# BoloniniD/CSWin-UNet

Measured on AMD Instinct MI355X. Metric: training images/sec (224x224, cswin_tiny), higher is better.
Workload: dtype f32; 1 GPU; cswin_tiny_224_lite, synthetic 224x224 9-class, bs=24/GPU, fp32 matmul, fwd + 0.4CE+0.6Dice + bwd + SGD(momentum) step, drop_path 0.2; global_batch=24, img_size=224, parallelism=dp1, hip_graph=True

## Files before the change

cswin_unet_amd/_lib.py:

```python
import ctypes
import os
from ctypes import c_char_p, c_double, c_float, c_int, c_long, c_size_t, c_void_p

import torch

_HERE = os.path.dirname(os.path.abspath(__file__))
LIB_PATH = os.path.join(_HERE, "libcswin_hip.so")

P, I, F, SZ, L, D = c_void_p, c_int, c_float, c_size_t, c_long, c_double

ABI_VERSION = 4

SIGNATURES = {
    "cswin_last_error": (c_char_p, []),
    "cswin_abi_version": (I, []),
    "cswin_device_ok": (I, []),
    "cswin_attn_fwd": (I, [P, P, P, P, P, P, I, I, I, I, P, P, I, F, F, ctypes.c_ulonglong, P, I, P]),
    "cswin_attn_bwd_workspace": (SZ, [I, I, I, I, P, P, I]),
    "cswin_attn_bwd": (I, [P, P, P, P, P, P, P, P, P, P, SZ, I, I, I, I, P, P, I, F, P, F, ctypes.c_ulonglong, P, I, P]),
    "cswin_img2windows": (I, [P, P, I, I, I, I, I, I, P]),
    "cswin_windows2img": (I, [P, P, I, I, I, I, I, I, P]),
    "cswin_layernorm_fwd": (I, [P, P, P, P, P, P, I, I, F, I, P]),
    "cswin_layernorm_bwd_workspace": (SZ, [I, I]),
    "cswin_layernorm_bwd": (I, [P, P, P, P, P, P, P, P, P, P, SZ, I, I, P, P, P]),
    "cswin_linear_fwd": (I, [P, P, I, P, P, P, P, P, P, I, I, I, I, I, I, P]),
    "cswin_linear_bwd_data": (I, [P, P, P, P, I, P, P, I, P, I, I, I, I, I, P]),
    "cswin_linear_bwd_weight_workspace": (SZ, [I, I, I]),
    "cswin_linear_bwd_weight": (I, [P, P, P, I, P, I, P, P, P, SZ, I, I, I, P, I, P]),
    "cswin_linear_bwd_weight_batch": (I, [P, I, P, P, I, P]),
    "cswin_linear_bwd_tail": (I, [P, P, P, I, I, I, P, I, P, P, I, P]),
    "cswin_linear_bwd_weight_batch_masked": (I, [P, I, P, P, I, P, P, P]),
    "cswin_linear_bwd_tail_masked": (I, [P, P, P, I, I, I, P, I, P, P, I, P, P, P]),
    "cswin_rows_sum_multi": (I, [P, I, P]),
    "cswin_conv_tok_fwd": (I, [P, P, P, P, I, I, I, I, I, I, I, I, I, P]),
    "cswin_conv_tok_bwd_data": (I, [P, P, P, I, I, I, I, I, I, I, I, I, P]),
    "cswin_conv_tok_bwd_weight_workspace": (SZ, [I, I, I, I, I, I, I, I]),
    "cswin_conv_tok_bwd_weight": (I, [P, P, P, P, P, SZ, I, I, I, I, I, I, I, I, I, P, I, P]),
    "cswin_conv_weight_permute": (I, [P, P, P, I, I, I, I, P]),
    "cswin_conv_weight_unpermute": (I, [P, P, I, I, I, I, P]),
    "cswin_conv_weight_flipT": (I, [P, P, I, I, I, P]),
    "cswin_conv_weight_images": (I, [P, I, P]),
    "cswin_conv_tok_bwd_weight_cpad": (I, [P, P, P, P, P, SZ, I, I, I, I, I, I, I, I, I, P, I, P]),
    "cswin_nchw_to_tokens": (I, [P, P, I, I, I, I, I, P]),
    "cswin_tokens_to_nchw": (I, [P, P, I, I, I, I, I, P]),
    "cswin_carafe_fwd": (I, [P, P, P, P, P, I, I, I, I, I, P]),
    "cswin_carafe_bwd_workspace": (SZ, [I, I, I, I, I]),
    "cswin_carafe_bwd": (I, [P, P, P, P, P, P, P, SZ, I, I, I, I, I, P, P]),
    "cswin_carafe_fwd_nchw": (I, [P, P, P, P, P, I, I, I, I, I, I, P]),
    "cswin_carafe_bwd_nchw_ok": (I, [I, I, I, I]),
    "cswin_carafe_bwd_nchw": (I, [P, P, P, P, P, P, P, SZ, I, I, I, I, I, I, P, P]),
    "cswin_head_compose": (I, [P, P, P, P, P, I, I, I, I, P]),
    "cswin_head_compose_bwd": (I, [P, P, P, P, P, P, P, P, I, I, I, P]),
    "cswin_loss_workspace": (SZ, [I, I, L]),
    "cswin_loss_sums": (I, [P, P, P, P, SZ, I, I, L, I, P]),
    "cswin_loss_finalize": (I, [P, P, P, D, I, F, F, P, P]),
    "cswin_loss_bwd": (I, [P, P, P, P, P, F, F, I, I, L, I, P]),
    "cswin_cl_loss_workspace": (SZ, [I, I, L]),
    "cswin_cl_loss_sums": (I, [P, P, P, I, P, P, P, P, SZ, I, I, I, L, F, F, F, P]),
    "cswin_cl_loss_finalize": (I, [P, P, P, D, D, I, F, F, F, F, P]),
    "cswin_cl_loss_bwd": (I, [P, P, P, I, P, P, P, P, P, F, F, F, I, I, I, L, F, F, F, P]),
    "cswin_dropout": (I, [P, P, P, P, L, L, F, ctypes.c_ulonglong, P, P]),
    "cswin_sgd_flat": (I, [P, P, P, L, P, F, F, F, P, P]),
    "cswin_multi_copy": (I, [P, I, P]),
    "cswin_chunk_sumsq": (I, [P, P, P, I, P, P]),
    "cswin_norm_finalize": (I, [P, P, I, F, F, P, P, P]),
    "cswin_adamw_flat": (I, [P, P, P, P, P, I, P, P, P, D, D, D, F, F, D, D, P, P]),
    "cswin_tpgm_chunk_stats": (I, [P, P, P, P, I, I, P, P]),
    "cswin_tpgm_finalize": (I, [P, P, I, I, P, P, P, P, D, D, D, D, I, P, P, P, P]),
    "cswin_tpgm_project": (I, [P, P, P, P, P, I, P, P]),
    "cswin_pack_bf16": (I, [P, P, L, P]),
    "cswin_pack_bf16_scaled": (I, [P, P, L, F, P]),
    "cswin_unpack_bf16": (I, [P, P, L, P]),
    "cswin_seg_metrics_nbins": (I, [I, I, I]),
    "cswin_seg_metrics_workspace": (SZ, [I, I, I, I, I]),
    "cswin_seg_metrics": (I, [P, P, P, P, P, SZ, I, I, I, I, I, P]),
    "cswin_resize_banded": (I, [P, P, P, P, I, P, P, I, I, I, I, I, I, I, P]),
    "cswin_argmax_zoom_back": (I, [P, P, P, P, I, I, I, I, I, I, P]),
    "cswin_argmax_zoom_back_classes": (I, [P, P, P, P, P, I, I, I, I, I, I, I, P]),
    "cswin_class_counts": (I, [P, I, P, I, P, I, L, I, P]),
    "cswin_augment_gather": (I, [P, P, P, I, I, I, I, I, I, P]),
    "cswin_augment_labels": (I, [P, P, P, P, P, P, P, I, I, I, I, I, I, P]),
}



class WgradDesc(ctypes.Structure):
    _fields_ = [("dy", c_void_p), ("x", c_void_p), ("row_scale", c_void_p), ("dw", c_void_p), ("dbias", c_void_p),
                ("workspace", c_void_p), ("ws_bytes", c_size_t), ("rows_per_sample", c_int), ("M", c_int), ("N", c_int),
                ("K", c_int), ("precision", c_int), ("io_bf16", c_int)]


class ReduceJob(ctypes.Structure):
    _fields_ = [("part", c_void_p), ("out", c_void_p), ("out2", c_void_p), ("n_first", ctypes.c_longlong),
                ("n", ctypes.c_longlong), ("stride", ctypes.c_longlong), ("rows", c_int), ("reserved", c_int),
                ("conv_kk", c_int), ("conv_cin", c_int)]


class ConvImageJob(ctypes.Structure):
    _fields_ = [("w", c_void_p), ("w_perm", c_void_p), ("w_permT", c_void_p), ("w_flipT", c_void_p), ("Cout", c_int),
                ("Cin", c_int), ("ks", c_int), ("Cpad", c_int)]


class AugmentDesc(ctypes.Structure):
    _fields_ = [("kind", c_int), ("k", c_int), ("axis", c_int), ("src", c_int), ("map", c_void_p)]


_lib = None

PREC_FP32, PREC_BF16 = 0, 1
_state = {"precision": PREC_FP32, "act_bf16": True}


def precision():
    return _state["precision"]


def act_bf16():
    return _state["precision"] == PREC_BF16 and _state["act_bf16"]


def set_act_bf16(on):
    prev = _state["act_bf16"]
    _state["act_bf16"] = bool(on)
    return prev


_shadows = []


class _Shadow:

    def __init__(self, owner_obj, owner, seen):
        import weakref
        self.ref = weakref.ref(owner_obj)
        self.base, self.nbytes, self.seen = owner.data_ptr(), owner.numel() * 4, seen


def register_shadow(owner_obj, owner):
    _shadows[:] = [e for e in _shadows if e.ref() is not None and e.base != owner.data_ptr()]
    _shadows.append(_Shadow(owner_obj, owner, {p.data_ptr(): p._version for p in owner_obj.params}))


def shadow_ptr(w):
    if not _shadows or w is None:
        return None
    a = w.data_ptr()
    for e in _shadows:
        if e.base <= a < e.base + e.nbytes:
            opt = e.ref()
            if opt is None:
                return None
            if e.seen.get(a) != w._version:
                opt.refresh_shadow()
                e.seen.clear()
                e.seen.update({p.data_ptr(): p._version for p in opt.params})
                e.seen[a] = w._version
            return c_void_p(opt.flat_param16.data_ptr() + (a - e.base) // 2)
    return None


def shadows_current(opt):
    if _state["precision"] != PREC_BF16:
        return
    for e in _shadows:
        if e.ref() is opt:
            if any(e.seen.get(p.data_ptr()) != p._version for p in opt.params):
                opt.refresh_shadow()
                e.seen.clear()
                e.seen.update({p.data_ptr(): p._version for p in opt.params})
            return


def set_precision(mode):
    prev = _state["precision"]
    _state["precision"] = int(mode)
    if int(mode) == PREC_BF16 and prev != PREC_BF16:
        for e in _shadows:
            opt = e.ref()
            if opt is not None:
# ... 53 lines not shown
```

cswin_unet_amd/csrc/gemm.hip:

```cpp
#include <stdlib.h>

#include <type_traits>
#include "common.h"
#include "gemm_epilogue.h"

int cswin_gemm16(int mode, int epi_mode, const void* A, const void* B, const void* epilogue, int M, int NO, int R, void* stream);
int cswin_wgrad16_batch(const cswin_wgrad_desc* d, int n, const int* splits, const int* rows_per_split, const cswin_reduce_job* pending,
                        int npending, void* stream, long long* stamps);

namespace {

constexpr int BKMAX = 64;

typedef __bf16 bf16x8 __attribute__((ext_vector_type(8)));

#define CSWIN_CHECK_PRECISION(p, who) CSWIN_REQUIRE((p) == 0 || (p) == 1, CSWIN_ERR_UNSUPPORTED, who ": precision %d (0 = fp32, 1 = bf16 operands)", (p))

struct PlainSrc {
    const float* p; long ld; int rows, cols;
    const float* row_scale; int rows_per_sample;
    int bf16;
    static constexpr bool fast_div = false;
    struct Row { const float* base; float s; };
    typedef int Col;
    __device__ Col col(int j) const { return j; }
    __device__ Row row(int i) const {
        Row r;
        r.base = (i < rows) ? p + (long)i * ld : nullptr;
        r.s = (row_scale && i < rows) ? row_scale[i / rows_per_sample] : 1.0f;
        return r;
    }
    __device__ const float* ptr(const Row& r, int j) const { return (r.base && j < cols) ? r.base + j : nullptr; }
};

template <class S> __device__ __forceinline__ bool src_is_bf16(const S&) { return false; }
__device__ __forceinline__ bool src_is_bf16(const PlainSrc& s) { return s.bf16 != 0; }
template <class S> __device__ __forceinline__ u32x2 src_load4_bf16(const S&, const float*) { return u32x2{0u, 0u}; }
__device__ __forceinline__ u32x2 src_load4_bf16(const PlainSrc& s, const float* p) {
    return *reinterpret_cast<const u32x2*>(reinterpret_cast<const __bf16*>(s.p) + (p - s.p));
}
template <class S> __device__ __forceinline__ typename S::Row src_mapped_row(const S&, int, float) { return typename S::Row{}; }
__device__ __forceinline__ PlainSrc::Row src_mapped_row(const PlainSrc& s, int row, float f) {
    PlainSrc::Row r;
    r.base = row >= 0 ? s.p + (long)row * s.ld : nullptr;
    r.s = f;
    return r;
}
template <class S> __device__ __forceinline__ const float* src_row_scale(const S&) { return nullptr; }
__device__ __forceinline__ const float* src_row_scale(const PlainSrc& s) { return s.row_scale; }

struct ConcatSrc {
    const float* p0; const float* p1; long ld0, ld1; int rows, cols, c0;
    static constexpr bool fast_div = false;
    struct Row { const float* b0; const float* b1; float s; };
    typedef int Col;
    __device__ Col col(int j) const { return j; }
    __device__ Row row(int i) const {
        Row r;
        r.b0 = (i < rows) ? p0 + (long)i * ld0 : nullptr;
        r.b1 = (i < rows) ? p1 + (long)i * ld1 : nullptr;
        r.s = 1.0f;
        return r;
    }
    __device__ const float* ptr(const Row& r, int j) const {
        if (!r.b0 || j >= cols) return nullptr;
        return j < c0 ? r.b0 + j : r.b1 + (j - c0);
    }
};

template <bool FAST> __device__ __forceinline__ int qdiv(int n, int d, unsigned m) {
    if constexpr (FAST) return fdiv1(n, m);
    else return n / d;
}
struct ConvMagics { unsigned img, w, c, ks, stride; };

template <bool FAST>
struct ConvSrcT {
    const float* x; int B, H, W, C, OH, OW, ks, stride, pad; int rows, cols;
    static constexpr bool fast_div = FAST;
    ConvMagics m;
    struct Row { int b, iy0, ix0; float s; };
    struct Col { int ky, kx, ci; };
    __device__ Row row(int i) const {
        Row r;
        r.s = 1.0f;
        if (i >= rows) { r.b = -1; r.iy0 = r.ix0 = 0; return r; }
        int ohw = OH * OW;
        r.b = qdiv<FAST>(i, ohw, m.img);
        int rem = i - r.b * ohw;
        int oy = qdiv<FAST>(rem, OW, m.w);
        r.iy0 = oy * stride - pad;
        r.ix0 = (rem - oy * OW) * stride - pad;
        return r;
    }
    __device__ Col col(int j) const {
        Col c;
        if (j >= cols) { c.ky = c.kx = 0; c.ci = -1; return c; }
        int tap = qdiv<FAST>(j, C, m.c);
        c.ci = j - tap * C;
        c.ky = qdiv<FAST>(tap, ks, m.ks);
        c.kx = tap - c.ky * ks;
        return c;
    }
    __device__ const float* ptr(const Row& r, const Col& c) const {
        if (r.b < 0 || c.ci < 0) return nullptr;
        int iy = r.iy0 + c.ky, ix = r.ix0 + c.kx;
        if ((unsigned)iy >= (unsigned)H || (unsigned)ix >= (unsigned)W) return nullptr;
        return x + ((long)(r.b * H + iy) * W + ix) * C + c.ci;
    }
};

template <bool FAST>
struct ConvTSrcT {
    const float* dy; int B, H, W, C, OH, OW, ks, stride, pad; int rows, cols;
    static constexpr bool fast_div = FAST;
    ConvMagics m;
    struct Row { int b, iy, ix; float s; };
    struct Col { int ky, kx, co; };
    __device__ Row row(int i) const {
        Row r;
        r.s = 1.0f;
        if (i >= rows) { r.b = -1; r.iy = r.ix = 0; return r; }
        int hw = H * W;
        r.b = qdiv<FAST>(i, hw, m.img);
        int rem = i - r.b * hw;
        r.iy = qdiv<FAST>(rem, W, m.w);
        r.ix = rem - r.iy * W;
        return r;
    }
    __device__ Col col(int j) const {
        Col c;
        if (j >= cols) { c.ky = c.kx = 0; c.co = -1; return c; }
        int tap = qdiv<FAST>(j, C, m.c);
        c.co = j - tap * C;
        c.ky = qdiv<FAST>(tap, ks, m.ks);
        c.kx = tap - c.ky * ks;
        return c;
    }
    __device__ const float* ptr(const Row& r, const Col& c) const {
        if (r.b < 0 || c.co < 0) return nullptr;
        int ty = r.iy + pad - c.ky, tx = r.ix + pad - c.kx;
        if (ty < 0 || tx < 0) return nullptr;
        int oy = qdiv<FAST>(ty, stride, m.stride), ox = qdiv<FAST>(tx, stride, m.stride);
        if (oy * stride != ty || ox * stride != tx || oy >= OH || ox >= OW) return nullptr;
        return dy + ((long)(r.b * OH + oy) * OW + ox) * C + c.co;
    }
};

template <bool FAST>
struct ConvTS2SrcT {
    const float* dy; int B, H, W, C, OH, OW, py, px, H2, W2, kys, kxs; int rows, cols;
    static constexpr bool fast_div = FAST;
    ConvMagics m;
    struct Row { int b, iy, ix; float s; };
    struct Col { int ky, kx, co; };
    __device__ Row row(int i) const {
        Row r;
        r.s = 1.0f;
        if (i >= rows) { r.b = -1; r.iy = r.ix = 0; return r; }
        const int hw = H2 * W2;
        r.b = qdiv<FAST>(i, hw, m.img);
        const int rem = i - r.b * hw;
        const int jy = qdiv<FAST>(rem, W2, m.w);
        r.iy = 2 * jy + py;
        r.ix = 2 * (rem - jy * W2) + px;
        return r;
    }
    __device__ Col col(int j) const {
        Col c;
        if (j >= cols) { c.ky = c.kx = 0; c.co = -1; return c; }
        const int t = qdiv<FAST>(j, C, m.c);
        c.co = j - t * C;
        c.ky = (kys >> (2 * t)) & 3;
        c.kx = (kxs >> (2 * t)) & 3;
        return c;
    }
    __device__ const float* ptr(const Row& r, const Col& c) const {
        if (r.b < 0 || c.co < 0) return nullptr;
        const int oy = (r.iy + 1 - c.ky) >> 1, ox = (r.ix + 1 - c.kx) >> 1;
        if (oy >= OH || ox >= OW) return nullptr;
        return dy + ((long)(r.b * OH + oy) * OW + ox) * C + c.co;
    }
};

template <bool FAST>
struct TapRowsSrcT {
    const float* w; int Cout, Cin, taps; int rows, cols;
    unsigned m_cout;
    struct Row { const float* base; float s; };
    typedef int Col;
    __device__ Row row(int i) const {
        Row r;
        r.s = 1.0f;
        if (i >= rows) { r.base = nullptr; return r; }
        const int t = qdiv<FAST>(i, Cout, m_cout), co = i - t * Cout;
        r.base = w + ((long)((taps >> (4 * t)) & 15) * Cout + co) * Cin;
        return r;
    }
    __device__ Col col(int j) const { return j; }
    __device__ const float* ptr(const Row& r, int j) const { return (r.base && j < cols) ? r.base + j : nullptr; }
};

template <int BM, int BN, int BK, int KW, bool A_RC, bool B_RC>
constexpr int gemm_lds_floats() {
    constexpr int NW = (BM >= 64 ? 2 : 1) * (BN >= 64 ? 2 : 1);
    constexpr int LDR = BK + 4;
    constexpr int A_ELEMS = A_RC ? BM * LDR : BK * (BM + 4);
    constexpr int B_ELEMS = B_RC ? BN * LDR : BK * (BN + 4);
    return (A_ELEMS + B_ELEMS) > NW * EP_WAVE_FLOATS ? (A_ELEMS + B_ELEMS) : NW * EP_WAVE_FLOATS;
}

struct RowMask { const float* skip; int nsamples, rows_per_sample, splits; unsigned magic; };
constexpr int MASK_MAX_SAMPLES = 256;
struct KeptList { int n; int idx[MASK_MAX_SAMPLES]; float scale[MASK_MAX_SAMPLES]; };

template <int BM, int BN, int BK, int KW, bool A_RC, bool B_RC, int VEC, int EPI, bool SCALE_A, int PREC, class ASrc, class BSrc,
          bool MASKED = false>
__device__ __forceinline__ void gemm_body(float* lds, const ASrc& A, const BSrc& B, const Epilogue& epi, int M, int N, int R,
                                          int r_per_split, int tiles_m, int tiles_n, int bid, int nblk, int stamp_row,
                                          const RowMask* mk = nullptr, KeptList* kept = nullptr) {
    constexpr int WGM = BM >= 64 ? 2 : 1, WGN = BN >= 64 ? 2 : 1, NW = WGM * WGN;
    constexpr int WM = BM / WGM, WN = BN / WGN;
    constexpr int FM = WM / 32, FN = WN / 32;
    constexpr int LDR = BK + 4;
    constexpr int LDA = A_RC ? LDR : BM + 4;
    constexpr int LDB = B_RC ? LDR : BN + 4;
    constexpr int A_ELEMS = A_RC ? BM * LDR : BK * (BM + 4);
    constexpr int B_ELEMS = B_RC ? BN * LDR : BK * (BN + 4);
    constexpr int LDS_FLOATS = gemm_lds_floats<BM, BN, BK, KW, A_RC, B_RC>();
    static_assert(LDS_FLOATS >= A_ELEMS + B_ELEMS && LDS_FLOATS >= NW * EP_WAVE_FLOATS, "gemm_lds_floats out of step with the tile geometry");
    float* As = lds;
    float* Bs = lds + A_ELEMS;
    constexpr int LD16 = BK + 8;
    unsigned short* As16 = reinterpret_cast<unsigned short*>(lds);
    unsigned short* Bs16 = As16 + BM * LD16;
    static_assert(PREC == 0 || ((BM + BN) * LD16 * 2 <= LDS_FLOATS * 4 && (BK / KW) % 16 == 0), "bf16 tile does not fit");

    constexpr int NTH = 64 * NW * KW;
    const int tid = threadIdx.x, lane = tid & 63, wave = (tid >> 6) % NW, kg = tid / (64 * NW);
    const int li = lane & 31, lh = lane >> 5;
    const int xq = nblk >> 3, xr = nblk & 7, xcd = bid & 7;
    const int lb = (xcd < xr ? xcd * (xq + 1) : xr * (xq + 1) + (xcd - xr) * xq) + (bid >> 3);
    const int tiles = tiles_m * tiles_n;
    const int split = lb / tiles;
    const int tile = lb - split * tiles;
    const int m0 = (tile / tiles_n) * BM, n0 = (tile % tiles_n) * BN;
    if constexpr (MASKED) {
        static_assert(!A_RC && !B_RC && VEC == 4 && BM == BN && std::is_same<ASrc, PlainSrc>::value && std::is_same<BSrc, PlainSrc>::value,
                      "the sample mask serves weight gradients of plain matrices (one row mapping for both operands)");
        if (tid < 64) {
            int n = 0;
            for (int s0 = 0; s0 < mk->nsamples; s0 += 64) {
                const int s = s0 + lane;
                const bool keep = s < mk->nsamples && mk->skip[s] != 0.0f;
                const unsigned long long bal = __ballot(keep);
                if (keep) {
                    const int at = n + __popcll(bal & ((1ull << lane) - 1ull));
                    kept->idx[at] = s;
                    kept->scale[at] = src_row_scale(A) ? src_row_scale(A)[s] : 1.0f;
                }
                n += __popcll(bal);
            }
            if (tid == 0) kept->n = n;
        }
        __syncthreads();
        R = __builtin_amdgcn_readfirstlane(kept->n) * mk->rows_per_sample;
        r_per_split = ((R + mk->splits - 1) / mk->splits + 7) / 8 * 8;
    }
    const int r_begin = split * r_per_split;
    const int r_end = min(R, r_begin + r_per_split);
    const int wm0 = (wave / WGN) * WM, wn0 = (wave % WGN) * WN;

    constexpr int QA = BM * BK / (4 * NTH), QB = BN * BK / (4 * NTH);
    static_assert(QA >= 1 && QB >= 1 && (BK / KW) % 8 == 0, "tile too small for this many wave groups");
    constexpr int A_CPR = A_RC ? BK / 4 : BM / 4;
    constexpr int B_CPR = B_RC ? BK / 4 : BN / 4;
    constexpr int A_RPP = NTH / A_CPR, B_RPP = NTH / B_CPR;
    const int a_c = tid % A_CPR, a_r = tid / A_CPR;
    const int b_c = tid % B_CPR, b_r = tid / B_CPR;

    typename ASrc::Row arow[QA];
    typename BSrc::Row brow[QB];
    if (A_RC) {
#pragma unroll
        for (int q = 0; q < QA; ++q) arow[q] = A.row(m0 + a_r + q * A_RPP);
    }
    if (B_RC) {
#pragma unroll
        for (int q = 0; q < QB; ++q) brow[q] = B.row(n0 + b_r + q * B_RPP);
    }

    const typename ASrc::Col acol = A.col(m0 + 4 * a_c);
    const typename BSrc::Col bcol = B.col(n0 + 4 * b_c);

    f32x4 pa[QA], pb[QB];
    u32x2 pa16[QA], pb16[QB];
    float pas[QA];
    auto fetch = [&](int r0, auto a16, auto b16) {
        int mrow[QA];
        float msc[QA];
        if constexpr (MASKED) {
#pragma unroll
            for (int q = 0; q < QA; ++q) {
                const int c = r0 + a_r + q * A_RPP;
                mrow[q] = -1;
                msc[q] = 1.0f;
                if (c < r_end) {
                    const int j = fdiv1(c, mk->magic);
                    mrow[q] = kept->idx[j] * mk->rows_per_sample + (c - j * mk->rows_per_sample);
                    msc[q] = kept->scale[j];
                }
            }
        }
#pragma unroll
        for (int q = 0; q < QA; ++q) {
            typename ASrc::Row rr;
            int j;
            if (A_RC) {
                rr = arow[q];
                j = r0 + 4 * a_c;
            } else {
                const int r = r0 + a_r + q * A_RPP;
                if constexpr (MASKED) rr = src_mapped_row(A, mrow[q], msc[q]);
                else rr = A.row(r < r_end ? r : 0x7fffffff);
                j = m0 + 4 * a_c;
            }
            if (SCALE_A) pas[q] = rr.s;
            if (VEC == 4) {
                const float* p = A_RC ? (j < r_end ? A.ptr(rr, A.col(j)) : nullptr) : A.ptr(rr, acol);
                if constexpr (decltype(a16)::value) {
                    pa16[q] = u32x2{0u, 0u};
                    if (p) pa16[q] = src_load4_bf16(A, p);
                } else {
                    pa[q] = f32x4{0.f, 0.f, 0.f, 0.f};
                    if (p) pa[q] = *reinterpret_cast<const f32x4*>(p);
                }
            } else {
#pragma unroll
                for (int e = 0; e < 4; ++e) {
                    const float* p = (!A_RC || j + e < r_end) ? A.ptr(rr, A.col(j + e)) : nullptr;
                    pa[q][e] = p ? *p : 0.f;
                }
            }
        }
#pragma unroll
        for (int q = 0; q < QB; ++q) {
            typename BSrc::Row rr;
            int j;
            if (B_RC) {
                rr = brow[q];
                j = r0 + 4 * b_c;
            } else {
                const int r = r0 + b_r + q * B_RPP;
                if constexpr (MASKED) rr = src_mapped_row(B, mrow[q], 1.0f);
                else rr = B.row(r < r_end ? r : 0x7fffffff);
                j = n0 + 4 * b_c;
            }
            if (VEC == 4) {
                const float* p = B_RC ? (j < r_end ? B.ptr(rr, B.col(j)) : nullptr) : B.ptr(rr, bcol);
                if constexpr (decltype(b16)::value) {
                    pb16[q] = u32x2{0u, 0u};
                    if (p) pb16[q] = src_load4_bf16(B, p);
                } else {
                    pb[q] = f32x4{0.f, 0.f, 0.f, 0.f};
                    if (p) pb[q] = *reinterpret_cast<const f32x4*>(p);
                }
            } else {
#pragma unroll
                for (int e = 0; e < 4; ++e) {
                    const float* p = (!B_RC || j + e < r_end) ? B.ptr(rr, B.col(j + e)) : nullptr;
                    pb[q][e] = p ? *p : 0.f;
                }
            }
        }
    };
    auto stash = [&](auto a16, auto b16) {
#pragma unroll
        for (int q = 0; q < QA; ++q) {
            f32x4 v = f32x4{0.f, 0.f, 0.f, 0.f};
            if constexpr (!decltype(a16)::value) v = pa[q];
            if constexpr (PREC == 1) {
                unsigned h01, h23;
                if constexpr (decltype(a16)::value) {
                    h01 = pa16[q][0];
                    h23 = pa16[q][1];
                    if (SCALE_A) {
                        const u32x2 u = __builtin_bit_cast(u32x2, __builtin_convertvector(widen_bf16x4(pa16[q]) * pas[q], bf16x4));
                        h01 = u[0]; h23 = u[1];
                    }
                } else {
                    if (SCALE_A) v *= pas[q];
                    const u32x2 u = __builtin_bit_cast(u32x2, __builtin_convertvector(v, bf16x4));
                    h01 = u[0]; h23 = u[1];
                }
                if (A_RC) {
                    *reinterpret_cast<u32x2*>(&As16[(a_r + q * A_RPP) * LD16 + 4 * a_c]) = u32x2{h01, h23};
                } else {
                    unsigned short* col = &As16[4 * a_c * LD16 + a_r + q * A_RPP];
                    col[0] = (unsigned short)(h01 & 0xffffu);
                    col[LD16] = (unsigned short)(h01 >> 16);
                    col[2 * LD16] = (unsigned short)(h23 & 0xffffu);
                    col[3 * LD16] = (unsigned short)(h23 >> 16);
                }
            } else {
                if (SCALE_A) v *= pas[q];
                *reinterpret_cast<f32x4*>(&As[(a_r + q * A_RPP) * LDA + 4 * a_c]) = v;
            }
        }
#pragma unroll
        for (int q = 0; q < QB; ++q) {
            if constexpr (PREC == 1) {
                u32x2 hb;
                if constexpr (decltype(b16)::value) hb = pb16[q];
                else hb = __builtin_bit_cast(u32x2, __builtin_convertvector(pb[q], bf16x4));
                if (B_RC) {
                    *reinterpret_cast<u32x2*>(&Bs16[(b_r + q * B_RPP) * LD16 + 4 * b_c]) = hb;
                } else {
                    static_assert(B_RC || BN == 64, "transposed-read B image is laid out for 64-column tiles");
                    const int row = b_r + q * B_RPP;
                    *reinterpret_cast<u32x2*>(&Bs16[row * BN + 8 * ((b_c >> 1) ^ (((row >> 1) & 1) << 2)) + 4 * (b_c & 1)]) = hb;
                }
            } else {
                *reinterpret_cast<f32x4*>(&Bs[(b_r + q * B_RPP) * LDB + 4 * b_c]) = pb[q];
            }
        }
    };

    f32x16 acc[FM][FN];
#pragma unroll
    for (int i = 0; i < FM; ++i)
#pragma unroll
        for (int j = 0; j < FN; ++j)
#pragma unroll
            for (int e = 0; e < 16; ++e) acc[i][j][e] = 0.f;

    float csum = 0.f;
    const bool do_colsum = !A_RC && epi.colsum && n0 == 0 && tid < BM;

    if (epi.stamps && tid == 0) { epi.stamps[8L * stamp_row + 0] = __builtin_amdgcn_s_memtime(); epi.stamps[8L * stamp_row + 4] = __builtin_amdgcn_s_getreg(6164); epi.stamps[8L * stamp_row + 5] = __builtin_amdgcn_s_memrealtime(); }
    auto main_loop = [&](auto a16, auto b16) {
        fetch(r_begin, a16, b16);
        stash(a16, b16);
        __syncthreads();
        if (epi.stamps && tid == 0) epi.stamps[8L * stamp_row + 1] = __builtin_amdgcn_s_memtime();
        for (int r0 = r_begin; r0 < r_end; r0 += BK) {
            const bool more = r0 + BK < r_end;
            if (more) fetch(r0 + BK, a16, b16);
            if (do_colsum) {
                if constexpr (PREC == 1) {
#pragma unroll 8
                    for (int r = 0; r < BK; ++r)
                        csum += __builtin_bit_cast(float, (unsigned)As16[tid * LD16 + r] << 16);
                } else {
#pragma unroll 8
                    for (int r = 0; r < BK; ++r) csum += As[r * LDA + tid];
                }
            }
            if constexpr (PREC == 1) {
#pragma unroll
                for (int kk = kg * (BK / KW); kk < (kg + 1) * (BK / KW); kk += 16) {
                    bf16x8 af[FM], bf[FN];
#pragma unroll
                    for (int i = 0; i < FM; ++i)
                        af[i] = *reinterpret_cast<const bf16x8*>(&As16[(wm0 + i * 32 + li) * LD16 + kk + 8 * lh]);
#pragma unroll
                    for (int j = 0; j < FN; ++j) {
                        if constexpr (B_RC) {
                            bf[j] = *reinterpret_cast<const bf16x8*>(&Bs16[(wn0 + j * 32 + li) * LD16 + kk + 8 * lh]);
                        } else {
                            typedef short s16x4 __attribute__((ext_vector_type(4)));
                            typedef short s16x8 __attribute__((ext_vector_type(8)));
                            typedef __attribute__((address_space(3))) s16x4 lds_s16x4;
                            const int col = wn0 + j * 32 + 16 * ((lane >> 4) & 1) + 4 * (lane & 3);
                            const int row = kk + 8 * lh + ((lane & 15) >> 2);
                            const int sw = ((row >> 1) & 1) << 2;
                            const unsigned short* a0 = &Bs16[row * BN + 8 * ((col >> 3) ^ sw) + (col & 7)];
                            const s16x4 v0 = __builtin_amdgcn_ds_read_tr16_b64_v4i16((lds_s16x4*)a0);
                            const s16x4 v1 = __builtin_amdgcn_ds_read_tr16_b64_v4i16((lds_s16x4*)(a0 + 4 * BN));
                            const s16x8 f = {v0[0], v0[1], v0[2], v0[3], v1[0], v1[1], v1[2], v1[3]};
                            bf[j] = __builtin_bit_cast(bf16x8, f);
                        }
                    }
#pragma unroll
                    for (int i = 0; i < FM; ++i)
#pragma unroll
                        for (int j = 0; j < FN; ++j)
                            acc[i][j] = __builtin_amdgcn_mfma_f32_32x32x16_bf16(af[i], bf[j], acc[i][j], 0, 0, 0);
                }
            } else
#pragma unroll
            for (int kk = kg * (BK / KW); kk < (kg + 1) * (BK / KW); kk += 8) {
                f32x4 af[FM], bf[FN];
#pragma unroll
                for (int i = 0; i < FM; ++i) {
                    if (A_RC) {
                        af[i] = *reinterpret_cast<const f32x4*>(&As[(wm0 + i * 32 + li) * LDA + kk + 4 * lh]);
                    } else {
#pragma unroll
                        for (int s = 0; s < 4; ++s) af[i][s] = As[(kk + 4 * lh + s) * LDA + wm0 + i * 32 + li];
                    }
                }
#pragma unroll
                for (int j = 0; j < FN; ++j) {
                    if (B_RC) {
                        bf[j] = *reinterpret_cast<const f32x4*>(&Bs[(wn0 + j * 32 + li) * LDB + kk + 4 * lh]);
                    } else {
#pragma unroll
                        for (int s = 0; s < 4; ++s) bf[j][s] = Bs[(kk + 4 * lh + s) * LDB + wn0 + j * 32 + li];
                    }
                }
#pragma unroll
                for (int s = 0; s < 4; ++s)
#pragma unroll
                    for (int i = 0; i < FM; ++i)
#pragma unroll
                        for (int j = 0; j < FN; ++j)
                            acc[i][j] = __builtin_amdgcn_mfma_f32_32x32x2f32(af[i][s], bf[j][s], acc[i][j], 0, 0, 0);
            }
            __syncthreads();
            if (more) {
                stash(a16, b16);
                __syncthreads();
            }
        }
    };
    if (r_begin < r_end) {
        constexpr bool CAN_A16 = PREC == 1 && A_RC && VEC == 4 && std::is_same<ASrc, PlainSrc>::value;
        constexpr bool CAN_B16 = PREC == 1 && A_RC && VEC == 4 && std::is_same<BSrc, PlainSrc>::value;
        const bool a_is16 = CAN_A16 && src_is_bf16(A), b_is16 = CAN_B16 && src_is_bf16(B);
        if constexpr (CAN_A16 && CAN_B16) {
            if (a_is16 && b_is16) main_loop(std::true_type{}, std::true_type{});
            else if (a_is16) main_loop(std::true_type{}, std::false_type{});
            else if (b_is16) main_loop(std::false_type{}, std::true_type{});
            else main_loop(std::false_type{}, std::false_type{});
        } else if constexpr (CAN_B16) {
            if (b_is16) main_loop(std::false_type{}, std::true_type{});
            else main_loop(std::false_type{}, std::false_type{});
        } else {
            main_loop(std::false_type{}, std::false_type{});
        }
    }

    if (epi.stamps && tid == 0) epi.stamps[8L * stamp_row + 2] = __builtin_amdgcn_s_memtime();
    if (KW > 1) {
        static_assert(KW == 1 || (KW / 2) * NW * FM * FN * 16 * 64 <= LDS_FLOATS, "LDS too small for the k-group reduction");
        constexpr int PATCH = FM * FN * 16 * 64;
#pragma unroll
        for (int half = KW / 2; half >= 1; half >>= 1) {
            if (kg >= half && kg < 2 * half) {
                float* dst = lds + ((kg - half) * NW + wave) * PATCH + lane;
#pragma unroll
                for (int i = 0; i < FM; ++i)
#pragma unroll
                    for (int j = 0; j < FN; ++j)
#pragma unroll
                        for (int g = 0; g < 16; ++g) dst[((i * FN + j) * 16 + g) * 64] = acc[i][j][g];
            }
            __syncthreads();
            if (kg < half) {
                const float* src = lds + (kg * NW + wave) * PATCH + lane;
#pragma unroll
                for (int i = 0; i < FM; ++i)
#pragma unroll
                    for (int j = 0; j < FN; ++j)
#pragma unroll
                        for (int g = 0; g < 16; ++g) acc[i][j][g] += src[((i * FN + j) * 16 + g) * 64];
            }
            __syncthreads();
        }
        if (kg != 0) return;
    }
    Epilogue e = epi;
    e.C += (long)split * e.split_stride;
    if constexpr (EPI == EPI_GELUBWD) {
        if (e.pre_bf16) run_epilogue<EPI, FM, FN, true>(e, acc, M, N, m0 + wm0, n0 + wn0, lane, lds + wave * EP_WAVE_FLOATS, e.vec_store != 0);
        else run_epilogue<EPI, FM, FN, false>(e, acc, M, N, m0 + wm0, n0 + wn0, lane, lds + wave * EP_WAVE_FLOATS, e.vec_store != 0);
    } else {
        if constexpr (ASrc::fast_div)
            run_epilogue<EPI, FM, FN, false, true>(e, acc, M, N, m0 + wm0, n0 + wn0, lane, lds + wave * EP_WAVE_FLOATS, e.vec_store != 0, A.m.img, A.m.w);
        else
            run_epilogue<EPI, FM, FN>(e, acc, M, N, m0 + wm0, n0 + wn0, lane, lds + wave * EP_WAVE_FLOATS, e.vec_store != 0);
    }
    if (epi.stamps && tid == 0) { epi.stamps[8L * stamp_row + 3] = __builtin_amdgcn_s_memtime(); epi.stamps[8L * stamp_row + 6] = __builtin_amdgcn_s_memrealtime(); }
    if (do_colsum && m0 + tid < M) epi.colsum[(long)split * epi.colsum_stride + m0 + tid] = csum;
}

constexpr int gemm_threads(int BM, int BN, int KW) { return 64 * (BM >= 64 ? 2 : 1) * (BN >= 64 ? 2 : 1) * KW; }

template <int BM, int BN, int BK, int KW, bool A_RC, bool B_RC, int VEC, int EPI, bool SCALE_A, int PREC, class ASrc, class BSrc>
__global__ __launch_bounds__(gemm_threads(BM, BN, KW)) void gemm_kernel(ASrc A, BSrc B, Epilogue epi, int M, int N, int R,
                                                    int r_per_split, int tiles_m, int tiles_n) {
    __shared__ __attribute__((aligned(16))) float lds[gemm_lds_floats<BM, BN, BK, KW, A_RC, B_RC>()];
    gemm_body<BM, BN, BK, KW, A_RC, B_RC, VEC, EPI, SCALE_A, PREC, ASrc, BSrc>(lds, A, B, epi, M, N, R, r_per_split, tiles_m, tiles_n,
                                                                              (int)blockIdx.x, (int)gridDim.x, (int)blockIdx.x);
}

constexpr int WGRAD_BATCH = 4;
template <class ASrc, class BSrc>
struct GemmBatch {
    ASrc A[WGRAD_BATCH];
    BSrc B[WGRAD_BATCH];
    Epilogue e[WGRAD_BATCH];
    int M[WGRAD_BATCH], N[WGRAD_BATCH], R[WGRAD_BATCH], rps[WGRAD_BATCH], tm[WGRAD_BATCH], tn[WGRAD_BATCH];
    int first[WGRAD_BATCH + 1];
    int n;
    RowMask mask[WGRAD_BATCH];
};
typedef GemmBatch<PlainSrc, PlainSrc> WgradBatch;

__device__ __forceinline__ void wgrad_masked_batch_body(float* lds, KeptList* kept, const WgradBatch& b, int p, int bid) {
    if (b.mask[p].skip) {
        gemm_body<64, 64, 64, 2, false, false, 4, EPI_PLAIN, true, 0, PlainSrc, PlainSrc, true>(
            lds, b.A[p], b.B[p], b.e[p], b.M[p], b.N[p], b.R[p], b.rps[p], b.tm[p], b.tn[p], bid - b.first[p],
            b.first[p + 1] - b.first[p], bid, &b.mask[p], kept);
        return;
    }
    gemm_body<64, 64, 64, 2, false, false, 4, EPI_PLAIN, true, 0, PlainSrc, PlainSrc>(
        lds, b.A[p], b.B[p], b.e[p], b.M[p], b.N[p], b.R[p], b.rps[p], b.tm[p], b.tn[p], bid - b.first[p],
        b.first[p + 1] - b.first[p], bid);
}

template <int PREC>
__global__ __launch_bounds__(512) void gemm_wgrad_batch_kernel(WgradBatch b) {
    int p = 0;
    while (p + 1 < b.n && (int)blockIdx.x >= b.first[p + 1]) ++p;
    __shared__ __attribute__((aligned(16))) float lds[gemm_lds_floats<64, 64, 64, 2, false, false>()];
    gemm_body<64, 64, 64, 2, false, false, 4, EPI_PLAIN, true, PREC, PlainSrc, PlainSrc>(
        lds, b.A[p], b.B[p], b.e[p], b.M[p], b.N[p], b.R[p], b.rps[p], b.tm[p], b.tn[p], (int)blockIdx.x - b.first[p],
        b.first[p + 1] - b.first[p], (int)blockIdx.x);
}
__global__ __launch_bounds__(512) void gemm_wgrad_batch_masked_kernel(WgradBatch b) {
    int p = 0;
    while (p + 1 < b.n && (int)blockIdx.x >= b.first[p + 1]) ++p;
    __shared__ __attribute__((aligned(16))) float lds[gemm_lds_floats<64, 64, 64, 2, false, false>()];
    __shared__ KeptList kept;
    wgrad_masked_batch_body(lds, &kept, b, p, (int)blockIdx.x);
}

struct BlockTail {
    PlainSrc dA, dB;
    Epilogue de;
    int dM, dN, dR, drps, dtm, dtn, nd;
    WgradBatch w;
    ReduceRiders r;
};
constexpr int BLOCK_TAIL_LDS = gemm_lds_floats<64, 64, 64, 2, true, false>() > gemm_lds_floats<64, 64, 64, 2, false, false>()
                                   ? gemm_lds_floats<64, 64, 64, 2, true, false>() : gemm_lds_floats<64, 64, 64, 2, false, false>();
template <bool MASKED>
__device__ __forceinline__ void block_tail_body(float (&lds)[BLOCK_TAIL_LDS], KeptList* kept, const BlockTail& t) {
    const WgradBatch& b = t.w;
    const int nw = b.first[b.n];
    if ((int)blockIdx.x >= nw + t.nd) {
        if (threadIdx.x >= 256) return;
        static_assert(sizeof(lds) >= sizeof(float) * RS_G * (RS_COLS + 1), "reduction scratch");
        rows_sum_dispatch(t.r.j, t.r.first_block, t.r.njobs, (int)blockIdx.x - nw - t.nd, reinterpret_cast<float(*)[RS_COLS + 1]>(lds));
        return;
    }
    if ((int)blockIdx.x >= nw) {
        gemm_body<64, 64, 64, 2, true, false, 4, EPI_PLAIN, false, 0, PlainSrc, PlainSrc>(
            lds, t.dA, t.dB, t.de, t.dM, t.dN, t.dR, t.drps, t.dtm, t.dtn, (int)blockIdx.x - nw, t.nd, (int)blockIdx.x);
        return;
    }
    const int bid = (int)blockIdx.x;
    int p = 0;
    while (p + 1 < b.n && bid >= b.first[p + 1]) ++p;
    if constexpr (MASKED) {
        wgrad_masked_batch_body(lds, kept, b, p, bid);
    } else {
        gemm_body<64, 64, 64, 2, false, false, 4, EPI_PLAIN, true, 0, PlainSrc, PlainSrc>(
            lds, b.A[p], b.B[p], b.e[p], b.M[p], b.N[p], b.R[p], b.rps[p], b.tm[p], b.tn[p], bid - b.first[p],
            b.first[p + 1] - b.first[p], (int)blockIdx.x);
    }
}
__global__ __launch_bounds__(512) void gemm_block_tail_kernel(BlockTail t) {
    __shared__ __attribute__((aligned(16))) float lds[BLOCK_TAIL_LDS];
    block_tail_body<false>(lds, nullptr, t);
}
__global__ __launch_bounds__(512) void gemm_block_tail_masked_kernel(BlockTail t) {
    __shared__ __attribute__((aligned(16))) float lds[BLOCK_TAIL_LDS];
    __shared__ KeptList kept;
    block_tail_body<true>(lds, &kept, t);
}

template <int KW, int PREC, bool FAST>
__global__ __launch_bounds__(256 * KW) void gemm_conv_s2_dgrad_batch_kernel(GemmBatch<ConvTS2SrcT<FAST>, TapRowsSrcT<FAST>> b) {
    int p = 0;
    while (p + 1 < b.n && (int)blockIdx.x >= b.first[p + 1]) ++p;
    __shared__ __attribute__((aligned(16))) float lds[gemm_lds_floats<64, 64, (KW == 1 ? 32 : 64), KW, true, false>()];
    gemm_body<64, 64, (KW == 1 ? 32 : 64), KW, true, false, 4, EPI_PLAIN, false, PREC, ConvTS2SrcT<FAST>, TapRowsSrcT<FAST>>(
        lds, b.A[p], b.B[p], b.e[p], b.M[p], b.N[p], b.R[p], b.rps[p], b.tm[p], b.tn[p], (int)blockIdx.x - b.first[p],
        b.first[p + 1] - b.first[p], (int)blockIdx.x);
}

template <int BM, int BN, int BK, int KW, bool A_RC, bool B_RC, int VEC, int EPI, bool SCALE_A, int PREC, class ASrc, class BSrc>
void launch_cfg(const ASrc& A, const BSrc& B, const Epilogue& epi, int M, int N, int R, int splits, int r_per_split,
                hipStream_t st) {
    int tm = cdiv(M, BM), tn = cdiv(N, BN);
    dim3 grid(tm * tn * splits);
    const int pad_lds = cswin_tuning().gemm_pad_lds;
    hipLaunchKernelGGL((gemm_kernel<BM, BN, BK, KW, A_RC, B_RC, VEC, EPI, SCALE_A, PREC, ASrc, BSrc>), grid, dim3(gemm_threads(BM, BN, KW)), pad_lds, st, A, B, epi,
                       M, N, R, r_per_split, tm, tn);
}

int k_groups(long blocks, int r_len) {
    if (blocks < 320 && r_len >= 512) return 4;
    if (blocks < 640 && r_len >= 256) return 2;
    return 1;
}

int one_split(int R) { return cdiv(R, BKMAX) * BKMAX; }

template <bool A_RC, bool B_RC, int VEC, int EPI, bool SCALE_A, class ASrc, class BSrc>
void launch_gemm(const ASrc& A, const BSrc& B, const Epilogue& epi_in, int M, int N, int R, int splits, int r_per_split,
                 int precision, hipStream_t st) {
    Epilogue epi = epi_in;
    epi.vec_store = epilogue_vec_ok(epi, N);
    auto blocks = [&](int bm, int bn) { return (long)cdiv(M, bm) * cdiv(N, bn) * splits; };
    const int forced_kw = cswin_tuning().gemm_kw;
    const int forced_tile = cswin_tuning().gemm_tile;
    const double pen2 = cswin_tuning().gemm_pen2;
    auto cost = [&](int bm, int bn, double pen) { return (double)((blocks(bm, bn) + 255) / 256) * bm * bn * pen; };
    int tile = 1;
    if (splits == 1 && cost(64, 32, pen2) < cost(64, 64, 1.0)) tile = 2;
    if (forced_tile) tile = forced_tile;
    const int r_len = r_per_split < R ? r_per_split : R;
    const bool wgrad = !A_RC && !B_RC;
    if (precision == 1) {
        if (k_groups(blocks(64, 64), r_len) >= 2 || (wgrad && r_len >= 256))
            launch_cfg<64, 64, 64, 2, A_RC, B_RC, VEC, EPI, SCALE_A, 1>(A, B, epi, M, N, R, splits, r_per_split, st);
        else launch_cfg<64, 64, 64, 1, A_RC, B_RC, VEC, EPI, SCALE_A, 1>(A, B, epi, M, N, R, splits, r_per_split, st);
        return;
    }
    if (tile == 2) {
        if (k_groups(blocks(64, 32), r_len) >= 2)
            return launch_cfg<64, 32, 64, 2, A_RC, B_RC, VEC, EPI, SCALE_A, 0>(A, B, epi, M, N, R, splits, r_per_split, st);
        return launch_cfg<64, 32, 32, 1, A_RC, B_RC, VEC, EPI, SCALE_A, 0>(A, B, epi, M, N, R, splits, r_per_split, st);
    }
    int kw = k_groups(blocks(64, 64), r_len);
    if (wgrad && r_len >= 256 && kw < 2) kw = 2;
    if (forced_kw) kw = forced_kw;
    if (kw == 4) launch_cfg<64, 64, 64, 4, A_RC, B_RC, VEC, EPI, SCALE_A, 0>(A, B, epi, M, N, R, splits, r_per_split, st);
    else if (kw == 2) launch_cfg<64, 64, 64, 2, A_RC, B_RC, VEC, EPI, SCALE_A, 0>(A, B, epi, M, N, R, splits, r_per_split, st);
    else launch_cfg<64, 64, 32, 1, A_RC, B_RC, VEC, EPI, SCALE_A, 0>(A, B, epi, M, N, R, splits, r_per_split, st);
}

template <bool A_RC, bool B_RC, int EPI, bool SCALE_A, class ASrc, class BSrc>
void launch_gemm_vec(bool vec, const ASrc& A, const BSrc& B, const Epilogue& epi, int M, int N, int R, int splits, int r_per_split,
// ... 222 lines not shown
        if (x.njobs > 0) {
            rblocks = fill_reduce_table(x.jobs, x.njobs, t.r.j, t.r.first_block);
            CSWIN_REQUIRE(rblocks >= 0, CSWIN_ERR_SHAPE, "linear_bwd_tail: bad pending reduction");
            t.r.njobs = x.njobs;
        }
        static_assert(sizeof(BlockTail) <= 4096, "kernel argument block");
        if (any_mask) hipLaunchKernelGGL(gemm_block_tail_masked_kernel, dim3(blocks + t.nd + rblocks), dim3(512), 0, (hipStream_t)stream, t);
        else hipLaunchKernelGGL(gemm_block_tail_kernel, dim3(blocks + t.nd + rblocks), dim3(512), 0, (hipStream_t)stream, t);
    } else if (any_mask) {
        hipLaunchKernelGGL(gemm_wgrad_batch_masked_kernel, dim3(blocks), dim3(512), 0, (hipStream_t)stream, b);
    } else if (precision == 1) {
        hipLaunchKernelGGL(gemm_wgrad_batch_kernel<1>, dim3(blocks), dim3(512), 0, (hipStream_t)stream, b);
    } else {
        hipLaunchKernelGGL(gemm_wgrad_batch_kernel<0>, dim3(blocks), dim3(512), 0, (hipStream_t)stream, b);
    }
    CSWIN_LAUNCH_CHECK();
    return CSWIN_OK;
}

bool conv_magics(ConvMagics* m, long nrows, int img, int w, long ncols, int c, int ks, int cmax, int stride) {
    *m = ConvMagics{fdiv_magic(img), fdiv_magic(w), fdiv_magic(c), fdiv_magic(ks), fdiv_magic(stride)};
    return fdiv_exact(nrows + 63, img) && fdiv_exact(img - 1, w) && fdiv_exact(ncols - 1, c) && fdiv_exact((long)ks * ks - 1, ks) &&
           (stride == 0 || fdiv_exact(cmax, stride));
}
template <class F> void with_fast_div(bool fast, F f) {
    if (fast) f(std::true_type{});
    else f(std::false_type{});
}

int conv_wgrad_impl(const float* dy, const float* x, float* dw_perm, float* dbias, void* workspace, size_t ws_bytes, int B, int H,
                    int W, int Cin, int Cout, int ks, int stride, int pad, int torch_layout, int Cin_param,
                    cswin_reduce_job* deferred, int precision, void* stream) {
    CSWIN_CHECK_PRECISION(precision, "conv_tok_bwd_weight");
    CSWIN_REQUIRE(dy && x && dw_perm, CSWIN_ERR_SHAPE, "conv_tok_bwd_weight: null pointer");
    CSWIN_REQUIRE(Cin % 4 == 0 && Cout % 4 == 0 && aligned16(dy) && aligned16(x), CSWIN_ERR_ALIGN, "conv_tok_bwd_weight: channels %% 4 and 16-B alignment required");
    CSWIN_REQUIRE(!torch_layout || Cin < 65536, CSWIN_ERR_UNSUPPORTED, "conv_tok_bwd_weight: torch_layout needs Cin < 65536");
    int OH = (H + 2 * pad - ks) / stride + 1, OW = (W + 2 * pad - ks) / stride + 1;
    int M = B * OH * OW, K = ks * ks * Cin;
    size_t need = WgradSlabs::bytes(M, Cout, K);
    CSWIN_REQUIRE(workspace && ws_bytes >= need, CSWIN_ERR_WORKSPACE, "conv_tok_bwd_weight: workspace %zu < %zu", ws_bytes, need);
    hipStream_t st = (hipStream_t)stream;
    int splits, rps;
    choose_split(M, Cout, K, &splits, &rps);
    const WgradSlabs slabs(workspace, Cout, K);
    PlainSrc A = {dy, Cout, M, Cout, nullptr, 1};
    ConvMagics mg;
    with_fast_div(conv_magics(&mg, M, OH * OW, OW, K, Cin, ks, 0, 0), [&](auto fast) {
        ConvSrcT<decltype(fast)::value> Bm = {x, B, H, W, Cin, OH, OW, ks, stride, pad, M, K, mg};
        launch_gemm<false, false, 4, EPI_PLAIN, false>(A, Bm, slabs.epilogue(dbias != nullptr), Cout, K, M, splits, rps, precision, st);
    });
    CSWIN_LAUNCH_CHECK();
    reduce_now_or_defer(slabs.job(dw_perm, dbias, splits, torch_layout ? ks * ks : 0,
                                  torch_layout ? (Cin | (Cin_param != Cin ? Cin_param << 16 : 0)) : 0), deferred, st);
    CSWIN_LAUNCH_CHECK();
    return CSWIN_OK;
}

}

extern "C" {

void cswin_debug_set_stamps(void* p) { g_stamps = (long long*)p; }

int cswin_linear_bwd_weight_batch_masked(const cswin_wgrad_desc* d, int n, cswin_reduce_job* deferred, const cswin_reduce_job* pending,
                                         int npending, const float* const* skip, const int* nsamples, void* stream);
int cswin_linear_bwd_tail_masked(const float* dy, const float* w, float* dx, int M, int N, int K, const cswin_wgrad_desc* d, int n,
                                 cswin_reduce_job* deferred, const cswin_reduce_job* pending, int npending, const float* const* skip,
                                 const int* nsamples, void* stream);

int cswin_linear_fwd(const float* x, const float* x2, int k_split, const float* w, const float* bias, float* y,
                     float* y_act, const float* residual, const float* row_scale, int rows_per_sample, int M, int N,
                     int K, int precision, int io_bf16, void* stream) {
    CSWIN_CHECK_PRECISION(precision, "linear_fwd");
    CSWIN_REQUIRE(io_bf16 == 0 || (precision == 1 && (!x2 || !(io_bf16 & 1)) && (io_bf16 & ~7) == 0 && K % 4 == 0 && N % 4 == 0 && !((io_bf16 & 2) && residual)), CSWIN_ERR_UNSUPPORTED,
                  "linear_fwd: bf16 storage (io_bf16 = %d: 1 = x, 2 = y / y_act, 4 = w) needs precision 1, a plain input for bit 1, K and N multiples of 4; a residual output stays fp32", io_bf16);
    CSWIN_REQUIRE(x && w && y && M > 0 && N > 0 && K > 0, CSWIN_ERR_SHAPE, "linear_fwd: bad arguments M=%d N=%d K=%d", M, N, K);
    CSWIN_REQUIRE(!x2 || (k_split > 0 && k_split < K), CSWIN_ERR_SHAPE, "linear_fwd: bad concat split %d of K=%d", k_split, K);
    CSWIN_REQUIRE(!row_scale || rows_per_sample > 0, CSWIN_ERR_SHAPE, "linear_fwd: rows_per_sample must be > 0");
    hipStream_t st = (hipStream_t)stream;
    Epilogue e = plain_epilogue(y, N);
    e.bias = bias;
    e.Cact = y_act; e.ldact = N;
    e.residual = residual; e.ldres = N;
    e.row_scale = row_scale; e.rows_per_sample = rows_per_sample;
    e.c_bf16 = (io_bf16 & 2) != 0;
    PlainSrc B = {w, K, N, K, nullptr, 1, (io_bf16 >> 2) & 1};
    CSWIN_REQUIRE(!(y_act && residual), CSWIN_ERR_UNSUPPORTED, "linear_fwd: activation and residual epilogues are exclusive");
    const int rk = one_split(K);
    if (x2) {
        CSWIN_REQUIRE(!y_act, CSWIN_ERR_UNSUPPORTED, "linear_fwd: concat input does not support the activation epilogue");
        ConcatSrc A = {x, x2, k_split, K - k_split, M, K, k_split};
        bool vec = (k_split % 4 == 0) && (K % 4 == 0) && aligned16(x) && aligned16(x2) && aligned16(w);
        CSWIN_REQUIRE(io_bf16 == 0 || (io_bf16 == 4 && vec), CSWIN_ERR_UNSUPPORTED, "linear_fwd: a concat input takes only the bf16 weight flag (4), with 16-B aligned operands");
        if (residual) launch_gemm_vec<true, true, EPI_RES, false>(vec, A, B, e, M, N, K, 1, rk, precision, st);
        else launch_gemm_vec<true, true, EPI_PLAIN, false>(vec, A, B, e, M, N, K, 1, rk, precision, st);
    } else {
        if (precision == 1 && (io_bf16 & 5) == 5) {
            if (cswin_gemm16(0, y_act ? EPI_ACT : (residual ? EPI_RES : EPI_PLAIN), x, w, &e, M, N, K, stream) == 0) {
                CSWIN_LAUNCH_CHECK();
                return CSWIN_OK;
            }
        }
        PlainSrc A = {x, K, M, K, nullptr, 1, io_bf16 & 1};
        bool vec = (K % 4 == 0) && aligned16(x) && aligned16(w);
        CSWIN_REQUIRE(io_bf16 == 0 || (vec && aligned16(y) && (!y_act || aligned16(y_act)) && (!bias || aligned16(bias))), CSWIN_ERR_ALIGN,
                      "linear_fwd: bf16 storage needs 16-B aligned operands");
        if (y_act) launch_gemm_vec<true, true, EPI_ACT, false>(vec, A, B, e, M, N, K, 1, rk, precision, st);
        else if (residual) launch_gemm_vec<true, true, EPI_RES, false>(vec, A, B, e, M, N, K, 1, rk, precision, st);
        else launch_gemm_vec<true, true, EPI_PLAIN, false>(vec, A, B, e, M, N, K, 1, rk, precision, st);
    }
    CSWIN_LAUNCH_CHECK();
    return CSWIN_OK;
}

int cswin_linear_bwd_data(const float* dy, const float* w, float* dx, float* dx2, int k_split, const float* gelu_pre,
                          const float* row_scale, int rows_per_sample, const float* add, int M, int N, int K,
                          int precision, int io_bf16, void* stream) {
    CSWIN_CHECK_PRECISION(precision, "linear_bwd_data");
    CSWIN_REQUIRE(io_bf16 == 0 || (precision == 1 && ((!dx2 && !add) || (io_bf16 & ~4) == 0) && (io_bf16 & ~15) == 0 && K % 4 == 0 && N % 4 == 0), CSWIN_ERR_UNSUPPORTED,
                  "linear_bwd_data: bf16 storage (io_bf16 = %d: 1 = dy, 2 = dx, 4 = w, 8 = gelu_pre) needs precision 1, K and N multiples of 4; split / add outputs take only the weight flag", io_bf16);
    CSWIN_REQUIRE(dy && w && dx && M > 0 && N > 0 && K > 0, CSWIN_ERR_SHAPE, "linear_bwd_data: bad arguments");
    CSWIN_REQUIRE(!dx2 || (k_split > 0 && k_split < K), CSWIN_ERR_SHAPE, "linear_bwd_data: bad concat split");
    CSWIN_REQUIRE(!row_scale || rows_per_sample > 0, CSWIN_ERR_SHAPE, "linear_bwd_data: rows_per_sample must be > 0");
    hipStream_t st = (hipStream_t)stream;
    Epilogue e = plain_epilogue(dx, dx2 ? k_split : K);
    e.C2 = dx2; e.ldc2 = K - k_split; e.col_split = dx2 ? k_split : 0;
    e.gelu_pre = gelu_pre; e.ldpre = K;
    e.row_scale = row_scale; e.rows_per_sample = rows_per_sample;
    e.residual = add; e.ldres = K;
    e.c_bf16 = (io_bf16 & 2) != 0;
    e.pre_bf16 = (io_bf16 & 8) != 0;
    CSWIN_REQUIRE(io_bf16 == 0 || (aligned16(dy) && aligned16(w) && aligned16(dx) && (!gelu_pre || aligned16(gelu_pre))), CSWIN_ERR_ALIGN,
                  "linear_bwd_data: bf16 storage needs 16-B aligned operands");
    PlainSrc A = {dy, N, M, N, nullptr, 1, io_bf16 & 1};
    PlainSrc B = {w, K, N, K, nullptr, 1, (io_bf16 >> 2) & 1};
    bool vec = (N % 4 == 0) && (K % 4 == 0) && aligned16(dy) && aligned16(w);
    const int rn = one_split(N);
    const int modes = (dx2 != nullptr) + (gelu_pre != nullptr) + (add != nullptr);
    CSWIN_REQUIRE(modes <= 1, CSWIN_ERR_UNSUPPORTED, "linear_bwd_data: dx2 / gelu_pre / add are mutually exclusive");
    if (precision == 1 && !dx2 && !add && (io_bf16 & 5) == 5) {
        if (cswin_gemm16(1, gelu_pre ? EPI_GELUBWD : EPI_PLAIN, dy, w, &e, M, K, N, stream) == 0) {
            CSWIN_LAUNCH_CHECK();
            return CSWIN_OK;
        }
    }
    if (dx2) launch_gemm_vec<true, false, EPI_SPLIT2, false>(vec, A, B, e, M, K, N, 1, rn, precision, st);
    else if (gelu_pre) launch_gemm_vec<true, false, EPI_GELUBWD, false>(vec, A, B, e, M, K, N, 1, rn, precision, st);
    else if (add) launch_gemm_vec<true, false, EPI_RES, false>(vec, A, B, e, M, K, N, 1, rn, precision, st);
    else launch_gemm_vec<true, false, EPI_PLAIN, false>(vec, A, B, e, M, K, N, 1, rn, precision, st);
    CSWIN_LAUNCH_CHECK();
    return CSWIN_OK;
}

size_t cswin_linear_bwd_weight_workspace(int M, int N, int K) { return WgradSlabs::bytes(M, N, K); }

int cswin_linear_bwd_weight(const float* dy, const float* x, const float* x2, int k_split, const float* row_scale,
                            int rows_per_sample, float* dw, float* dbias, void* workspace, size_t ws_bytes, int M,
                            int N, int K, cswin_reduce_job* deferred, int precision, void* stream) {
    CSWIN_CHECK_PRECISION(precision, "linear_bwd_weight");
    CSWIN_REQUIRE(dy && x && dw && M > 0 && N > 0 && K > 0, CSWIN_ERR_SHAPE, "linear_bwd_weight: bad arguments");
    CSWIN_REQUIRE(!x2 || (k_split > 0 && k_split < K), CSWIN_ERR_SHAPE, "linear_bwd_weight: bad concat split");
    CSWIN_REQUIRE(!row_scale || rows_per_sample > 0, CSWIN_ERR_SHAPE, "linear_bwd_weight: rows_per_sample must be > 0");
    size_t need = WgradSlabs::bytes(M, N, K);
    CSWIN_REQUIRE(workspace && ws_bytes >= need, CSWIN_ERR_WORKSPACE, "linear_bwd_weight: workspace %zu < %zu", ws_bytes, need);
    hipStream_t st = (hipStream_t)stream;
    const cswin_wgrad_desc d1 = {dy, x, row_scale, dw, dbias, workspace, ws_bytes, rows_per_sample, M, N, K, precision, 0};
    if (precision == 1 && !x2 && wgrad_aligned(d1)) {
        cswin_reduce_job job;
        int rc = wgrad_batch_impl(&d1, 1, &job, TailExtras{"linear_bwd_weight_batch"}, stream);
        if (rc) return rc;
        reduce_now_or_defer(job, deferred, st);
        CSWIN_LAUNCH_CHECK();
        return CSWIN_OK;
    }
    return wgrad_tiled(dy, x, x2, k_split, row_scale, rows_per_sample, dw, dbias, workspace, M, N, K, deferred, precision, st);
}

int cswin_linear_bwd_weight_batch(const cswin_wgrad_desc* d, int n, cswin_reduce_job* deferred, const cswin_reduce_job* pending, int npending,
                                  void* stream) {
    return cswin_linear_bwd_weight_batch_masked(d, n, deferred, pending, npending, nullptr, nullptr, stream);
}

int cswin_linear_bwd_weight_batch_masked(const cswin_wgrad_desc* d, int n, cswin_reduce_job* deferred, const cswin_reduce_job* pending,
                                         int npending, const float* const* skip, const int* nsamples, void* stream) {
    return wgrad_batch_impl(d, n, deferred,
                            TailExtras{"linear_bwd_weight_batch", nullptr, nullptr, nullptr, 0, 0, 0, pending, npending, skip, nsamples}, stream);
}

int cswin_linear_bwd_tail(const float* dy, const float* w, float* dx, int M, int N, int K, const cswin_wgrad_desc* d, int n,
                          cswin_reduce_job* deferred, const cswin_reduce_job* pending, int npending, void* stream) {
    return cswin_linear_bwd_tail_masked(dy, w, dx, M, N, K, d, n, deferred, pending, npending, nullptr, nullptr, stream);
}

int cswin_linear_bwd_tail_masked(const float* dy, const float* w, float* dx, int M, int N, int K, const cswin_wgrad_desc* d, int n,
                                 cswin_reduce_job* deferred, const cswin_reduce_job* pending, int npending, const float* const* skip,
                                 const int* nsamples, void* stream) {
    CSWIN_REQUIRE(dy && w && dx && M > 0 && N > 0 && K > 0, CSWIN_ERR_SHAPE, "linear_bwd_tail: bad data-gradient arguments");
    return wgrad_batch_impl(d, n, deferred, TailExtras{"linear_bwd_tail", dy, w, dx, M, N, K, pending, npending, skip, nsamples}, stream);
}

int cswin_conv_tok_fwd(const float* x, const float* w_perm, const float* bias, float* y, int B, int H, int W, int Cin,
                       int Cout, int ks, int stride, int pad, int precision, void* stream) {
    CSWIN_CHECK_PRECISION(precision, "conv_tok_fwd");
    CSWIN_REQUIRE(x && w_perm && y && B > 0 && H > 0 && W > 0 && Cin > 0 && Cout > 0, CSWIN_ERR_SHAPE, "conv_tok_fwd: bad arguments");
    CSWIN_REQUIRE(Cin % 4 == 0 && aligned16(x) && aligned16(w_perm), CSWIN_ERR_ALIGN, "conv_tok_fwd: Cin %% 4 and 16-B alignment required");
    int OH = (H + 2 * pad - ks) / stride + 1, OW = (W + 2 * pad - ks) / stride + 1;
    int M = B * OH * OW, R = ks * ks * Cin;
    PlainSrc Bm = {w_perm, R, Cout, R, nullptr, 1};
    Epilogue e = plain_epilogue(y, Cout);
    e.bias = bias;
    ConvMagics mg;
    with_fast_div(conv_magics(&mg, M, OH * OW, OW, R, Cin, ks, 0, 0), [&](auto fast) {
        ConvSrcT<decltype(fast)::value> A = {x, B, H, W, Cin, OH, OW, ks, stride, pad, M, R, mg};
        launch_gemm<true, true, 4, EPI_PLAIN, false>(A, Bm, e, M, Cout, R, 1, one_split(R), precision, (hipStream_t)stream);
    });
    CSWIN_LAUNCH_CHECK();
    return CSWIN_OK;
}

int cswin_conv_tok_bwd_data(const float* dy, const float* w_permT, float* dx, int B, int H, int W, int Cin, int Cout,
                            int ks, int stride, int pad, int precision, void* stream) {
    CSWIN_CHECK_PRECISION(precision, "conv_tok_bwd_data");
    CSWIN_REQUIRE(dy && w_permT && dx, CSWIN_ERR_SHAPE, "conv_tok_bwd_data: null pointer");
    CSWIN_REQUIRE(Cin % 4 == 0 && Cout % 4 == 0 && aligned16(dy) && aligned16(w_permT), CSWIN_ERR_ALIGN, "conv_tok_bwd_data: channels %% 4 and 16-B alignment required");
    int OH = (H + 2 * pad - ks) / stride + 1, OW = (W + 2 * pad - ks) / stride + 1;
    if (ks == 3 && stride == 2 && pad == 1) {
        bool fast_ok = true;
        for (int py = 0; py < 2; ++py)
            for (int px = 0; px < 2; ++px) {
                const int H2 = (H - py + 1) / 2, W2 = (W - px + 1) / 2;
                ConvMagics mg;
                if (H2 > 0 && W2 > 0) fast_ok = fast_ok && conv_magics(&mg, (long)B * H2 * W2, H2 * W2, W2, 4L * Cout, Cout, 1, 0, 0);
            }
        with_fast_div(fast_ok, [&](auto fast) {
            constexpr bool FAST = decltype(fast)::value;
            GemmBatch<ConvTS2SrcT<FAST>, TapRowsSrcT<FAST>> b = {};
            int rmax = 0;
            for (int py = 0; py < 2; ++py)
                for (int px = 0; px < 2; ++px) {
                    const int H2 = (H - py + 1) / 2, W2 = (W - px + 1) / 2;
                    if (H2 <= 0 || W2 <= 0) continue;
                    int kys = 0, kxs = 0, taps = 0, nt = 0;
                    for (int ky = (py ? 0 : 1); ky < 3; ky += 2)
                        for (int kx = (px ? 0 : 1); kx < 3; kx += 2) {
                            kys |= ky << (2 * nt);
                            kxs |= kx << (2 * nt);
                            taps |= (ky * 3 + kx) << (4 * nt);
                            ++nt;
                        }
                    const int Mc = B * H2 * W2, Rc = nt * Cout;
                    Epilogue e = plain_epilogue(dx, Cin);
                    e.rm_on = 1; e.rm_H = H; e.rm_W = W; e.rm_H2 = H2; e.rm_W2 = W2; e.rm_py = py; e.rm_px = px;
                    ConvMagics mg;
                    conv_magics(&mg, Mc, H2 * W2, W2, Rc, Cout, 1, 0, 0);
                    push(b, ConvTS2SrcT<FAST>{dy, B, H, W, Cout, OH, OW, py, px, H2, W2, kys, kxs, Mc, Rc, mg},
                         TapRowsSrcT<FAST>{w_permT, Cout, Cin, taps, Rc, Cin, mg.c}, e, Mc, Cin, Rc, one_split(Rc), 1);
                    rmax = Rc > rmax ? Rc : rmax;
                }
            if (b.n > 0) {
                const int blocks = b.first[b.n];
                hipStream_t st = (hipStream_t)stream;
                const int kw = k_groups(blocks, rmax);
                if (precision == 1) hipLaunchKernelGGL((gemm_conv_s2_dgrad_batch_kernel<2, 1, FAST>), dim3(blocks), dim3(512), 0, st, b);
                else if (kw == 4) hipLaunchKernelGGL((gemm_conv_s2_dgrad_batch_kernel<4, 0, FAST>), dim3(blocks), dim3(1024), 0, st, b);
                else if (kw == 2) hipLaunchKernelGGL((gemm_conv_s2_dgrad_batch_kernel<2, 0, FAST>), dim3(blocks), dim3(512), 0, st, b);
                else hipLaunchKernelGGL((gemm_conv_s2_dgrad_batch_kernel<1, 0, FAST>), dim3(blocks), dim3(256), 0, st, b);
            }
        });
        CSWIN_LAUNCH_CHECK();
        return CSWIN_OK;
    }
    int M = B * H * W, R = ks * ks * Cout;
    PlainSrc Bm = {w_permT, Cin, R, Cin, nullptr, 1};
    Epilogue e = plain_epilogue(dx, Cin);
    ConvMagics mg;
    with_fast_div(conv_magics(&mg, M, H * W, W, R, Cout, ks, (H > W ? H : W) + pad, stride), [&](auto fast) {
        ConvTSrcT<decltype(fast)::value> A = {dy, B, H, W, Cout, OH, OW, ks, stride, pad, M, R, mg};
        launch_gemm<true, false, 4, EPI_PLAIN, false>(A, Bm, e, M, Cin, R, 1, one_split(R), precision, (hipStream_t)stream);
    });
    CSWIN_LAUNCH_CHECK();
    return CSWIN_OK;
}

size_t cswin_conv_tok_bwd_weight_workspace(int B, int H, int W, int Cin, int Cout, int ks, int stride, int pad) {
    int OH = (H + 2 * pad - ks) / stride + 1, OW = (W + 2 * pad - ks) / stride + 1;
    return WgradSlabs::bytes(B * OH * OW, Cout, ks * ks * Cin);
}

int cswin_conv_tok_bwd_weight(const float* dy, const float* x, float* dw_perm, float* dbias, void* workspace,
                              size_t ws_bytes, int B, int H, int W, int Cin, int Cout, int ks, int stride, int pad,
                              int torch_layout, cswin_reduce_job* deferred, int precision, void* stream) {
    return conv_wgrad_impl(dy, x, dw_perm, dbias, workspace, ws_bytes, B, H, W, Cin, Cout, ks, stride, pad, torch_layout, Cin, deferred,
                           precision, stream);
}

int cswin_conv_tok_bwd_weight_cpad(const float* dy, const float* x, float* dw, float* dbias, void* workspace, size_t ws_bytes,
                                   int B, int H, int W, int Cin, int Cin_param, int Cout, int ks, int stride, int pad,
                                   cswin_reduce_job* deferred, int precision, void* stream) {
    CSWIN_REQUIRE(Cin_param > 0 && Cin_param <= Cin && Cin < 65536, CSWIN_ERR_SHAPE, "conv_tok_bwd_weight_cpad: 0 < Cin_param <= Cin < 65536");
    return conv_wgrad_impl(dy, x, dw, dbias, workspace, ws_bytes, B, H, W, Cin, Cout, ks, stride, pad, 1, Cin_param, deferred, precision,
                           stream);
}

int cswin_rows_sum_multi(const cswin_reduce_job* jobs, int njobs, void* stream) { return rows_sum_multi(jobs, njobs, stream); }

}
// ... 1 lines not shown
```

cswin_unet_amd/csrc/gemm_epilogue.h:

```cpp
#pragma once
#include "common.h"

namespace {

__device__ __forceinline__ f32x4 widen_bf16x4(u32x2 raw) {
    return f32x4{__builtin_bit_cast(float, raw[0] << 16), __builtin_bit_cast(float, raw[0] & 0xffff0000u),
                 __builtin_bit_cast(float, raw[1] << 16), __builtin_bit_cast(float, raw[1] & 0xffff0000u)};
}
__device__ __forceinline__ void epi_store4(float* base, long idx, f32x4 v, int bf16) {
    if (bf16) *reinterpret_cast<bf16x4*>(reinterpret_cast<__bf16*>(base) + idx) = __builtin_convertvector(v, bf16x4);
    else *reinterpret_cast<f32x4*>(base + idx) = v;
}

enum { EPI_PLAIN = 0, EPI_ACT = 1, EPI_RES = 2, EPI_GELUBWD = 3, EPI_SPLIT2 = 4 };

struct Epilogue {
    float* C; long ldc;
    float* C2; long ldc2; int col_split;
    const float* bias;
    float* Cact; long ldact;
    const float* residual; long ldres;
    const float* row_scale; int rows_per_sample;
    const float* gelu_pre; long ldpre;
    long split_stride;
    float* colsum; int colsum_stride;
    int rm_on, rm_H, rm_W, rm_H2, rm_W2, rm_py, rm_px;
    int vec_store;
    int c_bf16;
    int pre_bf16;
    long long* stamps;
};

constexpr int EP_LD = 36;
constexpr int EP_WAVE_FLOATS = 32 * EP_LD;

template <int EPI, int FM, int FN, bool PRE16 = false, bool FDIV = false>
__device__ __forceinline__ void run_epilogue(const Epilogue& e, f32x16 (&acc)[FM][FN], int M, int N, int mb, int nb,
                                             int lane, float* wbuf, bool vec, unsigned m_hw = 0, unsigned m_w2 = 0) {
    const int li = lane & 31, lh = lane >> 5;
    const int rrow = lane >> 3, rcol = (lane & 7) * 4;
    const bool has_rs = e.row_scale != nullptr;
    auto out_row = [&](int m) -> long {
        if (!e.rm_on) return m;
        const int hw = e.rm_H2 * e.rm_W2;
        int b, jy;
        if constexpr (FDIV) { b = fdiv1(m, m_hw); jy = fdiv1(m - b * hw, m_w2); }
        else { b = m / hw; jy = (m - b * hw) / e.rm_W2; }
        const int rem = m - b * hw;
        return ((long)b * e.rm_H + 2 * jy + e.rm_py) * e.rm_W + 2 * (rem - jy * e.rm_W2) + e.rm_px;
    };
#pragma unroll
    for (int i = 0; i < FM; ++i) {
#pragma unroll
        for (int j = 0; j < FN; ++j) {
#pragma unroll
            for (int g = 0; g < 16; ++g) wbuf[((g & 3) + 8 * (g >> 2) + 4 * lh) * EP_LD + li] = acc[i][j][g];
            __builtin_amdgcn_fence(__ATOMIC_RELEASE, "wavefront");
            __builtin_amdgcn_wave_barrier();
            __builtin_amdgcn_fence(__ATOMIC_ACQUIRE, "wavefront");
            const int n = nb + j * 32 + rcol;
            if (vec) {
                f32x4 bias_v = {0.f, 0.f, 0.f, 0.f};
                if (e.bias && n < N) bias_v = *reinterpret_cast<const f32x4*>(e.bias + n);
                f32x4 v[4], aux[4];
                u32x2 aux16[4];
                float rs[4];
#pragma unroll
                for (int p = 0; p < 4; ++p) {
                    const int m = mb + i * 32 + rrow + 8 * p;
                    const bool ok = m < M && n < N;
                    v[p] = *reinterpret_cast<const f32x4*>(&wbuf[(rrow + 8 * p) * EP_LD + rcol]);
                    rs[p] = (has_rs && ok) ? e.row_scale[m / e.rows_per_sample] : 1.0f;
                    if (EPI == EPI_RES || EPI == EPI_GELUBWD) {
                        const float* ap = EPI == EPI_RES ? e.residual : e.gelu_pre;
                        const long ld = EPI == EPI_RES ? e.ldres : e.ldpre;
                        aux[p] = f32x4{0.f, 0.f, 0.f, 0.f};
                        aux16[p] = u32x2{0u, 0u};
                        if (ok) {
                            if constexpr (PRE16) aux16[p] = *reinterpret_cast<const u32x2*>(reinterpret_cast<const __bf16*>(ap) + (long)m * ld + n);
                            else aux[p] = *reinterpret_cast<const f32x4*>(ap + (long)m * ld + n);
                        }
                    }
                }
#pragma unroll
                for (int p = 0; p < 4; ++p) {
                    const int m = mb + i * 32 + rrow + 8 * p;
                    if (m >= M || n >= N) continue;
                    f32x4 o = v[p] + bias_v;
                    if (EPI == EPI_GELUBWD) {
                        const f32x4 pre = PRE16 ? widen_bf16x4(aux16[p]) : aux[p];
#pragma unroll
                        for (int c = 0; c < 4; ++c) o[c] *= gelu_grad_f(pre[c]);
                    }
                    if (has_rs) o *= rs[p];
                    if (EPI == EPI_RES) o += aux[p];
                    if (EPI == EPI_SPLIT2 && n >= e.col_split)
                        *reinterpret_cast<f32x4*>(e.C2 + (long)m * e.ldc2 + (n - e.col_split)) = o;
                    else
                        epi_store4(e.C, out_row(m) * e.ldc + n, o, e.c_bf16);
                    if (EPI == EPI_ACT) {
                        f32x4 a;
#pragma unroll
                        for (int c = 0; c < 4; ++c) a[c] = gelu_f(o[c]);
                        epi_store4(e.Cact, (long)m * e.ldact + n, a, e.c_bf16);
                    }
                }
            } else {
#pragma unroll
                for (int p = 0; p < 4; ++p) {
                    const int m = mb + i * 32 + rrow + 8 * p;
                    if (m >= M) continue;
                    const float rsv = has_rs ? e.row_scale[m / e.rows_per_sample] : 1.0f;
#pragma unroll
                    for (int c = 0; c < 4; ++c) {
                        const int nn = n + c;
                        if (nn >= N) continue;
                        float o = wbuf[(rrow + 8 * p) * EP_LD + rcol + c] + (e.bias ? e.bias[nn] : 0.f);
                        if (EPI == EPI_GELUBWD) o *= gelu_grad_f(e.gelu_pre[(long)m * e.ldpre + nn]);
                        o *= rsv;
                        if (EPI == EPI_RES) o += e.residual[(long)m * e.ldres + nn];
                        if (EPI == EPI_SPLIT2 && nn >= e.col_split) e.C2[(long)m * e.ldc2 + (nn - e.col_split)] = o;
                        else e.C[out_row(m) * e.ldc + nn] = o;
                        if (EPI == EPI_ACT) e.Cact[(long)m * e.ldact + nn] = gelu_f(o);
                    }
                }
            }
            __builtin_amdgcn_fence(__ATOMIC_RELEASE, "wavefront");
            __builtin_amdgcn_wave_barrier();
        }
    }
}


inline bool aligned16(const void* p) { return (reinterpret_cast<uintptr_t>(p) & 15) == 0; }

inline int epilogue_vec_ok(const Epilogue& e, int n_out) {
    auto ok = [](const void* p, long ld) { return !p || (aligned16(p) && ld % 4 == 0); };
    return n_out % 4 == 0 && aligned16(e.C) && e.ldc % 4 == 0 && ok(e.C2, e.ldc2) && (!e.C2 || e.col_split % 4 == 0) &&
           ok(e.bias, 4) && ok(e.Cact, e.ldact) && ok(e.residual, e.ldres) && ok(e.gelu_pre, e.ldpre) &&
           e.split_stride % 4 == 0;
}

}
```

cswin_unet_amd/csrc/ln.hip:

```cpp
#include "common.h"

namespace {

__device__ __forceinline__ void ln_store4(float* y, long idx, f32x4 v, int y_bf16) {
    if (y_bf16) *reinterpret_cast<bf16x4*>(reinterpret_cast<__bf16*>(y) + idx) = __builtin_convertvector(v, bf16x4);
    else *reinterpret_cast<f32x4*>(y + idx) = v;
}

template <int LPR, int VPL>
__global__ __launch_bounds__(256) void ln_fwd_kernel(const float* __restrict__ x, const float* __restrict__ gamma,
                                                      const float* __restrict__ beta, float* __restrict__ y,
                                                      float* __restrict__ mean, float* __restrict__ rstd, int M,
                                                      float eps, int y_bf16) {
    constexpr int C = 4 * LPR * VPL;
    constexpr int RPB = 256 / LPR;
    const int sub = threadIdx.x % LPR, rib = threadIdx.x / LPR;
    f32x4 g[VPL], b[VPL];
#pragma unroll
    for (int v = 0; v < VPL; ++v) {
        g[v] = *reinterpret_cast<const f32x4*>(gamma + 4 * (sub + v * LPR));
        b[v] = *reinterpret_cast<const f32x4*>(beta + 4 * (sub + v * LPR));
    }
    for (long row = (long)blockIdx.x * RPB + rib; row < M; row += (long)gridDim.x * RPB) {
        f32x4 xv[VPL];
        float s = 0.f;
#pragma unroll
        for (int v = 0; v < VPL; ++v) {
            xv[v] = *reinterpret_cast<const f32x4*>(x + row * C + 4 * (sub + v * LPR));
            s += xv[v][0] + xv[v][1] + xv[v][2] + xv[v][3];
        }
#pragma unroll
        for (int o = LPR / 2; o > 0; o >>= 1) s += __shfl_xor(s, o, 64);
        const float mu = s * (1.0f / C);
        float q = 0.f;
#pragma unroll
        for (int v = 0; v < VPL; ++v)
#pragma unroll
            for (int e = 0; e < 4; ++e) {
                float d = xv[v][e] - mu;
                q += d * d;
            }
#pragma unroll
        for (int o = LPR / 2; o > 0; o >>= 1) q += __shfl_xor(q, o, 64);
        const float rs = rsqrtf(q * (1.0f / C) + eps);
#pragma unroll
        for (int v = 0; v < VPL; ++v) {
            f32x4 o4;
#pragma unroll
            for (int e = 0; e < 4; ++e) o4[e] = (xv[v][e] - mu) * rs * g[v][e] + b[v][e];
            ln_store4(y, row * C + 4 * (sub + v * LPR), o4, y_bf16);
        }
        if (sub == 0) {
            mean[row] = mu;
            rstd[row] = rs;
        }
    }
}

template <int LPR, int VPL>
__global__ __launch_bounds__(256) void ln_bwd_kernel(const float* __restrict__ dy, const float* __restrict__ x,
                                                      const float* __restrict__ mean, const float* __restrict__ rstd,
                                                      const float* __restrict__ gamma, const float* __restrict__ dres,
                                                      float* __restrict__ dx, float* __restrict__ partial, int M,
                                                      __bf16* __restrict__ dx16) {
    constexpr int C = 4 * LPR * VPL;
    constexpr int RPB = 256 / LPR;
    __shared__ float red[2 * RPB * C];
    const int sub = threadIdx.x % LPR, rib = threadIdx.x / LPR;
    f32x4 g[VPL], dg[VPL], db[VPL];
#pragma unroll
    for (int v = 0; v < VPL; ++v) {
        g[v] = *reinterpret_cast<const f32x4*>(gamma + 4 * (sub + v * LPR));
        dg[v] = f32x4{0.f, 0.f, 0.f, 0.f};
        db[v] = f32x4{0.f, 0.f, 0.f, 0.f};
    }
    for (long row = (long)blockIdx.x * RPB + rib; row < M; row += (long)gridDim.x * RPB) {
        const float mu = mean[row], rs = rstd[row];
        f32x4 xh[VPL], gy[VPL];
        float s1 = 0.f, s2 = 0.f;
#pragma unroll
        for (int v = 0; v < VPL; ++v) {
            const long off = row * C + 4 * (sub + v * LPR);
            f32x4 xv = *reinterpret_cast<const f32x4*>(x + off);
            f32x4 dv = *reinterpret_cast<const f32x4*>(dy + off);
#pragma unroll
            for (int e = 0; e < 4; ++e) {
                xh[v][e] = (xv[e] - mu) * rs;
                gy[v][e] = dv[e] * g[v][e];
                s1 += gy[v][e];
                s2 += gy[v][e] * xh[v][e];
                dg[v][e] += dv[e] * xh[v][e];
                db[v][e] += dv[e];
            }
        }
#pragma unroll
        for (int o = LPR / 2; o > 0; o >>= 1) {
            s1 += __shfl_xor(s1, o, 64);
            s2 += __shfl_xor(s2, o, 64);
        }
        s1 *= (1.0f / C);
        s2 *= (1.0f / C);
#pragma unroll
        for (int v = 0; v < VPL; ++v) {
            const long off = row * C + 4 * (sub + v * LPR);
            f32x4 o4;
#pragma unroll
            for (int e = 0; e < 4; ++e) o4[e] = rs * (gy[v][e] - s1 - xh[v][e] * s2);
            if (dres) o4 += *reinterpret_cast<const f32x4*>(dres + off);
            *reinterpret_cast<f32x4*>(dx + off) = o4;
            if (dx16) *reinterpret_cast<bf16x4*>(dx16 + off) = __builtin_convertvector(o4, bf16x4);
        }
    }
#pragma unroll
    for (int v = 0; v < VPL; ++v)
#pragma unroll
        for (int e = 0; e < 4; ++e) {
            const int c = 4 * (sub + v * LPR) + e;
            red[rib * C + c] = dg[v][e];
            red[RPB * C + rib * C + c] = db[v][e];
        }
    __syncthreads();
    for (int c = threadIdx.x; c < 2 * C; c += 256) {
        const int which = c / C, cc = c - which * C;
        float s = 0.f;
        for (int r = 0; r < RPB; ++r) s += red[which * RPB * C + r * C + cc];
        partial[(long)blockIdx.x * 2 * C + c] = s;
    }
}

constexpr int GEN_MAXV = 4;

__global__ __launch_bounds__(256) void ln_fwd_generic_kernel(const float* __restrict__ x, const float* __restrict__ gamma,
                                                              const float* __restrict__ beta, float* __restrict__ y,
                                                              float* __restrict__ mean, float* __restrict__ rstd, int M, int C,
                                                              float eps, int y_bf16) {
    const int lane = threadIdx.x & 63, wib = threadIdx.x >> 6, nchunk = C >> 2;
    for (long row = (long)blockIdx.x * 4 + wib; row < M; row += (long)gridDim.x * 4) {
        f32x4 xv[GEN_MAXV];
        float s = 0.f;
#pragma unroll
        for (int v = 0; v < GEN_MAXV; ++v) {
            const int ch = lane + 64 * v;
            xv[v] = ch < nchunk ? *reinterpret_cast<const f32x4*>(x + row * C + 4 * ch) : f32x4{0.f, 0.f, 0.f, 0.f};
            s += xv[v][0] + xv[v][1] + xv[v][2] + xv[v][3];
        }
        const float mu = wave_sum(s) / C;
        float q = 0.f;
#pragma unroll
        for (int v = 0; v < GEN_MAXV; ++v)
            if (lane + 64 * v < nchunk) {
#pragma unroll
                for (int e = 0; e < 4; ++e) q += (xv[v][e] - mu) * (xv[v][e] - mu);
            }
        const float rs = rsqrtf(wave_sum(q) / C + eps);
#pragma unroll
        for (int v = 0; v < GEN_MAXV; ++v) {
            const int ch = lane + 64 * v;
            if (ch < nchunk) {
                const f32x4 g = *reinterpret_cast<const f32x4*>(gamma + 4 * ch), b = *reinterpret_cast<const f32x4*>(beta + 4 * ch);
                f32x4 o4;
#pragma unroll
                for (int e = 0; e < 4; ++e) o4[e] = (xv[v][e] - mu) * rs * g[e] + b[e];
                ln_store4(y, row * C + 4 * ch, o4, y_bf16);
            }
        }
        if (lane == 0) {
            mean[row] = mu;
            rstd[row] = rs;
        }
    }
}

__global__ __launch_bounds__(256) void ln_bwd_generic_kernel(const float* __restrict__ dy, const float* __restrict__ x,
                                                              const float* __restrict__ mean, const float* __restrict__ rstd,
                                                              const float* __restrict__ gamma, const float* __restrict__ dres,
                                                              float* __restrict__ dx, float* __restrict__ partial, int M, int C,
                                                              __bf16* __restrict__ dx16) {
    extern __shared__ float red[];
    const int lane = threadIdx.x & 63, wib = threadIdx.x >> 6, nchunk = C >> 2;
    f32x4 dg[GEN_MAXV], db[GEN_MAXV];
#pragma unroll
    for (int v = 0; v < GEN_MAXV; ++v) dg[v] = db[v] = f32x4{0.f, 0.f, 0.f, 0.f};
    for (long row = (long)blockIdx.x * 4 + wib; row < M; row += (long)gridDim.x * 4) {
        const float mu = mean[row], rs = rstd[row];
        f32x4 xh[GEN_MAXV], gy[GEN_MAXV];
        float s1 = 0.f, s2 = 0.f;
#pragma unroll
        for (int v = 0; v < GEN_MAXV; ++v) {
            const int ch = lane + 64 * v;
            xh[v] = gy[v] = f32x4{0.f, 0.f, 0.f, 0.f};
            if (ch < nchunk) {
                const f32x4 xv = *reinterpret_cast<const f32x4*>(x + row * C + 4 * ch);
                const f32x4 dv = *reinterpret_cast<const f32x4*>(dy + row * C + 4 * ch);
                const f32x4 g = *reinterpret_cast<const f32x4*>(gamma + 4 * ch);
#pragma unroll
                for (int e = 0; e < 4; ++e) {
                    xh[v][e] = (xv[e] - mu) * rs;
                    gy[v][e] = dv[e] * g[e];
                    s1 += gy[v][e];
                    s2 += gy[v][e] * xh[v][e];
                    dg[v][e] += dv[e] * xh[v][e];
                    db[v][e] += dv[e];
                }
            }
        }
        s1 = wave_sum(s1) / C;
        s2 = wave_sum(s2) / C;
#pragma unroll
        for (int v = 0; v < GEN_MAXV; ++v) {
            const int ch = lane + 64 * v;
            if (ch < nchunk) {
                f32x4 o4;
#pragma unroll
                for (int e = 0; e < 4; ++e) o4[e] = rs * (gy[v][e] - s1 - xh[v][e] * s2);
                if (dres) o4 += *reinterpret_cast<const f32x4*>(dres + row * C + 4 * ch);
                *reinterpret_cast<f32x4*>(dx + row * C + 4 * ch) = o4;
                if (dx16) *reinterpret_cast<bf16x4*>(dx16 + row * C + 4 * ch) = __builtin_convertvector(o4, bf16x4);
            }
        }
    }
#pragma unroll
    for (int v = 0; v < GEN_MAXV; ++v) {
        const int ch = lane + 64 * v;
        if (ch < nchunk) {
#pragma unroll
            for (int e = 0; e < 4; ++e) {
                red[wib * 2 * C + 4 * ch + e] = dg[v][e];
                red[wib * 2 * C + C + 4 * ch + e] = db[v][e];
            }
        }
    }
    __syncthreads();
    for (int c = threadIdx.x; c < 2 * C; c += 256)
        partial[(long)blockIdx.x * 2 * C + c] = red[c] + red[2 * C + c] + red[4 * C + c] + red[6 * C + c];
}

int ln_grid(int M, int rpb) { return min(cdiv(M, rpb), 512); }

template <int LPR, int VPL>
void launch_fwd(const float* x, const float* g, const float* b, float* y, float* mean, float* rstd, int M, float eps,
                int y_bf16, hipStream_t st) {
    hipLaunchKernelGGL((ln_fwd_kernel<LPR, VPL>), dim3(ln_grid(M, 256 / LPR)), dim3(256), 0, st, x, g, b, y, mean, rstd, M, eps, y_bf16);
}
template <int LPR, int VPL>
void launch_bwd(const float* dy, const float* x, const float* mean, const float* rstd, const float* g,
                const float* dres, float* dx, float* partial, int M, __bf16* dx16, hipStream_t st) {
    hipLaunchKernelGGL((ln_bwd_kernel<LPR, VPL>), dim3(ln_grid(M, 256 / LPR)), dim3(256), 0, st, dy, x, mean, rstd, g, dres, dx, partial, M, dx16);
}

bool ln_fast(int C) { return C == 64 || C == 128 || C == 256 || C == 512 || C == 32 || C == 1024; }
bool ln_supported(int C) { return C > 0 && C % 4 == 0 && C <= 256 * GEN_MAXV; }

}

extern "C" {

int cswin_layernorm_fwd(const float* x, const float* gamma, const float* beta, float* y, float* mean, float* rstd,
                        int M, int C, float eps, int y_bf16, void* stream) {
    CSWIN_REQUIRE(x && gamma && beta && y && mean && rstd && M > 0, CSWIN_ERR_SHAPE, "layernorm_fwd: bad arguments");
    y_bf16 = y_bf16 != 0;
    CSWIN_REQUIRE(ln_supported(C), CSWIN_ERR_UNSUPPORTED, "layernorm: C=%d must be a multiple of 4, at most 1024", C);
    hipStream_t st = (hipStream_t)stream;
    if (!ln_fast(C)) {
        hipLaunchKernelGGL(ln_fwd_generic_kernel, dim3(ln_grid(M, 4)), dim3(256), 0, st, x, gamma, beta, y, mean, rstd, M, C, eps, y_bf16);
        CSWIN_LAUNCH_CHECK();
        return CSWIN_OK;
    }
    switch (C) {
        case 32: launch_fwd<8, 1>(x, gamma, beta, y, mean, rstd, M, eps, y_bf16, st); break;
        case 64: launch_fwd<16, 1>(x, gamma, beta, y, mean, rstd, M, eps, y_bf16, st); break;
        case 128: launch_fwd<32, 1>(x, gamma, beta, y, mean, rstd, M, eps, y_bf16, st); break;
        case 256: launch_fwd<64, 1>(x, gamma, beta, y, mean, rstd, M, eps, y_bf16, st); break;
        case 512: launch_fwd<64, 2>(x, gamma, beta, y, mean, rstd, M, eps, y_bf16, st); break;
        case 1024: launch_fwd<64, 4>(x, gamma, beta, y, mean, rstd, M, eps, y_bf16, st); break;
    }
    CSWIN_LAUNCH_CHECK();
    return CSWIN_OK;
}

size_t cswin_layernorm_bwd_workspace(int M, int C) {
    if (!ln_fast(C)) return (size_t)ln_grid(M, 4) * 2 * C * sizeof(float);
    int lpr = C / 4 > 64 ? 64 : C / 4;
    return (size_t)ln_grid(M, 256 / lpr) * 2 * C * sizeof(float);
}

int cswin_layernorm_bwd(const float* dy, const float* x, const float* mean, const float* rstd, const float* gamma,
                        const float* dres, float* dx, float* dgamma, float* dbeta, void* workspace, size_t ws_bytes,
                        int M, int C, cswin_reduce_job* deferred, void* dx_bf16, void* stream) {
    __bf16* dx16 = (__bf16*)dx_bf16;
    CSWIN_REQUIRE(dy && x && mean && rstd && gamma && dx && dgamma && dbeta && M > 0, CSWIN_ERR_SHAPE, "layernorm_bwd: bad arguments");
    CSWIN_REQUIRE(ln_supported(C), CSWIN_ERR_UNSUPPORTED, "layernorm: C=%d must be a multiple of 4, at most 1024", C);
    CSWIN_REQUIRE(workspace && ws_bytes >= cswin_layernorm_bwd_workspace(M, C), CSWIN_ERR_WORKSPACE, "layernorm_bwd: workspace too small");
    hipStream_t st = (hipStream_t)stream;
    float* partial = (float*)workspace;
    int lpr = C / 4 > 64 ? 64 : C / 4;
    int nblk = ln_fast(C) ? ln_grid(M, 256 / lpr) : ln_grid(M, 4);
    if (!ln_fast(C))
        hipLaunchKernelGGL(ln_bwd_generic_kernel, dim3(nblk), dim3(256), (size_t)8 * C * sizeof(float), st, dy, x, mean, rstd, gamma, dres, dx, partial, M, C, dx16);
    else switch (C) {
        case 32: launch_bwd<8, 1>(dy, x, mean, rstd, gamma, dres, dx, partial, M, dx16, st); break;
        case 64: launch_bwd<16, 1>(dy, x, mean, rstd, gamma, dres, dx, partial, M, dx16, st); break;
        case 128: launch_bwd<32, 1>(dy, x, mean, rstd, gamma, dres, dx, partial, M, dx16, st); break;
        case 256: launch_bwd<64, 1>(dy, x, mean, rstd, gamma, dres, dx, partial, M, dx16, st); break;
        case 512: launch_bwd<64, 2>(dy, x, mean, rstd, gamma, dres, dx, partial, M, dx16, st); break;
        case 1024: launch_bwd<64, 4>(dy, x, mean, rstd, gamma, dres, dx, partial, M, dx16, st); break;
    }
    CSWIN_LAUNCH_CHECK();
    cswin_reduce_job job = {partial, dgamma, dbeta, C, 2LL * C, 2LL * C, nblk, 0};
    reduce_now_or_defer(job, deferred, st);
    CSWIN_LAUNCH_CHECK();
    return CSWIN_OK;
}

}
```

cswin_unet_amd/networks/cswin_unet.py:

```python
import math

import numpy as np
import torch
import torch.nn as nn
import torch.utils.checkpoint as checkpoint

from .. import ops
from ..layers import DropPath, TokenRearrange, trunc_normal_


def _square_side(n_tokens):
    side = int(math.isqrt(n_tokens))
    if side * side != n_tokens:
        raise ValueError(f"token count {n_tokens} is not a square map")
    return side


class Mlp(nn.Module):
    def __init__(self, in_features, hidden_features=None, out_features=None, act_layer=nn.GELU, drop=0.):
        super().__init__()
        out_features = out_features or in_features
        hidden_features = hidden_features or in_features
        self.fc1 = nn.Linear(in_features, hidden_features)
        self.act = act_layer()
        self.fc2 = nn.Linear(hidden_features, out_features)
        self.drop = nn.Dropout(drop)
        if not isinstance(self.act, nn.GELU) or getattr(self.act, "approximate", "none") != "none":
            raise NotImplementedError("the HIP Mlp kernel fuses the exact (erf) GELU only")

    def forward(self, x, residual=None, row_scale=None):
        p = self.drop.p if self.training else 0.0
        return ops.mlp(x, self.fc1.weight, self.fc1.bias, self.fc2.weight, self.fc2.bias, residual, row_scale, drop_p=p)


class LePEAttention(nn.Module):

    def __init__(self, dim, resolution, idx, split_size, dim_out=None, num_heads=9, attn_drop=0., proj_drop=0.,
                 qk_scale=None):
        super().__init__()
        if idx not in (-1, 0, 1):
            raise ValueError(f"ERROR MODE {idx}")
        self.dim, self.dim_out = dim, dim_out or dim
        self.resolution, self.split_size, self.num_heads, self.idx = resolution, split_size, num_heads, idx
        self.scale = qk_scale or (dim // num_heads) ** -0.5
        self.H_sp = resolution if idx in (-1, 0) else split_size
        self.W_sp = resolution if idx in (-1, 1) else split_size
        self.get_v = nn.Conv2d(dim, dim, kernel_size=3, stride=1, padding=1, groups=dim)
        self.attn_drop = nn.Dropout(attn_drop)

    def forward(self, qkv):
        q, k, v = qkv[0], qkv[1], qkv[2]
        if q.shape[1] != self.resolution * self.resolution:
            raise AssertionError("flatten img_tokens has wrong size")
        packed = torch.cat([q, k, v], dim=-1)
        return ops.stripe_attention(packed, self.resolution, self.split_size, [self.idx], [self.num_heads],
                                    [self.get_v.weight], [self.get_v.bias], self.scale,
                                    attn_drop=self.attn_drop.p if self.training else 0.0)


class CSWinBlock(nn.Module):
    def __init__(self, dim, reso, num_heads, split_size, mlp_ratio=4., qkv_bias=False, qk_scale=None, drop=0.,
                 attn_drop=0., drop_path=0., act_layer=nn.GELU, norm_layer=nn.LayerNorm, last_stage=False):
        super().__init__()
        self.dim, self.num_heads, self.patches_resolution = dim, num_heads, reso
        self.split_size, self.mlp_ratio = split_size, mlp_ratio
        self.qkv = nn.Linear(dim, dim * 3, bias=qkv_bias)
        self.norm1 = norm_layer(dim)
        single = last_stage or reso == split_size
        self.branch_num = 1 if single else 2
        self.proj = nn.Linear(dim, dim)
        self.proj_drop = nn.Dropout(drop)
        bdim, bheads = (dim, num_heads) if single else (dim // 2, num_heads // 2)
        self.attns = nn.ModuleList(
            LePEAttention(bdim, resolution=reso, idx=(-1 if single else i), split_size=split_size, num_heads=bheads,
                          dim_out=bdim, qk_scale=qk_scale, attn_drop=attn_drop, proj_drop=drop)
            for i in range(self.branch_num))
        self.drop_path = DropPath(drop_path) if drop_path > 0. else nn.Identity()
        self.mlp = Mlp(in_features=dim, hidden_features=int(dim * mlp_ratio), out_features=dim, act_layer=act_layer,
                       drop=drop)
        self.norm2 = norm_layer(dim)

    def _keep_scales(self, x):
        dp = self.drop_path
        if isinstance(dp, DropPath) and self.training and dp.drop_prob > 0.:
            preset = getattr(self, "_dp_preset", None)
            if preset:
                return preset[0], preset[1]
            return dp.sample_scale(x.shape[0], x.device), dp.sample_scale(x.shape[0], x.device)
        return None, None

    def forward(self, x):
        B, L, C = x.shape
        if L != self.patches_resolution ** 2:
            raise AssertionError("flatten img_tokens has wrong size")
        a = self.attns
        ad = a[0].attn_drop.p if self.training else 0.0
        if type(self.norm1) is not nn.LayerNorm or type(self.norm2) is not nn.LayerNorm:
            raise NotImplementedError("the HIP block fuses nn.LayerNorm only")
        rs1, rs2 = self._keep_scales(x)
        if self.training and (self.proj_drop.p > 0 or self.mlp.drop.p > 0):
            n1, n2 = self.norm1, self.norm2
            qkv = ops.linear(ops.layer_norm(x, n1.weight, n1.bias, n1.eps), self.qkv.weight, self.qkv.bias)
            att = ops.stripe_attention(qkv, self.patches_resolution, self.split_size, [m.idx for m in a], [m.num_heads for m in a],
                                       [m.get_v.weight for m in a], [m.get_v.bias for m in a], a[0].scale, attn_drop=ad)
            x = ops.dropout(ops.linear(att, self.proj.weight, self.proj.bias), self.proj_drop.p, residual=x, row_scale=rs1)
            return self.mlp(ops.layer_norm(x, n2.weight, n2.bias, n2.eps), residual=x, row_scale=rs2)
        return ops.cswin_block(x, self.patches_resolution, self.split_size, [m.idx for m in a], [m.num_heads for m in a],
                               a[0].scale, self.norm1, self.qkv, self.proj, self.norm2, self.mlp.fc1, self.mlp.fc2,
                               [m.get_v.weight for m in a], [m.get_v.bias for m in a], rs1, rs2, attn_drop=ad)


def img2windows(img, H_sp, W_sp):
    return ops.img2windows(img, H_sp, W_sp)


def windows2img(img_splits_hw, H_sp, W_sp, H, W):
    return ops.windows2img(img_splits_hw, H_sp, W_sp, H, W)


class Merge_Block(nn.Module):
    def __init__(self, dim, dim_out, norm_layer=nn.LayerNorm):
        super().__init__()
        self.conv = nn.Conv2d(dim, dim_out, 3, 2, 1)
        self.norm = norm_layer(dim_out)

    def forward(self, x):
        side = _square_side(x.shape[1])
        y = ops.conv_tokens(x, self.conv.weight, self.conv.bias, side, side, 2, 1)
        return ops.layer_norm(y, self.norm.weight, self.norm.bias, self.norm.eps)


class _CarafeBase(nn.Module):
    def __init__(self, dim, dim_out, kernel_size, up_factor):
        super().__init__()
        if kernel_size != 3:
            raise NotImplementedError("the HIP reassembly kernel is written for the 3x3 neighbourhood the reference uses")
        self.kernel_size, self.up_factor = kernel_size, up_factor
        self.down = nn.Conv2d(dim, dim // 4, 1)
        self.encoder = nn.Conv2d(dim // 4, up_factor ** 2 * kernel_size ** 2, kernel_size, 1, kernel_size // 2)
        self.out = nn.Conv2d(dim, dim_out, 1)

    def kernel_logits(self, x, side):
        mid = ops.linear(x, self.down.weight.flatten(1), self.down.bias)
        return ops.conv_tokens(mid, self.encoder.weight, self.encoder.bias, side, side, 1, 1)

    def forward(self, x):
        side = _square_side(x.shape[1])
        mid, z = ops.linear_pair(x, self.down.weight.flatten(1), self.down.bias, self.out.weight.flatten(1), None)
        e = ops.conv_tokens(mid, self.encoder.weight, self.encoder.bias, side, side, 1, 1)
        return ops.carafe_reassemble(e, z, self.out.bias, side, side, self.up_factor)


class CARAFE(_CarafeBase):
    def __init__(self, dim, dim_out, kernel_size=3, up_factor=2):
        super().__init__(dim, dim_out, kernel_size, up_factor)


class CARAFE4(_CarafeBase):
    def __init__(self, dim, dim_out, kernel_size=3, up_factor=4):
        super().__init__(dim, dim_out, kernel_size, up_factor)


class _SumInputChannels(torch.autograd.Function):

    @staticmethod
    def forward(ctx, w):
        ctx.cin = w.shape[1]
        return w.sum(1, keepdim=True)

    @staticmethod
    def backward(ctx, g):
        return g.repeat(1, ctx.cin, 1, 1)


class _PatchEmbed(nn.Sequential):

    def conv_weight(self, img):
        w = self[0].weight
        if img.shape[1] == 1 and w.shape[1] > 1:
            w = _SumInputChannels.apply(w)
        return w

    def forward(self, img, w=None):
        conv, norm = self[0], self[2]
        if w is None:
            w = self.conv_weight(img)
        tok = ops.patch_embed_conv(img, w, conv.bias, conv.stride[0], conv.padding[0])
        return ops.layer_norm(tok, norm.weight, norm.bias, norm.eps)


class CSWinTransformer(nn.Module):

    def __init__(self, img_size=224, patch_size=16, in_chans=3, num_classes=8, embed_dim=64, depth=[1, 2, 9, 1],
                 split_size=[1, 2, 7, 7], num_heads=12, mlp_ratio=4., qkv_bias=True, qk_scale=None, drop_rate=0.,
                 attn_drop_rate=0., drop_path_rate=0, hybrid_backbone=None, norm_layer=nn.LayerNorm, use_chk=False):
        super().__init__()
        self.use_chk, self.num_classes = use_chk, num_classes
        self.num_features = self.embed_dim = embed_dim
        heads = num_heads
        E = embed_dim
        self.img_size = img_size

        self.stage1_conv_embed = _PatchEmbed(nn.Conv2d(in_chans, E, 7, 4, 2), TokenRearrange(), nn.LayerNorm(E))
        self.pos_drop = nn.Dropout(p=drop_rate)

        rates = torch.linspace(0, drop_path_rate, int(np.sum(depth))).tolist()
        first = np.concatenate([[0], np.cumsum(depth)]).astype(int)

        def make_stage(si, last=False):
            return nn.ModuleList(
                CSWinBlock(dim=E << si, num_heads=heads[si], reso=img_size // (4 << si), mlp_ratio=mlp_ratio,
                           qkv_bias=qkv_bias, qk_scale=qk_scale, split_size=split_size[si], drop=drop_rate,
                           attn_drop=attn_drop_rate, drop_path=rates[first[si] + i], norm_layer=norm_layer,
                           last_stage=last)
                for i in range(depth[si]))

        self.stage1 = make_stage(0)
        self.merge1 = Merge_Block(E, 2 * E)
        self.stage2 = make_stage(1)
        self.merge2 = Merge_Block(2 * E, 4 * E)
        self.stage3 = make_stage(2)
        self.merge3 = Merge_Block(4 * E, 8 * E)
        self.stage4 = make_stage(3, last=True)
        self.norm = norm_layer(8 * E)
        self.stage_up4 = make_stage(3, last=True)
        self.upsample4 = CARAFE(8 * E, 4 * E)
        self.concat_linear4 = nn.Linear(8 * E, 4 * E)
        self.stage_up3 = make_stage(2)
        self.upsample3 = CARAFE(4 * E, 2 * E)
        self.concat_linear3 = nn.Linear(4 * E, 2 * E)
        self.stage_up2 = make_stage(1)
        self.upsample2 = CARAFE(2 * E, E)
        self.concat_linear2 = nn.Linear(2 * E, E)
        self.stage_up1 = make_stage(0)
        self.upsample1 = CARAFE4(E, E)
        self.norm_up = norm_layer(E)
        self.output = nn.Conv2d(in_channels=E, out_channels=self.num_classes, kernel_size=1, bias=False)

        self.apply(self._init_weights)

    def _init_weights(self, m):
        if isinstance(m, nn.Linear):
            trunc_normal_(m.weight, std=.02)
            if m.bias is not None:
                nn.init.constant_(m.bias, 0)
        elif isinstance(m, (nn.LayerNorm, nn.BatchNorm2d)):
            nn.init.constant_(m.bias, 0)
            nn.init.constant_(m.weight, 1.0)

    @torch.jit.ignore
    def no_weight_decay(self):
        return {'pos_embed', 'cls_token'}

    @torch.jit.ignore
    def no_weight_decay_keywords(self):
        return {'relative_position_bias_table'}

    def _run(self, blocks, x):
        for blk in blocks:
            x = checkpoint.checkpoint(blk, x, use_reentrant=False) if self.use_chk else blk(x)
        return x

    def _predraw_drop_path(self, batch, device):
        blocks = [b for st in (self.stage1, self.stage2, self.stage3, self.stage4, self.stage_up4, self.stage_up3,
                               self.stage_up2, self.stage_up1) for b in st]
        live = [b for b in blocks if isinstance(b.drop_path, DropPath) and b.drop_path.drop_prob > 0.]
        for b in blocks:
            b._dp_preset = None
        if not (self.training and live):
            return
        cache = getattr(self, "_dp_keep", None)
        if cache is None or cache.device != device or cache.shape[0] != 2 * len(live):
            cache = torch.tensor([1.0 - b.drop_path.drop_prob for b in live for _ in (0, 1)], dtype=torch.float32,
                                 device=device)[:, None]
            self._dp_keep = cache
        keep = cache
        scales = (torch.rand(keep.shape[0], batch, device=device) < keep).to(torch.float32) / keep
        for i, b in enumerate(live):
            b._dp_preset = [scales[2 * i], scales[2 * i + 1]]

    def forward_features(self, x, pe_weight=None):
        self._predraw_drop_path(x.shape[0], x.device)
        ops.clear_twins()
        x = self.stage1_conv_embed(x, pe_weight)
        if self.pos_drop.p > 0 and self.training:
            x = ops.dropout(x, self.pos_drop.p)
        x = self._run(self.stage1, x)
        self.x1 = x
        x = self._run(self.stage2, self.merge1(x))
        self.x2 = x
        self.enc_mid_in = None
        if getattr(self, "detach_decoder_inputs", False) and torch.is_grad_enabled():
            x = x.detach().requires_grad_()
            self.enc_mid_in = x
        x = self._run(self.stage3, self.merge2(x))
        self.x3 = x
        x = self._run(self.stage4, self.merge3(x))
        return ops.layer_norm(x, self.norm.weight, self.norm.bias, self.norm.eps)

    def forward_up_features(self, x):
        _, s1, s2, s3 = getattr(self, "dec_in", None) or (None, self.x1, self.x2, self.x3)
        for blocks, up, cl, skip in ((self.stage_up4, self.upsample4, self.concat_linear4, s3),
                                    (self.stage_up3, self.upsample3, self.concat_linear3, s2),
                                    (self.stage_up2, self.upsample2, self.concat_linear2, s1)):
            x = up(self._run(blocks, x))
            x = ops.linear(skip, cl.weight, cl.bias, x2=x)
        x = self._run(self.stage_up1, x)
        return ops.layer_norm(x, self.norm_up.weight, self.norm_up.bias, self.norm_up.eps)

    def up_x4(self, x):
        up, head = self.upsample1, self.output
        side = _square_side(x.shape[1])
        ncls = head.out_channels
        cpad = max(16, 1 << (ncls - 1).bit_length())
        w_fused, b_fused = ops.head_compose(head.weight, up.out.weight, up.out.bias, cpad)
        mid, z = ops.linear_pair(x, up.down.weight.flatten(1), up.down.bias, w_fused, None)
        e = ops.conv_tokens(mid, up.encoder.weight, up.encoder.bias, side, side, 1, 1)
        return ops.carafe_reassemble_nchw(e, z, b_fused, side, side, up.up_factor, ncls)

    def _conv_specs(self, pe_weight):
        pe = self.stage1_conv_embed[0]
        specs = [(pe_weight, (pe_weight.shape[1] + 3) // 4 * 4, pe.stride[0], pe.padding[0])]
        specs += [(m.conv.weight, m.conv.weight.shape[1], 2, 1) for m in (self.merge1, self.merge2, self.merge3)]
        specs += [(u.encoder.weight, u.encoder.weight.shape[1], 1, 1)
                  for u in (self.upsample4, self.upsample3, self.upsample2, self.upsample1)]
        return specs

    def forward(self, x):
        pe_weight = self.stage1_conv_embed.conv_weight(x)
        with ops.conv_weight_images(self._conv_specs(pe_weight)):
            return self._forward(x, pe_weight)

    def _forward(self, x, pe_weight):
        x = self.forward_features(x, pe_weight)
        self.xb = x
        bound = [x, self.x1, self.x2, self.x3]
        if getattr(self, "detach_decoder_inputs", False) and torch.is_grad_enabled():
            bound = [t.detach().requires_grad_() for t in bound]
        self.dec_in = bound
        x = self.forward_up_features(bound[0])
        return self.up_x4(x)
```

cswin_unet_amd/ops.py:

```python
import ctypes
import math

import numpy as np
import torch
from torch.autograd import Function
from torch.autograd.function import once_differentiable

from ._lib import AugmentDesc, ConvImageJob, CswinHipError, ReduceJob, WgradDesc, act_bf16, call, dev_f32, lib, precision, ptr, shadow_ptr, stream

__all__ = ["layer_norm", "linear", "linear_pair", "mlp", "stripe_attention", "cswin_block", "conv_tokens", "patch_embed_conv", "carafe_reassemble",
           "carafe_reassemble_nchw", "conv_weight_images", "head_compose", "tokens_to_nchw", "matmul_nn", "ce_dice_loss", "continual_loss", "dropout", "img2windows", "windows2img",
           "seg_metrics", "resize_slices", "argmax_zoom_back", "augment_batch", "class_counts"]


MAX_REDUCE_JOBS = 48
TAIL_RIDER_JOBS = 16


class engine_backward:

    def __init__(self, opt=None):
        self._flat = opt.flat_grad if opt is not None else None
        self._slots = {p.data_ptr(): (o, p.numel()) for p, o in zip(opt.params, opt.offsets)} if opt is not None else {}
        self._queue = []
        self._given = set()

    def __enter__(self):
        global _pass
        self._outer, _pass = _pass, self
        return self

    def __exit__(self, *exc):
        global _pass
        _pass = self._outer
        if exc[0] is None:
            self.flush()
        return False

    def grad(self, param_key, shape, device):
        if param_key is None:
            return None
        n = math.prod(shape)
        o, numel = self._slots.get(param_key, (0, -1)) if param_key else (0, -1)
        if numel != n:
            return torch.empty(tuple(shape), dtype=torch.float32, device=device)
        if o in self._given:
            raise CswinHipError(f"engine_backward: two ops of one backward pass use the leaf parameter at offset {o} of flat_grad; "
                                f"the first gradient is already placed there and its reduction may still be waiting")
        self._given.add(o)
        return self._flat[o:o + n].view(shape)

    def _in_flat(self, address):
        return self._flat is not None and 0 <= address - self._flat.data_ptr() < 4 * self._flat.numel()

    def reduce(self, jobs, reads):
        now = []
        for j in jobs:
            if j.part and all(self._in_flat(a) for a in (j.out, j.out2) if a):
                self._queue.append((ReduceJob.from_buffer_copy(j), reads))
            elif j.part:
                now.append(j)
        if now:
            _rows_sum((ReduceJob * len(now))(*now))

    def queued_outputs(self):
        return [a for j, _ in self._queue for a in (j.out, j.out2) if a]

    def take_pending(self, maxn=TAIL_RIDER_JOBS):
        taken, self._queue = self._queue[:maxn], self._queue[maxn:]
        arr = (ReduceJob * len(taken))(*[j for j, _ in taken])
        return (_job_ptr(arr) if taken else None), len(taken), (arr, taken)

    def flush(self):
        while self._queue:
            _rows_sum(self.take_pending(MAX_REDUCE_JOBS)[2][0])


_pass = engine_backward()


def _param_keys(*ts):
    return tuple(None if t is None else t.data_ptr() if t.is_leaf else 0 for t in ts)


def _job_ptr(jobs, i=0):
    return ctypes.c_void_p(ctypes.addressof(jobs) + i * ctypes.sizeof(ReduceJob))


def _rows_sum(jobs):
    call("cswin_rows_sum_multi", _job_ptr(jobs), len(jobs), stream())


def _ws(nbytes, device):
    return torch.empty(max(int(nbytes), 16) // 4 + 4, dtype=torch.float32, device=device)


def _reduced(nbytes, device, launch, njobs=1):
    ws, jobs = _ws(nbytes, device), (ReduceJob * njobs)()
    launch(ptr(ws), nbytes, _job_ptr(jobs))
    _pass.reduce(jobs, (ws,))


def _int_array(vals):
    return (ctypes.c_int * len(vals))(*vals)


def _ptr_array(tensors):
    return (ctypes.c_void_p * len(tensors))(*[t.data_ptr() for t in tensors])


def _stored16(*ts):
    return sum(1 << i for i, t in enumerate(ts) if t is not None and t.dtype == torch.bfloat16)


def _rows_per_sample(t):
    return t.numel() // (t.shape[0] * t.shape[-1])


def _layernorm_fwd(x, gamma, beta, eps, dtype=torch.float32):
    C = x.shape[-1]
    M = x.numel() // C
    y = torch.empty_like(x, dtype=dtype)
    mean = torch.empty(M, dtype=torch.float32, device=x.device)
    rstd = torch.empty_like(mean)
    call("cswin_layernorm_fwd", ptr(x), ptr(gamma), ptr(beta), ptr(y), ptr(mean), ptr(rstd), M, C, eps, _stored16(y), stream())
    return y, mean, rstd


def _layernorm_bwd(dy, x, mean, rstd, gamma, dx, dg, db, slab=None, *, dres=None, dx16=None):
    C = x.shape[-1]
    M = x.numel() // C
    if slab is None:
        return _reduced(lib().cswin_layernorm_bwd_workspace(M, C), x.device,
                        lambda *s: _layernorm_bwd(dy, x, mean, rstd, gamma, dx, dg, db, s, dres=dres, dx16=dx16))
    ws, nbytes, job = slab
    call("cswin_layernorm_bwd", ptr(dy), ptr(x), ptr(mean), ptr(rstd), ptr(gamma), ptr(dres), ptr(dx), ptr(dg), ptr(db), ws, nbytes,
         M, C, job, ptr(dx16), stream())


class _LayerNorm(Function):
    @staticmethod
    def forward(ctx, x, gamma, beta, eps):
        x, gamma, beta = dev_f32(x, "layer_norm input"), dev_f32(gamma), dev_f32(beta)
        y, mean, rstd = _layernorm_fwd(x, gamma, beta, eps)
        ctx.save_for_backward(x, gamma, mean, rstd)
        ctx.keys = _param_keys(gamma, beta)
        return y

    @staticmethod
    @once_differentiable
    def backward(ctx, dy):
        x, gamma, mean, rstd = ctx.saved_tensors
        dx = torch.empty_like(x)
        dg, db = (_pass.grad(k, gamma.shape, gamma.device) for k in ctx.keys)
        _layernorm_bwd(dev_f32(dy), x, mean, rstd, gamma, dx, dg, db)
        return dx, dg, db, None


def layer_norm(x, gamma, beta, eps=1e-5):
    return _LayerNorm.apply(x, gamma, beta, eps)


_twins = {}


def _twin_put(t, t16):
    _twins[t.data_ptr()] = (t, t16)


def _twin_take(t):
    e = _twins.pop(t.data_ptr(), None)
    return e[1] if e is not None and e[0]._cdata == t._cdata else None


def clear_twins():
    _twins.clear()


def _wsrc(w):
    if act_bf16() and w.shape[0] % 4 == 0 and w.shape[1] % 4 == 0:
        sp = shadow_ptr(w)
        if sp is not None:
            return sp, 4
    return ptr(w), 0


def _linear_fwd(x, w, b, N, *, dtype=torch.float32, gelu=False, x2=None, residual=None, row_scale=None):
    pw, w16 = w if isinstance(w, tuple) else (ptr(w), 0)
    K1 = x.shape[-1]
    K = K1 + (x2.shape[-1] if x2 is not None else 0)
    y = torch.empty(x.shape[:-1] + (N,), dtype=dtype, device=x.device)
    y_act = torch.empty_like(y) if gelu else None
    call("cswin_linear_fwd", ptr(x), ptr(x2), K1 if x2 is not None else 0, pw, ptr(b), ptr(y), ptr(y_act), ptr(residual), ptr(row_scale),
         _rows_per_sample(x), x.numel() // K1, N, K, precision(), _stored16(x, y) | w16, stream())
    return (y, y_act) if gelu else y


def _linear_bwd_data(dy, w, dx, *, dx2=None, gelu_pre=None, row_scale=None, add=None):
    pw, w16 = w if isinstance(w, tuple) else (ptr(w), 0)
    N, K1 = dy.shape[-1], dx.shape[-1]
    K = K1 + (dx2.shape[-1] if dx2 is not None else 0)
    call("cswin_linear_bwd_data", ptr(dy), pw, ptr(dx), ptr(dx2), K1 if dx2 is not None else 0, ptr(gelu_pre), ptr(row_scale),
         _rows_per_sample(dy), ptr(add), dy.numel() // N, N, K, precision(), _stored16(dy, dx, None, gelu_pre) | w16, stream())


def _linear_bwd_weight(dy, x, dw, db, slab=None, *, x2=None, row_scale=None):
    N, K1 = dy.shape[-1], x.shape[-1]
    K = K1 + (x2.shape[-1] if x2 is not None else 0)
    M = dy.numel() // N
    if slab is None:
        return _reduced(lib().cswin_linear_bwd_weight_workspace(M, N, K), dy.device,
                        lambda *s: _linear_bwd_weight(dy, x, dw, db, s, x2=x2, row_scale=row_scale))
    ws, nbytes, job = slab
    call("cswin_linear_bwd_weight", ptr(dy), ptr(x), ptr(x2), K1 if x2 is not None else 0, ptr(row_scale), _rows_per_sample(dy),
         ptr(dw), ptr(db), ws, nbytes, M, N, K, job, precision(), stream())


MAX_MASK_SAMPLES = 256


def _fill_wgrad(d, dy, x, row_scale, dw, dbias, workspace, ws_bytes):
    d.dy, d.x, d.row_scale, d.dw, d.dbias = (t.data_ptr() if t is not None else None for t in (dy, x, row_scale, dw, dbias))
    d.workspace, d.ws_bytes, d.rows_per_sample = workspace, ws_bytes, _rows_per_sample(dy)
    d.N, d.K = dy.shape[-1], x.shape[-1]
    d.M, d.precision, d.io_bf16 = dy.numel() // d.N, precision(), _stored16(dy, x)


def _linear_bwd_weight_batch(wg, jobs, pending=(None, 0)):
    call("cswin_linear_bwd_weight_batch", ctypes.cast(wg, ctypes.c_void_p), len(wg), _job_ptr(jobs), *pending, stream())


class _Linear(Function):
    @staticmethod
    def forward(ctx, x, w, b, x2, residual, row_scale):
        x, w = dev_f32(x, "linear input"), dev_f32(w, "linear weight")
        b, x2, residual, row_scale = dev_f32(b), dev_f32(x2), dev_f32(residual), dev_f32(row_scale)
        K = x.shape[-1] + (x2.shape[-1] if x2 is not None else 0)
        assert w.shape[1] == K, f"linear: weight {tuple(w.shape)} vs input features {K}"
        y = _linear_fwd(x, _wsrc(w), b, w.shape[0], x2=x2, residual=residual, row_scale=row_scale)
        ctx.save_for_backward(x, w, x2, row_scale)
        ctx.has_res, ctx.keys = residual is not None, _param_keys(w, b)
        return y

    @staticmethod
    @once_differentiable
    def backward(ctx, dy):
        x, w, x2, row_scale = ctx.saved_tensors
        dy = dev_f32(dy)
        need = ctx.needs_input_grad
        dx = dx2 = dw = db = None
        if need[0] or (x2 is not None and need[3]):
            dx = torch.empty_like(x)
            dx2 = torch.empty_like(x2) if x2 is not None else None
            _linear_bwd_data(dy, _wsrc(w), dx, dx2=dx2, row_scale=row_scale)
        if need[1]:
            dw = _pass.grad(ctx.keys[0], w.shape, w.device)
            db = _pass.grad(ctx.keys[1], w.shape[:1], w.device)
            _linear_bwd_weight(dy, x, dw, db, x2=x2, row_scale=row_scale)
        return dx, dw, db, dx2, (dy if ctx.has_res else None), None


def linear(x, w, b=None, x2=None, residual=None, row_scale=None):
    return _Linear.apply(x, w, b, x2, residual, row_scale)


class _LinearPair(Function):

    @staticmethod
    def forward(ctx, x, w1, b1, w2, b2):
        x, w1, b1, w2, b2 = (dev_f32(t) for t in (x, w1, b1, w2, b2))
        assert w1.shape[1] == w2.shape[1] == x.shape[-1]
        ctx.save_for_backward(x, w1, w2)
        ctx.keys = _param_keys(w1, b1, w2, b2)
        return tuple(_linear_fwd(x, w, b, w.shape[0]) for w, b in ((w1, b1), (w2, b2)))

    @staticmethod
    @once_differentiable
    def backward(ctx, dy1, dy2):
        x, w1, w2 = ctx.saved_tensors
        dy1, dy2 = dev_f32(dy1), dev_f32(dy2)
        K = x.shape[-1]
        M = x.numel() // K
        dx = None
        if ctx.needs_input_grad[0]:
            dx = torch.empty_like(x)
            _linear_bwd_data(dy1, w1, dx)
            _linear_bwd_data(dy2, w2, dx, add=dx)
        grads, keep = [], []
        wg, jobs = (WgradDesc * 2)(), (ReduceJob * 2)()
        for i, (dy, w) in enumerate(((dy1, w1), (dy2, w2))):
            dw = _pass.grad(ctx.keys[2 * i], w.shape, w.device)
            db = _pass.grad(ctx.keys[2 * i + 1], w.shape[:1], w.device)
            nbytes = lib().cswin_linear_bwd_weight_workspace(M, w.shape[0], K)
            keep.append(_ws(nbytes, w.device))
            _fill_wgrad(wg[i], dy, x, None, dw, db, ptr(keep[-1]), nbytes)
            grads += [dw, db]
        _linear_bwd_weight_batch(wg, jobs)
        _pass.reduce(jobs, keep)
        return (dx,) + tuple(grads)


def linear_pair(x, w1, b1, w2, b2):
    return _LinearPair.apply(x, w1, b1, w2, b2)


_epoch = {}


def dropout_epoch(device):
    t = _epoch.get(device)
    if t is None:
        t = _epoch[device] = torch.zeros(1, dtype=torch.int64, device=device)
    return t


def advance_dropout_epoch(device):
    dropout_epoch(device).add_(1)


def _draw_seeds(n):
    return tuple(int(v) for v in torch.randint(0, 2 ** 62, (n,)).tolist())


def _dropout(x, y, p, seed, *, residual=None, row_scale=None):
    call("cswin_dropout", ptr(x), ptr(residual), ptr(row_scale), ptr(y), x.numel(), x.numel() // x.shape[0], float(p), int(seed),
         ptr(dropout_epoch(x.device)), stream())


class _Mlp(Function):

    @staticmethod
    def forward(ctx, x, w1, b1, w2, b2, residual, row_scale, drop_p, seeds):
        x, w1, b1, w2, b2 = (dev_f32(t) for t in (x, w1, b1, w2, b2))
        residual, row_scale = dev_f32(residual), dev_f32(row_scale)
        s1, s2 = _wsrc(w1), _wsrc(w2)
        pre, act = _linear_fwd(x, s1, b1, w1.shape[0], gelu=True)
        if drop_p > 0:
            _dropout(act, act, drop_p, seeds[0])
            y = _linear_fwd(act, s2, b2, w2.shape[0])
            _dropout(y, y, drop_p, seeds[1], residual=residual, row_scale=row_scale)
        else:
            y = _linear_fwd(act, s2, b2, w2.shape[0], residual=residual, row_scale=row_scale)
        ctx.save_for_backward(x, w1, w2, pre, act, row_scale)
        ctx.has_res, ctx.keys = residual is not None, _param_keys(w1, b1, w2, b2)
        ctx.drop = (float(drop_p), seeds)
        return y

    @staticmethod
    @once_differentiable
    def backward(ctx, dy):
        x, w1, w2, pre, act, row_scale = ctx.saved_tensors
        dy = dev_f32(dy)
        K = x.shape[-1]
        Hd, N = w1.shape[0], w2.shape[0]
        M = x.numel() // K
        dev = x.device
        drop_p, seeds = ctx.drop
        dyl, rs_gemm = dy, row_scale
        if drop_p > 0:
            dyl = torch.empty_like(dy)
            _dropout(dy, dyl, drop_p, seeds[1], row_scale=row_scale)
            rs_gemm = None
        dpre = torch.empty_like(pre)
        _linear_bwd_data(dyl, w2, dpre, gelu_pre=pre, row_scale=rs_gemm)
        if drop_p > 0:
            _dropout(dpre, dpre, drop_p, seeds[0])
        dx = None
        if ctx.needs_input_grad[0]:
            dx = torch.empty_like(x)
            _linear_bwd_data(dpre, w1, dx)
        k1, kb1, k2, kb2 = ctx.keys
        dw2, db2 = _pass.grad(k2, w2.shape, dev), _pass.grad(kb2, (N,), dev)
        nbytes = max(lib().cswin_linear_bwd_weight_workspace(M, N, Hd), lib().cswin_linear_bwd_weight_workspace(M, Hd, K))
        ws, ws1 = _ws(nbytes, dev), _ws(nbytes, dev)
        jobs = (ReduceJob * 2)()
        _linear_bwd_weight(dyl, act, dw2, db2, (ptr(ws), nbytes, _job_ptr(jobs, 0)), row_scale=rs_gemm)
        dw1, db1 = _pass.grad(k1, w1.shape, dev), _pass.grad(kb1, (Hd,), dev)
        _linear_bwd_weight(dpre, x, dw1, db1, (ptr(ws1), nbytes, _job_ptr(jobs, 1)))
        _pass.reduce(jobs, (ws, ws1))
        return dx, dw1, db1, dw2, db2, (dy if ctx.has_res else None), None, None, None


def mlp(x, w1, b1, w2, b2, residual=None, row_scale=None, drop_p=0.0):
    return _Mlp.apply(x, w1, b1, w2, b2, residual, row_scale, float(drop_p), _draw_seeds(2) if drop_p > 0 else (0, 0))


class _MatmulNN(Function):

    @staticmethod
    def forward(ctx, a, b):
        a, b = dev_f32(a), dev_f32(b)
        c = torch.empty(a.shape[0], b.shape[1], dtype=torch.float32, device=a.device)
        _linear_bwd_data(a, b, c)
        ctx.save_for_backward(a, b)
        return c

    @staticmethod
    @once_differentiable
    def backward(ctx, dc):
        a, b = ctx.saved_tensors
        dc = dev_f32(dc)
        da = _linear_fwd(dc, b, None, a.shape[1])
        db = torch.empty_like(b)
        _linear_bwd_weight(a, dc, db, None)
        return da, db


def matmul_nn(a, b):
    return _MatmulNN.apply(a, b)


ATTN_FP32, ATTN_QKV16, ATTN_IO16, ATTN_MFMA16 = 0, 1, 3, 7


def _attn_drop_args(drop, device):
    return drop[0], drop[1], ptr(dropout_epoch(device)) if drop[0] > 0 else None


def _attn_fwd(qkv, lw, lb, y, y0, lse, reso, split, idx, heads, scale, drop, mode):
    B, _, C3 = qkv.shape
    call("cswin_attn_fwd", ptr(qkv), _ptr_array(lw), _ptr_array(lb), ptr(y), ptr(y0), ptr(lse), B, reso, C3 // 3, len(idx),
         _int_array(heads), _int_array(idx), split, float(scale or 0.0), *_attn_drop_args(drop, qkv.device), mode, stream())


def _attn_bwd(qkv, lw, lb, lse, y0, dy, dqkv, dlw, dlb, reso, split, idx, heads, scale, drop, mode, slab=None):
    B, _, C3 = qkv.shape
    ha, ia = _int_array(heads), _int_array(idx)
    if slab is None:
        nbytes = lib().cswin_attn_bwd_workspace(B, reso, C3 // 3, len(idx), ha, ia, split)
        again = lambda *s: _attn_bwd(qkv, lw, lb, lse, y0, dy, dqkv, dlw, dlb, reso, split, idx, heads, scale, drop, mode, s)
        return _reduced(nbytes, qkv.device, again, njobs=2)
    ws, nbytes, jobs = slab
    call("cswin_attn_bwd", ptr(qkv), _ptr_array(lw), _ptr_array(lb), ptr(lse), ptr(y0), ptr(dy), ptr(dqkv), _ptr_array(dlw),
         _ptr_array(dlb), ws, nbytes, B, reso, C3 // 3, len(idx), ha, ia, split, float(scale or 0.0), jobs,
         *_attn_drop_args(drop, qkv.device), mode, stream())


class _StripeAttention(Function):
    @staticmethod
    def forward(ctx, qkv, reso, split, idx, heads, scale, drop, *wb):
        q16 = qkv.dtype == torch.bfloat16 and qkv.is_cuda
        qkv = qkv.contiguous() if q16 else dev_f32(qkv, "attention qkv")
        nb = len(idx)
        ws_ = [dev_f32(t).view(t.shape[0], 9) for t in wb[:nb]]
        bs_ = [dev_f32(t) for t in wb[nb:]]
        B, L, C3 = qkv.shape
        if L != reso * reso:
            raise ValueError("flatten img_tokens has wrong size")
        y = torch.empty(B, L, C3 // 3, dtype=torch.float32, device=qkv.device)
        y0 = torch.empty_like(y) if any(ctx.needs_input_grad) else None
        lse = torch.empty(B, sum(heads), L, dtype=torch.float32, device=qkv.device)
        ctx.meta = (reso, split, tuple(idx), tuple(heads), scale, drop, ATTN_QKV16 if q16 else ATTN_FP32)
        _attn_fwd(qkv, ws_, bs_, y, y0, lse, *ctx.meta)
        ctx.save_for_backward(qkv, lse, y0, *ws_, *bs_)
        ctx.keys = _param_keys(*wb)
        return y

    @staticmethod
    @once_differentiable
    def backward(ctx, dy):
        qkv, lse, y0, *wb_ = ctx.saved_tensors
        nb = len(wb_) // 2
        ws_, bs_ = wb_[:nb], wb_[nb:]
        dqkv = torch.empty_like(qkv)
        dws = [_pass.grad(k, t.shape, t.device) for k, t in zip(ctx.keys[:nb], ws_)]
        dbs = [_pass.grad(k, t.shape, t.device) for k, t in zip(ctx.keys[nb:], bs_)]
        _attn_bwd(qkv, ws_, bs_, lse, y0, dev_f32(dy), dqkv, dws, dbs, *ctx.meta)
        return (dqkv, None, None, None, None, None, None) + tuple(d.view(d.shape[0], 1, 3, 3) for d in dws) + tuple(dbs)


def _attn_drop(p):
    p = float(p)
    return (p, _draw_seeds(1)[0]) if p > 0 else (0.0, 0)


def stripe_attention(qkv, reso, split, idx, heads, lepe_w, lepe_b, scale=None, attn_drop=0.0):
    return _StripeAttention.apply(qkv, reso, split, tuple(idx), tuple(heads), scale, _attn_drop(attn_drop), *lepe_w, *lepe_b)


class _CSWinBlock(Function):

    @staticmethod
    def forward(ctx, x, reso, split, idx, heads, scale, eps1, eps2, rs1, rs2, drop, g1, b1, wqkv, bqkv, wp, bp, g2, b2, w1, bb1,
                w2, bb2, *lepe):
        x = dev_f32(x, "block input")
        B, L, C = x.shape
        if L != reso * reso:
            raise ValueError("flatten img_tokens has wrong size")
        dev = x.device
        nb = len(idx)
        lw = [dev_f32(t).view(t.shape[0], 9) for t in lepe[:nb]]
        lb = [dev_f32(t) for t in lepe[nb:]]
        rs1, rs2 = dev_f32(rs1), dev_f32(rs2)
        s16 = act_bf16() and C % 4 == 0
        t16 = torch.bfloat16 if s16 else torch.float32
        E16 = lambda *shape: torch.empty(*shape, dtype=t16, device=dev)
        sq, sp, s1, s2 = (_wsrc(w) if s16 else w for w in (wqkv, wp, w1, w2))
        attn = (reso, split, tuple(idx), tuple(heads), scale, drop, ATTN_MFMA16 if s16 else ATTN_FP32)
        h1, m1, r1 = _layernorm_fwd(x, g1, b1, eps1, t16)
        qkv = _linear_fwd(h1, sq, bqkv, 3 * C, dtype=t16)
        att, lse = E16(B, L, C), torch.empty(B, sum(heads), L, dtype=torch.float32, device=dev)
        att0 = E16(B, L, C) if any(ctx.needs_input_grad) else None
        _attn_fwd(qkv, lw, lb, att, att0, lse, *attn)
        x1 = _linear_fwd(att, sp, bp, C, residual=x, row_scale=rs1)
        h2, m2, r2 = _layernorm_fwd(x1, g2, b2, eps2, t16)
        pre, act = _linear_fwd(h2, s1, bb1, w1.shape[0], dtype=t16, gelu=True)
        y = _linear_fwd(act, s2, bb2, C, residual=x1, row_scale=rs2)
        ctx.save_for_backward(x, m1, r1, h1, qkv, lse, att, att0, x1, m2, r2, h2, pre, act, rs1, rs2, g1, wqkv, wp, g2, w1, w2, *lw, *lb)
        ctx.attn = attn
        ctx.keys = _param_keys(g1, b1, wqkv, bqkv, wp, bp, g2, b2, w1, bb1, w2, bb2, *lepe)
        return y

    @staticmethod
    @once_differentiable
    def backward(ctx, dy):
        (x, m1, r1, h1, qkv, lse, att, att0, x1, m2, r2, h2, pre, act, rs1, rs2, g1, wqkv, wp, g2, w1, w2, *lwb) = ctx.saved_tensors
        nb = len(lwb) // 2
        lw, lb = lwb[:nb], lwb[nb:]
        dy = dev_f32(dy)
        B, L, C = x.shape
        M, Hd = B * L, w1.shape[0]
        dev, h = x.device, lib()
        s16 = h1.dtype == torch.bfloat16
        wq, lq = h.cswin_linear_bwd_weight_workspace, h.cswin_layernorm_bwd_workspace
        sizes = [wq(M, C, Hd), wq(M, Hd, C), lq(M, C), wq(M, C, C), wq(M, 3 * C, C), lq(M, C)]
        sizes = [(n + 255) // 256 * 256 for n in sizes]
        ws = _ws(sum(sizes), dev)
        wsp = [ctypes.c_void_p(ws.data_ptr() + sum(sizes[:i])) for i in range(6)]
        jobs = (ReduceJob * 8)()
        sq, sp, s1, s2 = (_wsrc(w) if s16 else w for w in (wqkv, wp, w1, w2))
        dy16 = _twin_take(dy) if s16 else None
        dyg = dy16 if dy16 is not None else dy
        dpre = torch.empty_like(pre)
        _linear_bwd_data(dyg, s2, dpre, gelu_pre=pre, row_scale=rs2)
        wg = (WgradDesc * 4)()
        kg1, kb1, kwqkv, kbqkv, kwp, kbp, kg2, kb2, kw1, kbb1, kw2, kbb2, *klepe = ctx.keys
        G = lambda key, *shape: _pass.grad(key, shape, dev)
        dw2, db2 = G(kw2, *w2.shape), G(kbb2, C)
        _fill_wgrad(wg[0], dyg, act, rs2, dw2, db2, wsp[0], sizes[0])
        dw1, db1 = G(kw1, *w1.shape), G(kbb1, Hd)
        _fill_wgrad(wg[1], dpre, h2, None, dw1, db1, wsp[1], sizes[1])
        dh2 = torch.empty_like(x)
        _linear_bwd_data(dpre, s1, dh2)
        dx1, dg2, dbt2 = torch.empty_like(x), G(kg2, C), G(kb2, C)
        dx1_16 = torch.empty_like(x, dtype=torch.bfloat16) if s16 else None
        _layernorm_bwd(dh2, x1, m2, r2, g2, dx1, dg2, dbt2, (wsp[2], sizes[2], _job_ptr(jobs, 2)), dres=dy, dx16=dx1_16)
        dx1g = dx1_16 if s16 else dx1
        datt = dh2
        _linear_bwd_data(dx1g, sp, datt, row_scale=rs1)
        dwp, dbp = G(kwp, *wp.shape), G(kbp, C)
        _fill_wgrad(wg[2], dx1g, att, rs1, dwp, dbp, wsp[3], sizes[3])
        dqkv = torch.empty_like(qkv)
        dlw = [G(k, *t.shape) for k, t in zip(klepe[:nb], lw)]
        dlb = [G(k, *t.shape) for k, t in zip(klepe[nb:], lb)]
        reso, split, idx, heads = ctx.attn[:4]
        naw = h.cswin_attn_bwd_workspace(B, reso, C, nb, _int_array(heads), _int_array(idx), split)
        aws = _ws(naw, dev)
        _attn_bwd(qkv, lw, lb, lse, att0, datt, dqkv, dlw, dlb, *ctx.attn, (ptr(aws), naw, _job_ptr(jobs, 6)))
        dwqkv, dbqkv = G(kwqkv, *wqkv.shape), G(kbqkv, 3 * C)
        _fill_wgrad(wg[3], dqkv, h1, None, dwqkv, dbqkv, wsp[4], sizes[4])
        wjobs = (ReduceJob * 4)()
        dh1 = datt
        pend, npend, riders = _pass.take_pending()
        if precision() == 0:
            tail = (ptr(dqkv), ptr(wqkv), ptr(dh1), M, 3 * C, C, ctypes.cast(wg, ctypes.c_void_p), 4, _job_ptr(wjobs), pend, npend)
            masks = (rs2, rs2, rs1, rs1) if B <= MAX_MASK_SAMPLES else (None,) * 4
            if any(m is not None for m in masks):
                skip = (ctypes.c_void_p * 4)(*[m.data_ptr() if m is not None else None for m in masks])
                call("cswin_linear_bwd_tail_masked", *tail, skip, _int_array([B] * 4), stream())
            else:
                call("cswin_linear_bwd_tail", *tail, stream())
        else:
            _linear_bwd_weight_batch(wg, wjobs, (pend, npend))
            _linear_bwd_data(dqkv, sq, dh1)
        for slot, ji in enumerate((0, 1, 3, 4)):
            jobs[ji] = wjobs[slot]
        dx, dg1, dbt1 = torch.empty_like(x), G(kg1, C), G(kb1, C)
        dx16 = torch.empty_like(x, dtype=torch.bfloat16) if s16 else None
        _layernorm_bwd(dh1, x, m1, r1, g1, dx, dg1, dbt1, (wsp[5], sizes[5], _job_ptr(jobs, 5)), dres=dx1, dx16=dx16)
        if s16:
            _twin_put(dx, dx16)
        _pass.reduce(jobs, (ws, aws))
        grads = (dx, None, None, None, None, None, None, None, None, None, None, dg1, dbt1, dwqkv, dbqkv, dwp, dbp, dg2, dbt2, dw1, db1,
                 dw2, db2)
        return grads + tuple(d.view(d.shape[0], 1, 3, 3) for d in dlw) + tuple(dlb)


def cswin_block(x, reso, split, idx, heads, scale, norm1, qkv, proj, norm2, fc1, fc2, lepe_w, lepe_b, rs1=None, rs2=None, attn_drop=0.0):
    return _CSWinBlock.apply(x, reso, split, tuple(idx), tuple(heads), scale, norm1.eps, norm2.eps, rs1, rs2, _attn_drop(attn_drop),
                             norm1.weight, norm1.bias, qkv.weight, qkv.bias, proj.weight, proj.bias, norm2.weight,
                             norm2.bias, fc1.weight, fc1.bias, fc2.weight, fc2.bias, *lepe_w, *lepe_b)


MAX_CONV_IMAGE_JOBS = 16
_conv_images = {}


def _same_conv(w, stride, pad):
    return stride == 1 and 2 * pad == w.shape[2] - 1 and w.shape[0] % 4 == 0


class conv_weight_images:

    def __init__(self, specs):
        self._specs = [sp for sp in specs if sp[0] is not None and sp[0].is_cuda and sp[0].dtype == torch.float32 and sp[0].is_contiguous()]

    def __enter__(self):
        global _conv_images
        self._outer = _conv_images
        images, jobs = {}, []
        grad = torch.is_grad_enabled()
        for w, cpad, stride, pad in self._specs[:MAX_CONV_IMAGE_JOBS]:
            Cout, Cin, ks, _ = w.shape
            E = lambda *shape: torch.empty(*shape, dtype=torch.float32, device=w.device)
            same = _same_conv(w, stride, pad)
            need_dx = grad and cpad == Cin
            wp = E(Cout, ks * ks, cpad)
            wpt = E(ks * ks, Cout, cpad) if need_dx and not same else None
            wf = E(Cin, ks * ks, Cout) if need_dx and same else None
            images[w.data_ptr()] = (w, cpad, wp, wpt, wf)
            jobs.append(ConvImageJob(w.data_ptr(), wp.data_ptr(), wpt.data_ptr() if wpt is not None else None,
                                     wf.data_ptr() if wf is not None else None, Cout, Cin, ks, cpad))
        if jobs:
            arr = (ConvImageJob * len(jobs))(*jobs)
            call("cswin_conv_weight_images", ctypes.cast(arr, ctypes.c_void_p), len(jobs), stream())
        _conv_images = images
        return self

    def __exit__(self, *exc):
        global _conv_images
        _conv_images = self._outer
        return False


def _images_of(w, cpad):
    e = _conv_images.get(w.data_ptr())
    if e is not None and e[0].shape == w.shape and e[1] == cpad:
        return e[2:]
    return None


def _permute_w(w, cpad, want_t):
    Cout, Cin, ks, _ = w.shape
    wp = torch.empty(Cout, ks * ks, cpad, dtype=torch.float32, device=w.device)
    wpt = torch.empty(ks * ks, Cout, cpad, dtype=torch.float32, device=w.device) if want_t else None
    call("cswin_conv_weight_permute", ptr(w), ptr(wp), ptr(wpt), Cout, Cin, ks, cpad, stream())
    return wp, wpt


def _conv_tok_fwd(x, w_img, b, y, H, W, ks, stride, pad):
    call("cswin_conv_tok_fwd", ptr(x), ptr(w_img), ptr(b), ptr(y), x.shape[0], H, W, x.shape[-1], y.shape[-1], ks, stride, pad,
         precision(), stream())


class _ConvTokens(Function):
    @staticmethod
    def forward(ctx, x, w, b, H, W, stride, pad):
        x, w, b = dev_f32(x, "conv input"), dev_f32(w), dev_f32(b)
        B, L, Cin = x.shape
        assert L == H * W and w.shape[1] == Cin
        Cout, ks = w.shape[0], w.shape[2]
        OH, OW = (H + 2 * pad - ks) // stride + 1, (W + 2 * pad - ks) // stride + 1
        need_dx = ctx.needs_input_grad[0]
        same = _same_conv(w, stride, pad)
        img = _images_of(w, Cin)
        wf = None
        if img is not None and (img[1] is not None or same or not need_dx):
            wp, wpt, wf = img
        else:
            wp, wpt = _permute_w(w, Cin, need_dx and not same)
        y = torch.empty(B, OH * OW, Cout, dtype=torch.float32, device=x.device)
        _conv_tok_fwd(x, wp, b, y, H, W, ks, stride, pad)
        ctx.save_for_backward(x, w, wpt, wf if need_dx else None)
        ctx.meta = (H, W, stride, pad)
        ctx.keys = _param_keys(w, b)
        return y

    @staticmethod
    @once_differentiable
    def backward(ctx, dy):
        x, w, wpt, wf = ctx.saved_tensors
        H, W, stride, pad = ctx.meta
        dy = dev_f32(dy)
        B, L, Cin = x.shape
        Cout, ks = w.shape[0], w.shape[2]
        dx = None
        if ctx.needs_input_grad[0]:
            dx = torch.empty_like(x)
            if _same_conv(w, stride, pad):
                if wf is None:
                    wf = torch.empty(Cin, ks * ks, Cout, dtype=torch.float32, device=x.device)
                    call("cswin_conv_weight_flipT", ptr(w), ptr(wf), Cout, Cin, ks, stream())
                _conv_tok_fwd(dy, wf, None, dx, H, W, ks, 1, pad)
            else:
                if wpt is None:
                    _, wpt = _permute_w(w, Cin, True)
                call("cswin_conv_tok_bwd_data", ptr(dy), ptr(wpt), ptr(dx), B, H, W, Cin, Cout, ks, stride, pad, precision(), stream())
        dw = _pass.grad(ctx.keys[0], w.shape, x.device)
        db = _pass.grad(ctx.keys[1], (Cout,), x.device)
        _reduced(lib().cswin_conv_tok_bwd_weight_workspace(B, H, W, Cin, Cout, ks, stride, pad), x.device,
                 lambda ws, nbytes, job: call("cswin_conv_tok_bwd_weight", ptr(dy), ptr(x), ptr(dw), ptr(db), ws, nbytes, B, H, W, Cin,
                                              Cout, ks, stride, pad, 1, job, precision(), stream()))
        return dx, dw, db, None, None, None, None


def conv_tokens(x, w, b, H, W, stride, pad):
    return _ConvTokens.apply(x, w, b, H, W, stride, pad)


class _PatchEmbedConv(Function):

    @staticmethod
    def forward(ctx, img, w, b, stride, pad):
        img, w, b = dev_f32(img, "image"), dev_f32(w), dev_f32(b)
        B, Cin, H, W = img.shape
        Cout, ks = w.shape[0], w.shape[2]
        cpad = (Cin + 3) // 4 * 4
        st = stream()
        x = torch.empty(B, H * W, cpad, dtype=torch.float32, device=img.device)
        call("cswin_nchw_to_tokens", ptr(img), ptr(x), B, Cin, H, W, cpad, st)
        images = _images_of(w, cpad)
        wp = images[0] if images is not None else _permute_w(w, cpad, False)[0]
        OH, OW = (H + 2 * pad - ks) // stride + 1, (W + 2 * pad - ks) // stride + 1
        y = torch.empty(B, OH * OW, Cout, dtype=torch.float32, device=img.device)
        _conv_tok_fwd(x, wp, b, y, H, W, ks, stride, pad)
        ctx.save_for_backward(x, w)
        ctx.meta = (H, W, stride, pad)
        ctx.keys = _param_keys(w, b)
        return y

    @staticmethod
    @once_differentiable
    def backward(ctx, dy):
        x, w = ctx.saved_tensors
        H, W, stride, pad = ctx.meta
        dy = dev_f32(dy)
        B, cpad = x.shape[0], x.shape[-1]
        Cout, Cin, ks, _ = w.shape
        dw = _pass.grad(ctx.keys[0], w.shape, x.device)
        db = _pass.grad(ctx.keys[1], (Cout,), x.device)
        _reduced(lib().cswin_conv_tok_bwd_weight_workspace(B, H, W, cpad, Cout, ks, stride, pad), x.device,
                 lambda ws, nbytes, job: call("cswin_conv_tok_bwd_weight_cpad", ptr(dy), ptr(x), ptr(dw), ptr(db), ws, nbytes, B, H, W,
                                              cpad, Cin, Cout, ks, stride, pad, job, precision(), stream()))
# ... 459 lines not shown
```

include/cswin_hip.h:

```cpp
#ifndef CSWIN_HIP_H
#define CSWIN_HIP_H

#include <stddef.h>

#ifdef __cplusplus
extern "C" {
#endif

#define CSWIN_ABI_VERSION 4

#define CSWIN_OK 0
#define CSWIN_ERR_SHAPE (-1)
#define CSWIN_ERR_ALIGN (-2)
#define CSWIN_ERR_WORKSPACE (-3)
#define CSWIN_ERR_HIP (-4)
#define CSWIN_ERR_UNSUPPORTED (-5)

typedef struct cswin_reduce_job {
    const float* part;
    float* out;
    float* out2;
    long long n_first, n, stride;
    int rows, reserved;
    int conv_kk, conv_cin;
} cswin_reduce_job;

const char* cswin_last_error(void);
int cswin_abi_version(void);
int cswin_device_ok(void);

int cswin_attn_fwd(const float* qkv, const float* const* lepe_w, const float* const* lepe_b, float* y, float* y0, float* lse,
                   int B, int reso, int C, int nbranch, const int* heads, const int* idx, int split, float scale,
                   float drop_p, unsigned long long drop_seed, const unsigned long long* drop_epoch, int qkv_bf16, void* stream);
size_t cswin_attn_bwd_workspace(int B, int reso, int C, int nbranch, const int* heads, const int* idx, int split);
int cswin_attn_bwd(const float* qkv, const float* const* lepe_w, const float* const* lepe_b, const float* lse,
                   const float* y0, const float* dy, float* dqkv, float* const* dlepe_w, float* const* dlepe_b,
                   void* workspace, size_t ws_bytes, int B, int reso, int C, int nbranch, const int* heads, const int* idx,
                   int split, float scale, cswin_reduce_job* deferred, float drop_p, unsigned long long drop_seed,
                   const unsigned long long* drop_epoch, int qkv_bf16, void* stream);

int cswin_img2windows(const float* img, float* out, int B, int C, int H, int W, int H_sp, int W_sp, void* stream);
int cswin_windows2img(const float* win, float* out, int B, int C, int H, int W, int H_sp, int W_sp, void* stream);

int cswin_layernorm_fwd(const float* x, const float* gamma, const float* beta, float* y, float* mean, float* rstd,
                        int M, int C, float eps, int y_bf16, void* stream);
size_t cswin_layernorm_bwd_workspace(int M, int C);
int cswin_layernorm_bwd(const float* dy, const float* x, const float* mean, const float* rstd, const float* gamma,
                        const float* dres, float* dx, float* dgamma, float* dbeta, void* workspace, size_t ws_bytes,
                        int M, int C, cswin_reduce_job* deferred, void* dx_bf16, void* stream);

int cswin_linear_fwd(const float* x, const float* x2, int k_split, const float* w, const float* bias, float* y,
                     float* y_act, const float* residual, const float* row_scale, int rows_per_sample, int M, int N,
                     int K, int precision, int io_bf16, void* stream);
int cswin_linear_bwd_data(const float* dy, const float* w, float* dx, float* dx2, int k_split, const float* gelu_pre,
                          const float* row_scale, int rows_per_sample, const float* add, int M, int N, int K,
                          int precision, int io_bf16, void* stream);
size_t cswin_linear_bwd_weight_workspace(int M, int N, int K);
int cswin_linear_bwd_weight(const float* dy, const float* x, const float* x2, int k_split, const float* row_scale,
                            int rows_per_sample, float* dw, float* dbias, void* workspace, size_t ws_bytes, int M,
                            int N, int K, cswin_reduce_job* deferred, int precision, void* stream);
typedef struct cswin_wgrad_desc {
    const float* dy;
    const float* x;
    const float* row_scale;
    float* dw;
    float* dbias;
    void* workspace;
    size_t ws_bytes;
    int rows_per_sample, M, N, K;
    int precision;
    int io_bf16;
} cswin_wgrad_desc;
int cswin_linear_bwd_weight_batch(const cswin_wgrad_desc* problems, int n, cswin_reduce_job* deferred, const cswin_reduce_job* pending,
                                  int npending, void* stream);
int cswin_linear_bwd_tail(const float* dy, const float* w, float* dx, int M, int N, int K, const cswin_wgrad_desc* problems, int n,
                          cswin_reduce_job* deferred, const cswin_reduce_job* pending, int npending, void* stream);
int cswin_linear_bwd_weight_batch_masked(const cswin_wgrad_desc* problems, int n, cswin_reduce_job* deferred,
                                         const cswin_reduce_job* pending, int npending, const float* const* skip, const int* nsamples,
                                         void* stream);
int cswin_linear_bwd_tail_masked(const float* dy, const float* w, float* dx, int M, int N, int K, const cswin_wgrad_desc* problems, int n,
                                 cswin_reduce_job* deferred, const cswin_reduce_job* pending, int npending, const float* const* skip,
                                 const int* nsamples, void* stream);
int cswin_rows_sum_multi(const cswin_reduce_job* jobs, int njobs, void* stream);

int cswin_conv_tok_fwd(const float* x, const float* w_perm, const float* bias, float* y, int B, int H, int W, int Cin,
                       int Cout, int ks, int stride, int pad, int precision, void* stream);
int cswin_conv_tok_bwd_data(const float* dy, const float* w_permT, float* dx, int B, int H, int W, int Cin, int Cout,
                            int ks, int stride, int pad, int precision, void* stream);
size_t cswin_conv_tok_bwd_weight_workspace(int B, int H, int W, int Cin, int Cout, int ks, int stride, int pad);
int cswin_conv_tok_bwd_weight(const float* dy, const float* x, float* dw, float* dbias, void* workspace,
                              size_t ws_bytes, int B, int H, int W, int Cin, int Cout, int ks, int stride, int pad,
                              int torch_layout, cswin_reduce_job* deferred, int precision, void* stream);
int cswin_conv_weight_permute(const float* w, float* w_perm, float* w_permT, int Cout, int Cin, int ks, int Cpad,
                              void* stream);
int cswin_conv_weight_unpermute(const float* dw_perm, float* dw, int Cout, int Cin, int ks, int Cpad, void* stream);
int cswin_conv_weight_flipT(const float* w, float* wf, int Cout, int Cin, int ks, void* stream);
typedef struct cswin_conv_image_job {
    const float* w;
    float* w_perm;
    float* w_permT;
    float* w_flipT;
    int Cout, Cin, ks, Cpad;
} cswin_conv_image_job;
int cswin_conv_weight_images(const cswin_conv_image_job* jobs, int njobs, void* stream);
int cswin_conv_tok_bwd_weight_cpad(const float* dy, const float* x, float* dw, float* dbias, void* workspace, size_t ws_bytes,
                                   int B, int H, int W, int Cin, int Cin_param, int Cout, int ks, int stride, int pad,
                                   cswin_reduce_job* deferred, int precision, void* stream);

int cswin_nchw_to_tokens(const float* x, float* y, int B, int C, int H, int W, int Cpad, void* stream);
int cswin_tokens_to_nchw(const float* x, float* y, int B, int C, int H, int W, int Cpad, void* stream);

int cswin_carafe_fwd(const float* e, const float* z, const float* bias, float* out, float* wt_save, int B, int H,
                     int W, int Cz, int S, void* stream);
size_t cswin_carafe_bwd_workspace(int B, int H, int W, int Cz, int S);
int cswin_carafe_bwd(const float* dout, const float* z, const float* wt_save, float* de, float* dz, float* dbias,
                     void* workspace, size_t ws_bytes, int B, int H, int W, int Cz, int S, cswin_reduce_job* deferred, void* stream);
int cswin_carafe_fwd_nchw(const float* e, const float* z, const float* bias, float* out, float* wt_save, int B, int H, int W,
                          int Cz, int C, int S, void* stream);
int cswin_carafe_bwd_nchw_ok(int H, int W, int Cz, int S);
int cswin_carafe_bwd_nchw(const float* dout, const float* z, const float* wt_save, float* de, float* dz, float* dbias,
                          void* workspace, size_t ws_bytes, int B, int H, int W, int Cz, int C, int S, cswin_reduce_job* deferred,
                          void* stream);

int cswin_head_compose(const float* w_head, const float* w_out, const float* b_out, float* w_fused, float* b_fused, int ncls,
                       int E, int C, int Cpad, void* stream);
int cswin_head_compose_bwd(const float* w_head, const float* w_out, const float* b_out, const float* dw_fused,
                           const float* db_fused, float* dw_head, float* dw_out, float* db_out, int ncls, int E, int C,
                           void* stream);

size_t cswin_loss_workspace(int B, int ncls, long HW);
int cswin_loss_sums(const float* logits, const long long* labels, float* sums, void* workspace, size_t ws_bytes, int B,
                    int ncls, long HW, int inputs_are_probs, void* stream);
int cswin_loss_finalize(const float* sums, float* out3, float* coef, double n_pixels, int ncls, float w_ce,
                        float w_dice, const float* class_weight, void* stream);
int cswin_loss_bwd(const float* logits, const long long* labels, const float* coef, const float* grad_out,
                   float* dlogits, float ce_scale, float dice_scale, int B, int ncls, long HW, int inputs_are_probs,
                   void* stream);

size_t cswin_cl_loss_workspace(int B, int ncls, long HW);
int cswin_cl_loss_sums(const float* logits, const long long* labels, const int* label_map, int n_map, const float* teacher,
                       const float* class_weight, float* sums, void* workspace, size_t ws_bytes, int B, int ncls, int nold,
                       long HW, float temperature, float focal_alpha, float focal_gamma, void* stream);
int cswin_cl_loss_finalize(const float* sums, float* out5, float* coef, double n_pixels, double batch, int ncls, float w_focal,
                           float w_dice, float kd_weight, float temperature, void* stream);
int cswin_cl_loss_bwd(const float* logits, const long long* labels, const int* label_map, int n_map, const float* teacher,
                      const float* class_weight, const float* coef, const float* grad_out, float* dlogits, float focal_scale,
                      float dice_scale, float kd_scale, int B, int ncls, int nold, long HW, float temperature, float focal_alpha,
                      float focal_gamma, void* stream);

int cswin_sgd_flat(float* p, const float* g, float* m, long n, const float* lr_dev, float momentum,
                   float weight_decay, float grad_scale, void* shadow_bf16, void* stream);
int cswin_multi_copy(const void* table, int nchunks, void* stream);


int cswin_chunk_sumsq(const float* g, const float* p, const void* chunks, int nchunks, float* partial, void* stream);
int cswin_norm_finalize(const float* partial, const int* first_chunk, int ntensors, float grad_scale, float max_norm,
                        float* tensor_sumsq, float* scalars, void* stream);
int cswin_adamw_flat(float* p, const float* g, float* m, float* v, const void* chunks, int nchunks, const float* lr_dev,
                     const float* lr_mult, const float* scalars, double beta1, double beta2, double eps, float weight_decay,
                     float grad_scale, double bc1, double bc2, void* shadow_bf16, void* stream);

int cswin_tpgm_chunk_stats(const float* p, const float* anchor, const float* g, const void* chunks, int nchunks, int l1,
                           float* partial, void* stream);
int cswin_tpgm_finalize(const float* partial, const int* first_chunk, int ntensors, int l1, const int* flags, float* gamma,
                        float* gm, float* gv, double grad_scale, double proj_lr, double bc1, double bc2, int mode, float* ratio,
                        float* norm, float* scalars, void* stream);
int cswin_tpgm_project(const float* src, const float* anchor, float* dst, const float* ratio, const void* chunks, int nchunks,
                       void* shadow_bf16, void* stream);

int cswin_dropout(const float* x, const float* residual, const float* row_scale, float* y, long n, long elems_per_sample,
                  float p, unsigned long long seed, const unsigned long long* seed_epoch, void* stream);
int cswin_pack_bf16(const float* src, void* dst_bf16, long n, void* stream);
int cswin_pack_bf16_scaled(const float* src, void* dst_bf16, long n, float scale, void* stream);
int cswin_unpack_bf16(const void* src_bf16, float* dst, long n, void* stream);

int    cswin_seg_metrics_nbins(int D, int H, int W);
size_t cswin_seg_metrics_workspace(int D, int H, int W, int ndim, int ncls);
int    cswin_seg_metrics(const unsigned char* pred, const unsigned char* label, long long* counts, unsigned int* hist,
                         void* workspace, size_t ws_bytes, int D, int H, int W, int ndim, int ncls, void* stream);

int cswin_resize_banded(const void* x, float* y, const double* wh, const int* sh, int Th, const double* ww, const int* sw, int Tw,
                        int D, int H, int W, int h, int w, int x_f64, void* stream);
int cswin_argmax_zoom_back(const float* logits, unsigned char* out, const int* src_row, const int* src_col, int B, int ncls, int h,
                           int w, int H, int W, void* stream);
int cswin_argmax_zoom_back_classes(const float* logits, unsigned char* out, const int* src_row, const int* src_col,
                                   const int* classes, int nsel, int B, int ncls, int h, int w, int H, int W, void* stream);

int cswin_class_counts(const void* labels, int label_bytes, const int* label_map, int nmap, long long* counts, int N,
                       long long slice_elems, int ncls, void* stream);

typedef struct cswin_augment_desc {
    int kind, k, axis;
    int src;
    const int* map;
} cswin_augment_desc;
int cswin_augment_gather(const float* x, float* y, const void* table, int n, int B, int H, int W, int Ho, int Wo, void* stream);
int cswin_augment_labels(const unsigned char* lab, long long* out, const void* table, const int* src_row, const int* src_col,
                         const int* src_row_t, const int* src_col_t, int n, int B, int H, int W, int h, int w, void* stream);

#ifdef __cplusplus
}
#endif
#endif
```

Baseline: 1946 images/sec.

## Fuse paired layernorms and paired linear forward/dgrad into single kernels

Adds a layernorm-pair kernel that computes two consecutive layernorms on the same row in one pass, so a block can take a precomputed norm1, along with its matching fused backward. Also adds a paired linear forward that stacks both weight matrices into one GEMM with a split epilogue and per-half bias, plus a paired data-gradient GEMM that concatenates both dy inputs along K and accumulates in one launch. The aim is fewer launches and fewer passes over activations. The cost is more code paths and extra arguments on the block autograd function.

```diff
diff --git a/cswin_unet_amd/_lib.py b/cswin_unet_amd/_lib.py
--- a/cswin_unet_amd/_lib.py
+++ b/cswin_unet_amd/_lib.py
@@ -23,8 +23,13 @@
     "cswin_layernorm_fwd": (I, [P, P, P, P, P, P, I, I, F, I, P]),
     "cswin_layernorm_bwd_workspace": (SZ, [I, I]),
     "cswin_layernorm_bwd": (I, [P, P, P, P, P, P, P, P, P, P, SZ, I, I, P, P, P]),
+    "cswin_layernorm_pair_fwd": (I, [P, P, P, P, P, P, P, P, P, P, P, I, I, F, F, P]),
+    "cswin_layernorm_pair_bwd_workspace": (SZ, [I, I]),
+    "cswin_layernorm_pair_bwd": (I, [P] * 16 + [SZ, I, I, P, P]),
     "cswin_linear_fwd": (I, [P, P, I, P, P, P, P, P, P, I, I, I, I, I, I, P]),
     "cswin_linear_bwd_data": (I, [P, P, P, P, I, P, P, I, P, I, I, I, I, I, P]),
+    "cswin_linear_pair_fwd": (I, [P, P, P, P, P, P, P, I, I, I, I, I, P]),
+    "cswin_linear_pair_bwd_data": (I, [P, P, P, P, P, I, I, I, I, I, P]),
     "cswin_linear_bwd_weight_workspace": (SZ, [I, I, I]),
     "cswin_linear_bwd_weight": (I, [P, P, P, I, P, I, P, P, P, SZ, I, I, I, P, I, P]),
     "cswin_linear_bwd_weight_batch": (I, [P, I, P, P, I, P]),
diff --git a/cswin_unet_amd/csrc/gemm.hip b/cswin_unet_amd/csrc/gemm.hip
--- a/cswin_unet_amd/csrc/gemm.hip
+++ b/cswin_unet_amd/csrc/gemm.hip
@@ -65,6 +65,38 @@
     __device__ const float* ptr(const Row& r, int j) const {
         if (!r.b0 || j >= cols) return nullptr;
         return j < c0 ? r.b0 + j : r.b1 + (j - c0);
+    }
+};
+
+struct StackSrc {
+    const float* p0; const float* p1; long ld; int rows, cols, n0, s1;
+    struct Row { const float* base; float s; };
+    typedef int Col;
+    __device__ Col col(int j) const { return j; }
+    __device__ Row row(int i) const {
+        Row r;
+        r.base = i < n0 ? p0 + (long)i * ld : (i >= s1 && i < rows ? p1 + (long)(i - s1) * ld : nullptr);
+        r.s = 1.0f;
+        return r;
+    }
+    __device__ const float* ptr(const Row& r, int j) const { return (r.base && j < cols) ? r.base + j : nullptr; }
+};
+struct ConcatGapSrc {
+    const float* p0; const float* p1; long ld0, ld1; int rows, cols, n0, s1;
+    static constexpr bool fast_div = false;
+    struct Row { const float* b0; const float* b1; float s; };
+    typedef int Col;
+    __device__ Col col(int j) const { return j; }
+    __device__ Row row(int i) const {
+        Row r;
+        r.b0 = (i < rows) ? p0 + (long)i * ld0 : nullptr;
+        r.b1 = (i < rows) ? p1 + (long)i * ld1 : nullptr;
+        r.s = 1.0f;
+        return r;
+    }
+    __device__ const float* ptr(const Row& r, int j) const {
+        if (!r.b0 || j >= cols) return nullptr;
+        return j < n0 ? r.b0 + j : (j >= s1 ? r.b1 + (j - s1) : nullptr);
     }
 };
 
@@ -215,10 +247,11 @@
 struct KeptList { int n; int idx[MASK_MAX_SAMPLES]; float scale[MASK_MAX_SAMPLES]; };
 
 template <int BM, int BN, int BK, int KW, bool A_RC, bool B_RC, int VEC, int EPI, bool SCALE_A, int PREC, class ASrc, class BSrc,
-          bool MASKED = false>
+          bool MASKED = false, bool SEG = false>
 __device__ __forceinline__ void gemm_body(float* lds, const ASrc& A, const BSrc& B, const Epilogue& epi, int M, int N, int R,
                                           int r_per_split, int tiles_m, int tiles_n, int bid, int nblk, int stamp_row,
-                                          const RowMask* mk = nullptr, KeptList* kept = nullptr) {
+                                          const RowMask* mk = nullptr, KeptList* kept = nullptr, int seg_r = 0) {
+    static_assert(!SEG || (KW == 1 && PREC == 0 && !MASKED), "the two-range reduction is built for one k-group of fp32 MFMAs");
     constexpr int WGM = BM >= 64 ? 2 : 1, WGN = BN >= 64 ? 2 : 1, NW = WGM * WGN;
     constexpr int WM = BM / WGM, WN = BN / WGN;
     constexpr int FM = WM / 32, FN = WN / 32;
@@ -434,6 +467,7 @@
 #pragma unroll
             for (int e = 0; e < 16; ++e) acc[i][j][e] = 0.f;
 
+    f32x16 first[SEG ? FM : 1][SEG ? FN : 1];
     float csum = 0.f;
     const bool do_colsum = !A_RC && epi.colsum && n0 == 0 && tid < BM;
 
@@ -517,6 +551,18 @@
                         for (int j = 0; j < FN; ++j)
                             acc[i][j] = __builtin_amdgcn_mfma_f32_32x32x2f32(af[i][s], bf[j][s], acc[i][j], 0, 0, 0);
             }
+            if constexpr (SEG) {
+                if (r0 + BK == seg_r) {
+#pragma unroll
+                    for (int i = 0; i < FM; ++i)
+#pragma unroll
+                        for (int j = 0; j < FN; ++j) {
+                            first[i][j] = acc[i][j];
+#pragma unroll
+                            for (int e = 0; e < 16; ++e) acc[i][j][e] = 0.f;
+                        }
+                }
+            }
             __syncthreads();
             if (more) {
                 stash(a16, b16);
@@ -541,6 +587,12 @@
         }
     }
 
+    if constexpr (SEG) {
+#pragma unroll
+        for (int i = 0; i < FM; ++i)
+#pragma unroll
+            for (int j = 0; j < FN; ++j) acc[i][j] += first[i][j];
+    }
     if (epi.stamps && tid == 0) epi.stamps[8L * stamp_row + 2] = __builtin_amdgcn_s_memtime();
     if (KW > 1) {
         static_assert(KW == 1 || (KW / 2) * NW * FM * FN * 16 * 64 <= LDS_FLOATS, "LDS too small for the k-group reduction");
@@ -593,6 +645,14 @@
     __shared__ __attribute__((aligned(16))) float lds[gemm_lds_floats<BM, BN, BK, KW, A_RC, B_RC>()];
     gemm_body<BM, BN, BK, KW, A_RC, B_RC, VEC, EPI, SCALE_A, PREC, ASrc, BSrc>(lds, A, B, epi, M, N, R, r_per_split, tiles_m, tiles_n,
                                                                               (int)blockIdx.x, (int)gridDim.x, (int)blockIdx.x);
+}
+
+template <int BN>
+__global__ __launch_bounds__(gemm_threads(64, BN, 1)) void gemm_pair_dgrad_kernel(ConcatGapSrc A, StackSrc B, Epilogue epi, int M, int N,
+                                                                                  int R, int seg_r, int tiles_m, int tiles_n) {
+    __shared__ __attribute__((aligned(16))) float lds[gemm_lds_floats<64, BN, 32, 1, true, false>()];
+    gemm_body<64, BN, 32, 1, true, false, 4, EPI_PLAIN, false, 0, ConcatGapSrc, StackSrc, false, true>(
+        lds, A, B, epi, M, N, R, R, tiles_m, tiles_n, (int)blockIdx.x, (int)gridDim.x, (int)blockIdx.x, nullptr, nullptr, seg_r);
 }
 
 constexpr int WGRAD_BATCH = 4;
@@ -1121,6 +1181,56 @@
     return CSWIN_OK;
 }
 
+static bool pair_one_launch(const void* a, const void* b, const void* c, const void* d, const void* e, int N1, int N2, int K, int precision) {
+    return precision == 0 && N1 % 4 == 0 && N2 % 4 == 0 && K % 4 == 0 && aligned16(a) && aligned16(b) && aligned16(c) && aligned16(d) && aligned16(e);
+}
+
+int cswin_linear_pair_fwd(const float* x, const float* w1, const float* b1, const float* w2, const float* b2, float* y1, float* y2,
+                          int M, int N1, int N2, int K, int precision, void* stream) {
+    CSWIN_CHECK_PRECISION(precision, "linear_pair_fwd");
+    CSWIN_REQUIRE(x && w1 && w2 && y1 && y2 && M > 0 && N1 > 0 && N2 > 0 && K > 0, CSWIN_ERR_SHAPE, "linear_pair_fwd: bad arguments");
+    if (!pair_one_launch(x, w1, w2, y1, y2, N1, N2, K, precision) || (b1 && !aligned16(b1)) || (b2 && !aligned16(b2))) {
+        int rc = cswin_linear_fwd(x, nullptr, 0, w1, b1, y1, nullptr, nullptr, nullptr, 1, M, N1, K, precision, 0, stream);
+        if (rc) return rc;
+        return cswin_linear_fwd(x, nullptr, 0, w2, b2, y2, nullptr, nullptr, nullptr, 1, M, N2, K, precision, 0, stream);
+    }
+    const int N = N1 + N2;
+    Epilogue e = plain_epilogue(y1, N1);
+    e.C2 = y2; e.ldc2 = N2; e.col_split = N1;
+    e.bias = b1; e.bias2 = b2;
+    PlainSrc A = {x, K, M, K, nullptr, 1, 0};
+    StackSrc B = {w1, w2, K, N, K, N1, N1};
+    launch_gemm<true, true, 4, EPI_SPLIT2, false>(A, B, e, M, N, K, 1, one_split(K), 0, (hipStream_t)stream);
+    CSWIN_LAUNCH_CHECK();
+    return CSWIN_OK;
+}
+
+int cswin_linear_pair_bwd_data(const float* dy1, const float* dy2, const float* w1, const float* w2, float* dx, int M, int N1, int N2,
+                               int K, int precision, void* stream) {
+    CSWIN_CHECK_PRECISION(precision, "linear_pair_bwd_data");
+    CSWIN_REQUIRE(dy1 && dy2 && w1 && w2 && dx && M > 0 && N1 > 0 && N2 > 0 && K > 0, CSWIN_ERR_SHAPE, "linear_pair_bwd_data: bad arguments");
+    if (!pair_one_launch(dy1, dy2, w1, w2, dx, N1, N2, K, precision)) {
+        int rc = cswin_linear_bwd_data(dy1, w1, dx, nullptr, 0, nullptr, nullptr, 1, nullptr, M, N1, K, precision, 0, stream);
+        if (rc) return rc;
+        return cswin_linear_bwd_data(dy2, w2, dx, nullptr, 0, nullptr, nullptr, 1, dx, M, N2, K, precision, 0, stream);
+    }
+    const int seg = cdiv(N1, 32) * 32, R = seg + N2;
+    ConcatGapSrc A = {dy1, dy2, N1, N2, M, R, N1, seg};
+    StackSrc B = {w1, w2, K, R, K, N1, seg};
+    Epilogue e = plain_epilogue(dx, K);
+    e.vec_store = epilogue_vec_ok(e, K);
+    auto units = [&](int bn) { return (double)(((long)cdiv(M, 64) * cdiv(K, bn) + 255) / 256) * 64 * bn; };
+    const int tm = cdiv(M, 64);
+    if (units(32) * cswin_tuning().gemm_pen2 < units(64))
+        hipLaunchKernelGGL(gemm_pair_dgrad_kernel<32>, dim3(tm * cdiv(K, 32)), dim3(gemm_threads(64, 32, 1)), 0, (hipStream_t)stream, A, B, e,
+                           M, K, R, seg, tm, cdiv(K, 32));
+    else
+        hipLaunchKernelGGL(gemm_pair_dgrad_kernel<64>, dim3(tm * cdiv(K, 64)), dim3(gemm_threads(64, 64, 1)), 0, (hipStream_t)stream, A, B, e,
+                           M, K, R, seg, tm, cdiv(K, 64));
+    CSWIN_LAUNCH_CHECK();
+    return CSWIN_OK;
+}
+
 size_t cswin_linear_bwd_weight_workspace(int M, int N, int K) { return WgradSlabs::bytes(M, N, K); }
 
 int cswin_linear_bwd_weight(const float* dy, const float* x, const float* x2, int k_split, const float* row_scale,
diff --git a/cswin_unet_amd/csrc/gemm_epilogue.h b/cswin_unet_amd/csrc/gemm_epilogue.h
--- a/cswin_unet_amd/csrc/gemm_epilogue.h
+++ b/cswin_unet_amd/csrc/gemm_epilogue.h
@@ -29,6 +29,7 @@
     int c_bf16;
     int pre_bf16;
     long long* stamps;
+    const float* bias2;
 };
 
 constexpr int EP_LD = 36;
@@ -61,7 +62,9 @@
             const int n = nb + j * 32 + rcol;
             if (vec) {
                 f32x4 bias_v = {0.f, 0.f, 0.f, 0.f};
-                if (e.bias && n < N) bias_v = *reinterpret_cast<const f32x4*>(e.bias + n);
+                if (EPI == EPI_SPLIT2 && n >= e.col_split) {
+                    if (e.bias2 && n < N) bias_v = *reinterpret_cast<const f32x4*>(e.bias2 + (n - e.col_split));
+                } else if (e.bias && n < N) bias_v = *reinterpret_cast<const f32x4*>(e.bias + n);
                 f32x4 v[4], aux[4];
                 u32x2 aux16[4];
                 float rs[4];
@@ -115,7 +118,9 @@
                     for (int c = 0; c < 4; ++c) {
                         const int nn = n + c;
                         if (nn >= N) continue;
-                        float o = wbuf[(rrow + 8 * p) * EP_LD + rcol + c] + (e.bias ? e.bias[nn] : 0.f);
+                        float o;
+                        if (EPI == EPI_SPLIT2 && nn >= e.col_split) o = wbuf[(rrow + 8 * p) * EP_LD + rcol + c] + (e.bias2 ? e.bias2[nn - e.col_split] : 0.f);
+                        else o = wbuf[(rrow + 8 * p) * EP_LD + rcol + c] + (e.bias ? e.bias[nn] : 0.f);
                         if (EPI == EPI_GELUBWD) o *= gelu_grad_f(e.gelu_pre[(long)m * e.ldpre + nn]);
                         o *= rsv;
                         if (EPI == EPI_RES) o += e.residual[(long)m * e.ldres + nn];
@@ -137,7 +142,7 @@
 inline int epilogue_vec_ok(const Epilogue& e, int n_out) {
     auto ok = [](const void* p, long ld) { return !p || (aligned16(p) && ld % 4 == 0); };
     return n_out % 4 == 0 && aligned16(e.C) && e.ldc % 4 == 0 && ok(e.C2, e.ldc2) && (!e.C2 || e.col_split % 4 == 0) &&
-           ok(e.bias, 4) && ok(e.Cact, e.ldact) && ok(e.residual, e.ldres) && ok(e.gelu_pre, e.ldpre) &&
+           ok(e.bias, 4) && ok(e.bias2, 4) && ok(e.Cact, e.ldact) && ok(e.residual, e.ldres) && ok(e.gelu_pre, e.ldpre) &&
            e.split_stride % 4 == 0;
 }
 
diff --git a/cswin_unet_amd/csrc/ln.hip b/cswin_unet_amd/csrc/ln.hip
--- a/cswin_unet_amd/csrc/ln.hip
+++ b/cswin_unet_amd/csrc/ln.hip
@@ -128,6 +128,153 @@
     }
 }
 
+__device__ __forceinline__ float unfused(float v) {
+    asm("" : "+v"(v));
+    return v;
+}
+template <int LPR, int VPL>
+__global__ __launch_bounds__(256) void ln_pair_fwd_kernel(const float* __restrict__ x, const float* __restrict__ gamma_a,
+                                                           const float* __restrict__ beta_a, const float* __restrict__ gamma_b,
+                                                           const float* __restrict__ beta_b, float* __restrict__ y,
+                                                           float* __restrict__ h, float* __restrict__ mean_a,
+                                                           float* __restrict__ rstd_a, float* __restrict__ mean_b,
+                                                           float* __restrict__ rstd_b, int M, float eps_a, float eps_b) {
+    constexpr int C = 4 * LPR * VPL;
+    constexpr int RPB = 256 / LPR;
+    const int sub = threadIdx.x % LPR, rib = threadIdx.x / LPR;
+    f32x4 ga[VPL], ba[VPL], gb[VPL], bb[VPL];
+#pragma unroll
+    for (int v = 0; v < VPL; ++v) {
+        ga[v] = *reinterpret_cast<const f32x4*>(gamma_a + 4 * (sub + v * LPR));
+        ba[v] = *reinterpret_cast<const f32x4*>(beta_a + 4 * (sub + v * LPR));
+        gb[v] = *reinterpret_cast<const f32x4*>(gamma_b + 4 * (sub + v * LPR));
+        bb[v] = *reinterpret_cast<const f32x4*>(beta_b + 4 * (sub + v * LPR));
+    }
+    for (long row = (long)blockIdx.x * RPB + rib; row < M; row += (long)gridDim.x * RPB) {
+        f32x4 xv[VPL];
+#pragma unroll
+        for (int v = 0; v < VPL; ++v) xv[v] = *reinterpret_cast<const f32x4*>(x + row * C + 4 * (sub + v * LPR));
+#pragma unroll
+        for (int pass = 0; pass < 2; ++pass) {
+            float s = 0.f;
+#pragma unroll
+            for (int v = 0; v < VPL; ++v) s += xv[v][0] + xv[v][1] + xv[v][2] + xv[v][3];
+#pragma unroll
+            for (int o = LPR / 2; o > 0; o >>= 1) s += __shfl_xor(s, o, 64);
+            const float mu = unfused(s * (1.0f / C));
+            float q = 0.f;
+#pragma unroll
+            for (int v = 0; v < VPL; ++v)
+#pragma unroll
+                for (int e = 0; e < 4; ++e) {
+                    float d = xv[v][e] - mu;
+                    q += unfused(d * d);
+                }
+#pragma unroll
+            for (int o = LPR / 2; o > 0; o >>= 1) q += __shfl_xor(q, o, 64);
+            const float rs = rsqrtf(__builtin_fmaf(q, 1.0f / C, pass ? eps_b : eps_a));
+#pragma unroll
+            for (int v = 0; v < VPL; ++v) {
+                const f32x4 g = pass ? gb[v] : ga[v], b = pass ? bb[v] : ba[v];
+#pragma unroll
+                for (int e = 0; e < 4; ++e) xv[v][e] = __builtin_fmaf((xv[v][e] - mu) * rs, g[e], b[e]);
+                *reinterpret_cast<f32x4*>((pass ? h : y) + row * C + 4 * (sub + v * LPR)) = xv[v];
+            }
+            if (sub == 0) {
+                (pass ? mean_b : mean_a)[row] = mu;
+                (pass ? rstd_b : rstd_a)[row] = rs;
+            }
+        }
+    }
+}
+
+template <int LPR, int VPL>
+__global__ __launch_bounds__(256) void ln_pair_bwd_kernel(const float* __restrict__ dh, const float* __restrict__ dy,
+                                                           const float* __restrict__ x, const float* __restrict__ ya,
+                                                           const float* __restrict__ mean_a, const float* __restrict__ rstd_a,
+                                                           const float* __restrict__ mean_b, const float* __restrict__ rstd_b,
+                                                           const float* __restrict__ gamma_a, const float* __restrict__ gamma_b,
+                                                           float* __restrict__ dx, float* __restrict__ part_a,
+                                                           float* __restrict__ part_b, int M) {
+    constexpr int C = 4 * LPR * VPL;
+    constexpr int RPB = 256 / LPR;
+    __shared__ float red[2 * RPB * C];
+    const int sub = threadIdx.x % LPR, rib = threadIdx.x / LPR;
+    f32x4 ga[VPL], gb[VPL], dga[VPL], dba[VPL], dgb[VPL], dbb[VPL];
+#pragma unroll
+    for (int v = 0; v < VPL; ++v) {
+        ga[v] = *reinterpret_cast<const f32x4*>(gamma_a + 4 * (sub + v * LPR));
+        gb[v] = *reinterpret_cast<const f32x4*>(gamma_b + 4 * (sub + v * LPR));
+        dga[v] = dba[v] = dgb[v] = dbb[v] = f32x4{0.f, 0.f, 0.f, 0.f};
+    }
+    for (long row = (long)blockIdx.x * RPB + rib; row < M; row += (long)gridDim.x * RPB) {
+        f32x4 d[VPL];
+#pragma unroll
+        for (int v = 0; v < VPL; ++v) d[v] = *reinterpret_cast<const f32x4*>(dh + row * C + 4 * (sub + v * LPR));
+#pragma unroll
+        for (int pass = 0; pass < 2; ++pass) {
+            const float mu = (pass ? mean_a : mean_b)[row], rs = (pass ? rstd_a : rstd_b)[row];
+            f32x4 xh[VPL], gy[VPL];
+            float s1 = 0.f, s2 = 0.f;
+#pragma unroll
+            for (int v = 0; v < VPL; ++v) {
+                const long off = row * C + 4 * (sub + v * LPR);
+                const f32x4 xv = *reinterpret_cast<const f32x4*>((pass ? x : ya) + off);
+                const f32x4 g = pass ? ga[v] : gb[v];
+#pragma unroll
+                for (int e = 0; e < 4; ++e) {
+                    xh[v][e] = (xv[e] - mu) * rs;
+                    gy[v][e] = d[v][e] * g[e];
+                    s1 += gy[v][e];
+                    s2 += gy[v][e] * xh[v][e];
+                    if (pass) {
+                        dga[v][e] += d[v][e] * xh[v][e];
+                        dba[v][e] += d[v][e];
+                    } else {
+                        dgb[v][e] += d[v][e] * xh[v][e];
+                        dbb[v][e] += d[v][e];
+                    }
+                }
+            }
+#pragma unroll
+            for (int o = LPR / 2; o > 0; o >>= 1) {
+                s1 += __shfl_xor(s1, o, 64);
+                s2 += __shfl_xor(s2, o, 64);
+            }
+            s1 *= (1.0f / C);
+            s2 *= (1.0f / C);
+#pragma unroll
+            for (int v = 0; v < VPL; ++v) {
+                const long off = row * C + 4 * (sub + v * LPR);
+#pragma unroll
+                for (int e = 0; e < 4; ++e) d[v][e] = rs * (gy[v][e] - s1 - xh[v][e] * s2);
+                if (pass) *reinterpret_cast<f32x4*>(dx + off) = d[v];
+                else if (dy) d[v] += *reinterpret_cast<const f32x4*>(dy + off);
+            }
+        }
+    }
+#pragma unroll
+    for (int pass = 0; pass < 2; ++pass) {
+        if (pass) __syncthreads();
+#pragma unroll
+        for (int v = 0; v < VPL; ++v)
+#pragma unroll
+            for (int e = 0; e < 4; ++e) {
+                const int c = 4 * (sub + v * LPR) + e;
+                red[rib * C + c] = pass ? dga[v][e] : dgb[v][e];
+                red[RPB * C + rib * C + c] = pass ? dba[v][e] : dbb[v][e];
+            }
+        __syncthreads();
+        float* partial = pass ? part_a : part_b;
+        for (int c = threadIdx.x; c < 2 * C; c += 256) {
+            const int which = c / C, cc = c - which * C;
+            float s = 0.f;
+            for (int r = 0; r < RPB; ++r) s += red[which * RPB * C + r * C + cc];
+            partial[(long)blockIdx.x * 2 * C + c] = s;
+        }
+    }
+}
+
 constexpr int GEN_MAXV = 4;
 
 __global__ __launch_bounds__(256) void ln_fwd_generic_kernel(const float* __restrict__ x, const float* __restrict__ gamma,
@@ -248,7 +395,22 @@
     hipLaunchKernelGGL((ln_bwd_kernel<LPR, VPL>), dim3(ln_grid(M, 256 / LPR)), dim3(256), 0, st, dy, x, mean, rstd, g, dres, dx, partial, M, dx16);
 }
 
+template <int LPR, int VPL>
+void launch_pair_fwd(const float* x, const float* ga, const float* ba, const float* gb, const float* bb, float* y, float* h, float* mean_a,
+                     float* rstd_a, float* mean_b, float* rstd_b, int M, float eps_a, float eps_b, hipStream_t st) {
+    hipLaunchKernelGGL((ln_pair_fwd_kernel<LPR, VPL>), dim3(ln_grid(M, 256 / LPR)), dim3(256), 0, st, x, ga, ba, gb, bb, y, h, mean_a, rstd_a,
+                       mean_b, rstd_b, M, eps_a, eps_b);
+}
+template <int LPR, int VPL>
+void launch_pair_bwd(const float* dh, const float* dy, const float* x, const float* ya, const float* mean_a, const float* rstd_a,
+                     const float* mean_b, const float* rstd_b, const float* ga, const float* gb, float* dx, float* part_a, float* part_b,
+                     int M, hipStream_t st) {
+    hipLaunchKernelGGL((ln_pair_bwd_kernel<LPR, VPL>), dim3(ln_grid(M, 256 / LPR)), dim3(256), 0, st, dh, dy, x, ya, mean_a, rstd_a, mean_b,
+                       rstd_b, ga, gb, dx, part_a, part_b, M);
+}
+
 bool ln_fast(int C) { return C == 64 || C == 128 || C == 256 || C == 512 || C == 32 || C == 1024; }
+bool ln_pair_fused(int C) { return C == 64 || C == 128 || C == 256 || C == 512; }
 bool ln_supported(int C) { return C > 0 && C % 4 == 0 && C <= 256 * GEN_MAXV; }
 
 }
@@ -312,4 +474,65 @@
     return CSWIN_OK;
 }
 
-}
+int cswin_layernorm_pair_fwd(const float* x, const float* gamma_a, const float* beta_a, const float* gamma_b, const float* beta_b,
+                             float* y, float* h, float* mean_a, float* rstd_a, float* mean_b, float* rstd_b, int M, int C, float eps_a,
+                             float eps_b, void* stream) {
+    CSWIN_REQUIRE(x && gamma_a && beta_a && gamma_b && beta_b && y && h && mean_a && rstd_a && mean_b && rstd_b && M > 0, CSWIN_ERR_SHAPE,
+                  "layernorm_pair_fwd: bad arguments");
+    if (!ln_pair_fused(C)) {
+        int rc = cswin_layernorm_fwd(x, gamma_a, beta_a, y, mean_a, rstd_a, M, C, eps_a, 0, stream);
+        if (rc) return rc;
+        return cswin_layernorm_fwd(y, gamma_b, beta_b, h, mean_b, rstd_b, M, C, eps_b, 0, stream);
+    }
+    hipStream_t st = (hipStream_t)stream;
+    switch (C) {
+        case 64: launch_pair_fwd<16, 1>(x, gamma_a, beta_a, gamma_b, beta_b, y, h, mean_a, rstd_a, mean_b, rstd_b, M, eps_a, eps_b, st); break;
+        case 128: launch_pair_fwd<32, 1>(x, gamma_a, beta_a, gamma_b, beta_b, y, h, mean_a, rstd_a, mean_b, rstd_b, M, eps_a, eps_b, st); break;
+        case 256: launch_pair_fwd<64, 1>(x, gamma_a, beta_a, gamma_b, beta_b, y, h, mean_a, rstd_a, mean_b, rstd_b, M, eps_a, eps_b, st); break;
+        case 512: launch_pair_fwd<64, 2>(x, gamma_a, beta_a, gamma_b, beta_b, y, h, mean_a, rstd_a, mean_b, rstd_b, M, eps_a, eps_b, st); break;
+    }
+    CSWIN_LAUNCH_CHECK();
+    return CSWIN_OK;
+}
+
+size_t cswin_layernorm_pair_bwd_workspace(int M, int C) {
+    return 2 * cswin_layernorm_bwd_workspace(M, C) + (ln_pair_fused(C) ? 0 : (size_t)M * C * sizeof(float));
+}
+
+int cswin_layernorm_pair_bwd(const float* dh, const float* dy, const float* x, const float* ya, const float* mean_a, const float* rstd_a,
+                             const float* mean_b, const float* rstd_b, const float* gamma_a, const float* gamma_b, float* dx,
+                             float* dgamma_a, float* dbeta_a, float* dgamma_b, float* dbeta_b, void* workspace, size_t ws_bytes, int M,
+                             int C, cswin_reduce_job* deferred, void* stream) {
+    CSWIN_REQUIRE(dh && x && ya && mean_a && rstd_a && mean_b && rstd_b && gamma_a && gamma_b && dx && dgamma_a && dbeta_a && dgamma_b &&
+                  dbeta_b && M > 0, CSWIN_ERR_SHAPE, "layernorm_pair_bwd: bad arguments");
+    CSWIN_REQUIRE(ln_supported(C), CSWIN_ERR_UNSUPPORTED, "layernorm: C=%d must be a multiple of 4, at most 1024", C);
+    CSWIN_REQUIRE(workspace && ws_bytes >= cswin_layernorm_pair_bwd_workspace(M, C), CSWIN_ERR_WORKSPACE, "layernorm_pair_bwd: workspace too small");
+    const size_t one = cswin_layernorm_bwd_workspace(M, C);
+    float* part_a = (float*)workspace;
+    float* part_b = (float*)((char*)workspace + one);
+    if (!ln_pair_fused(C)) {
+        float* mid = (float*)((char*)workspace + 2 * one);
+        int rc = cswin_layernorm_bwd(dh, ya, mean_b, rstd_b, gamma_b, dy, mid, dgamma_b, dbeta_b, part_b, one, M, C,
+                                     deferred ? deferred + 1 : nullptr, nullptr, stream);
+        if (rc) return rc;
+        return cswin_layernorm_bwd(mid, x, mean_a, rstd_a, gamma_a, nullptr, dx, dgamma_a, dbeta_a, part_a, one, M, C, deferred, nullptr, stream);
+    }
+    hipStream_t st = (hipStream_t)stream;
+    const int lpr = C / 4 > 64 ? 64 : C / 4;
+    const int nblk = ln_grid(M, 256 / lpr);
+    switch (C) {
+        case 64: launch_pair_bwd<16, 1>(dh, dy, x, ya, mean_a, rstd_a, mean_b, rstd_b, gamma_a, gamma_b, dx, part_a, part_b, M, st); break;
+        case 128: launch_pair_bwd<32, 1>(dh, dy, x, ya, mean_a, rstd_a, mean_b, rstd_b, gamma_a, gamma_b, dx, part_a, part_b, M, st); break;
+        case 256: launch_pair_bwd<64, 1>(dh, dy, x, ya, mean_a, rstd_a, mean_b, rstd_b, gamma_a, gamma_b, dx, part_a, part_b, M, st); break;
+        case 512: launch_pair_bwd<64, 2>(dh, dy, x, ya, mean_a, rstd_a, mean_b, rstd_b, gamma_a, gamma_b, dx, part_a, part_b, M, st); break;
+    }
+    CSWIN_LAUNCH_CHECK();
+    const cswin_reduce_job job_a = {part_a, dgamma_a, dbeta_a, C, 2LL * C, 2LL * C, nblk, 0};
+    const cswin_reduce_job job_b = {part_b, dgamma_b, dbeta_b, C, 2LL * C, 2LL * C, nblk, 0};
+    reduce_now_or_defer(job_a, deferred, st);
+    reduce_now_or_defer(job_b, deferred ? deferred + 1 : nullptr, st);
+    CSWIN_LAUNCH_CHECK();
+    return CSWIN_OK;
+}
+
+}
diff --git a/cswin_unet_amd/networks/cswin_unet.py b/cswin_unet_amd/networks/cswin_unet.py
--- a/cswin_unet_amd/networks/cswin_unet.py
+++ b/cswin_unet_amd/networks/cswin_unet.py
@@ -89,7 +89,10 @@
             return dp.sample_scale(x.shape[0], x.device), dp.sample_scale(x.shape[0], x.device)
         return None, None
 
-    def forward(self, x):
+    def live_dropout(self):
+        return self.training and (self.proj_drop.p > 0 or self.mlp.drop.p > 0)
+
+    def forward(self, x, pre=None):
         B, L, C = x.shape
         if L != self.patches_resolution ** 2:
             raise AssertionError("flatten img_tokens has wrong size")
@@ -98,7 +101,8 @@
         if type(self.norm1) is not nn.LayerNorm or type(self.norm2) is not nn.LayerNorm:
             raise NotImplementedError("the HIP block fuses nn.LayerNorm only")
         rs1, rs2 = self._keep_scales(x)
-        if self.training and (self.proj_drop.p > 0 or self.mlp.drop.p > 0):
+        if self.live_dropout():
+            assert pre is None
             n1, n2 = self.norm1, self.norm2
             qkv = ops.linear(ops.layer_norm(x, n1.weight, n1.bias, n1.eps), self.qkv.weight, self.qkv.bias)
             att = ops.stripe_attention(qkv, self.patches_resolution, self.split_size, [m.idx for m in a], [m.num_heads for m in a],
@@ -107,7 +111,7 @@
             return self.mlp(ops.layer_norm(x, n2.weight, n2.bias, n2.eps), residual=x, row_scale=rs2)
         return ops.cswin_block(x, self.patches_resolution, self.split_size, [m.idx for m in a], [m.num_heads for m in a],
                                a[0].scale, self.norm1, self.qkv, self.proj, self.norm2, self.mlp.fc1, self.mlp.fc2,
-                               [m.get_v.weight for m in a], [m.get_v.bias for m in a], rs1, rs2, attn_drop=ad)
+                               [m.get_v.weight for m in a], [m.get_v.bias for m in a], rs1, rs2, attn_drop=ad, pre=pre)
 
 
 def img2windows(img, H_sp, W_sp):
@@ -124,9 +128,11 @@
         self.conv = nn.Conv2d(dim, dim_out, 3, 2, 1)
         self.norm = norm_layer(dim_out)
 
-    def forward(self, x):
+    def forward(self, x, then=None):
         side = _square_side(x.shape[1])
         y = ops.conv_tokens(x, self.conv.weight, self.conv.bias, side, side, 2, 1)
+        if then is not None:
+            return ops.layer_norm_pair(y, self.norm, then)
         return ops.layer_norm(y, self.norm.weight, self.norm.bias, self.norm.eps)
 
 
@@ -181,11 +187,13 @@
             w = _SumInputChannels.apply(w)
         return w
 
-    def forward(self, img, w=None):
+    def forward(self, img, w=None, then=None):
         conv, norm = self[0], self[2]
         if w is None:
             w = self.conv_weight(img)
         tok = ops.patch_embed_conv(img, w, conv.bias, conv.stride[0], conv.padding[0])
+        if then is not None:
+            return ops.layer_norm_pair(tok, norm, then)
         return ops.layer_norm(tok, norm.weight, norm.bias, norm.eps)
 
 
@@ -261,6 +269,17 @@
             x = checkpoint.checkpoint(blk, x, use_reentrant=False) if self.use_chk else blk(x)
         return x
 
+    def _enter(self, blocks, entry, *args, dropout=0.0):
+        first = blocks[0]
+        norms = (entry[2] if isinstance(entry, _PatchEmbed) else entry.norm, first.norm1, first.norm2)
+        if not (self.use_chk or dropout > 0 or ops.act_bf16() or first.live_dropout() or any(type(n) is not nn.LayerNorm for n in norms)):
+            x, pre = entry(*args, then=first.norm1)
+            return self._run(list(blocks)[1:], first(x, pre=pre))
+        x = entry(*args)
+        if dropout > 0:
+            x = ops.dropout(x, dropout)
+        return self._run(blocks, x)
+
     def _predraw_drop_path(self, batch, device):
         blocks = [b for st in (self.stage1, self.stage2, self.stage3, self.stage4, self.stage_up4, self.stage_up3,
                                self.stage_up2, self.stage_up1) for b in st]
@@ -282,20 +301,17 @@
     def forward_features(self, x, pe_weight=None):
         self._predraw_drop_path(x.shape[0], x.device)
         ops.clear_twins()
-        x = self.stage1_conv_embed(x, pe_weight)
-        if self.pos_drop.p > 0 and self.training:
-            x = ops.dropout(x, self.pos_drop.p)
-        x = self._run(self.stage1, x)
+        x = self._enter(self.stage1, self.stage1_conv_embed, x, pe_weight, dropout=self.pos_drop.p if self.training else 0.0)
         self.x1 = x
-        x = self._run(self.stage2, self.merge1(x))
+        x = self._enter(self.stage2, self.merge1, x)
         self.x2 = x
         self.enc_mid_in = None
         if getattr(self, "detach_decoder_inputs", False) and torch.is_grad_enabled():
             x = x.detach().requires_grad_()
             self.enc_mid_in = x
-        x = self._run(self.stage3, self.merge2(x))
+        x = self._enter(self.stage3, self.merge2, x)
         self.x3 = x
-        x = self._run(self.stage4, self.merge3(x))
+        x = self._enter(self.stage4, self.merge3, x)
         return ops.layer_norm(x, self.norm.weight, self.norm.bias, self.norm.eps)
 
     def forward_up_features(self, x):
diff --git a/cswin_unet_amd/ops.py b/cswin_unet_amd/ops.py
--- a/cswin_unet_amd/ops.py
+++ b/cswin_unet_amd/ops.py
@@ -8,7 +8,7 @@
 
 from ._lib import AugmentDesc, ConvImageJob, CswinHipError, ReduceJob, WgradDesc, act_bf16, call, dev_f32, lib, precision, ptr, shadow_ptr, stream
 
-__all__ = ["layer_norm", "linear", "linear_pair", "mlp", "stripe_attention", "cswin_block", "conv_tokens", "patch_embed_conv", "carafe_reassemble",
+__all__ = ["layer_norm", "layer_norm_pair", "linear", "linear_pair", "mlp", "stripe_attention", "cswin_block", "conv_tokens", "patch_embed_conv", "carafe_reassemble",
            "carafe_reassemble_nchw", "conv_weight_images", "head_compose", "tokens_to_nchw", "matmul_nn", "ce_dice_loss", "continual_loss", "dropout", "img2windows", "windows2img",
            "seg_metrics", "resize_slices", "argmax_zoom_back", "augment_batch", "class_counts"]
 
@@ -159,6 +159,44 @@
 
 def layer_norm(x, gamma, beta, eps=1e-5):
     return _LayerNorm.apply(x, gamma, beta, eps)
+
+
+class _LayerNormPair(Function):
+
+    @staticmethod
+    def forward(ctx, x, ga, ba, eps_a, gb, bb, eps_b):
+        x, ga, ba, gb, bb = (dev_f32(t, "layer_norm_pair input") for t in (x, ga, ba, gb, bb))
+        C = x.shape[-1]
+        M = x.numel() // C
+        y, h = torch.empty_like(x), torch.empty_like(x)
+        ma, ra, mb, rb = (torch.empty(M, dtype=torch.float32, device=x.device) for _ in range(4))
+        call("cswin_layernorm_pair_fwd", ptr(x), ptr(ga), ptr(ba), ptr(gb), ptr(bb), ptr(y), ptr(h), ptr(ma), ptr(ra), ptr(mb), ptr(rb),
+             M, C, eps_a, eps_b, stream())
+        ctx.save_for_backward(x, y, ga, gb, ma, ra, mb, rb)
+        ctx.keys = _param_keys(ga, ba, gb, bb)
+        ctx.mark_non_differentiable(mb, rb)
+        ctx.set_materialize_grads(False)
+        return y, h, mb, rb
+
+    @staticmethod
+    @once_differentiable
+    def backward(ctx, dy, dh, _dmean, _drstd):
+        x, y, ga, gb, ma, ra, mb, rb = ctx.saved_tensors
+        C = x.shape[-1]
+        M = x.numel() // C
+        dx = torch.empty_like(x)
+        dga, dba, dgb, dbb = (_pass.grad(k, ga.shape, ga.device) for k in ctx.keys)
+        dy, dh = dev_f32(dy), dev_f32(dh) if dh is not None else torch.zeros_like(x)
+        _reduced(lib().cswin_layernorm_pair_bwd_workspace(M, C), x.device,
+                 lambda ws, nbytes, jobs: call("cswin_layernorm_pair_bwd", ptr(dh), ptr(dy), ptr(x), ptr(y), ptr(ma), ptr(ra), ptr(mb), ptr(rb),
+                                               ptr(ga), ptr(gb), ptr(dx), ptr(dga), ptr(dba), ptr(dgb), ptr(dbb), ws, nbytes, M, C, jobs,
+                                               stream()), njobs=2)
+        return dx, dga, dba, None, dgb, dbb, None
+
+
+def layer_norm_pair(x, norm_a, norm_b):
+    y, h, mean, rstd = _LayerNormPair.apply(x, norm_a.weight, norm_a.bias, norm_a.eps, norm_b.weight, norm_b.bias, norm_b.eps)
+    return y, (h, mean, rstd)
 
 
 _twins = {}
@@ -272,7 +310,11 @@
         assert w1.shape[1] == w2.shape[1] == x.shape[-1]
         ctx.save_for_backward(x, w1, w2)
         ctx.keys = _param_keys(w1, b1, w2, b2)
-        return tuple(_linear_fwd(x, w, b, w.shape[0]) for w, b in ((w1, b1), (w2, b2)))
+        K = x.shape[-1]
+        y1, y2 = (torch.empty(x.shape[:-1] + (w.shape[0],), dtype=torch.float32, device=x.device) for w in (w1, w2))
+        call("cswin_linear_pair_fwd", ptr(x), ptr(w1), ptr(b1), ptr(w2), ptr(b2), ptr(y1), ptr(y2), x.numel() // K, w1.shape[0], w2.shape[0],
+             K, precision(), stream())
+        return y1, y2
 
     @staticmethod
     @once_differentiable
@@ -284,8 +326,7 @@
         dx = None
         if ctx.needs_input_grad[0]:
             dx = torch.empty_like(x)
-            _linear_bwd_data(dy1, w1, dx)
-            _linear_bwd_data(dy2, w2, dx, add=dx)
+            call("cswin_linear_pair_bwd_data", ptr(dy1), ptr(dy2), ptr(w1), ptr(w2), ptr(dx), M, w1.shape[0], w2.shape[0], K, precision(), stream())
         grads, keep = [], []
         wg, jobs = (WgradDesc * 2)(), (ReduceJob * 2)()
         for i, (dy, w) in enumerate(((dy1, w1), (dy2, w2))):
@@ -481,8 +522,8 @@
 class _CSWinBlock(Function):
 
     @staticmethod
-    def forward(ctx, x, reso, split, idx, heads, scale, eps1, eps2, rs1, rs2, drop, g1, b1, wqkv, bqkv, wp, bp, g2, b2, w1, bb1,
-                w2, bb2, *lepe):
+    def forward(ctx, x, reso, split, idx, heads, scale, eps1, eps2, rs1, rs2, drop, pre_h, pre_mean, pre_rstd, g1, b1, wqkv, bqkv, wp, bp,
+                g2, b2, w1, bb1, w2, bb2, *lepe):
         x = dev_f32(x, "block input")
         B, L, C = x.shape
         if L != reso * reso:
@@ -497,7 +538,12 @@
         E16 = lambda *shape: torch.empty(*shape, dtype=t16, device=dev)
         sq, sp, s1, s2 = (_wsrc(w) if s16 else w for w in (wqkv, wp, w1, w2))
         attn = (reso, split, tuple(idx), tuple(heads), scale, drop, ATTN_MFMA16 if s16 else ATTN_FP32)
-        h1, m1, r1 = _layernorm_fwd(x, g1, b1, eps1, t16)
+        ctx.pre = pre_h is not None
+        if ctx.pre:
+            assert not s16 and g1 is None and b1 is None, "a precomputed norm1 is fp32 and brings its own parameters"
+            h1, m1, r1 = dev_f32(pre_h), dev_f32(pre_mean), dev_f32(pre_rstd)
+        else:
+            h1, m1, r1 = _layernorm_fwd(x, g1, b1, eps1, t16)
         qkv = _linear_fwd(h1, sq, bqkv, 3 * C, dtype=t16)
         att, lse = E16(B, L, C), torch.empty(B, sum(heads), L, dtype=torch.float32, device=dev)
         att0 = E16(B, L, C) if any(ctx.needs_input_grad) else None
@@ -575,20 +621,25 @@
             _linear_bwd_data(dqkv, sq, dh1)
         for slot, ji in enumerate((0, 1, 3, 4)):
             jobs[ji] = wjobs[slot]
-        dx, dg1, dbt1 = torch.empty_like(x), G(kg1, C), G(kb1, C)
-        dx16 = torch.empty_like(x, dtype=torch.bfloat16) if s16 else None
-        _layernorm_bwd(dh1, x, m1, r1, g1, dx, dg1, dbt1, (wsp[5], sizes[5], _job_ptr(jobs, 5)), dres=dx1, dx16=dx16)
-        if s16:
-            _twin_put(dx, dx16)
+        if ctx.pre:
+            dx, dpre, dg1, dbt1 = dx1, dh1, None, None
+        else:
+            dx, dpre, dg1, dbt1 = torch.empty_like(x), None, G(kg1, C), G(kb1, C)
+            dx16 = torch.empty_like(x, dtype=torch.bfloat16) if s16 else None
+            _layernorm_bwd(dh1, x, m1, r1, g1, dx, dg1, dbt1, (wsp[5], sizes[5], _job_ptr(jobs, 5)), dres=dx1, dx16=dx16)
+            if s16:
+                _twin_put(dx, dx16)
         _pass.reduce(jobs, (ws, aws))
-        grads = (dx, None, None, None, None, None, None, None, None, None, None, dg1, dbt1, dwqkv, dbqkv, dwp, dbp, dg2, dbt2, dw1, db1,
-                 dw2, db2)
+        grads = (dx, None, None, None, None, None, None, None, None, None, None, dpre, None, None, dg1, dbt1, dwqkv, dbqkv, dwp, dbp, dg2,
+                 dbt2, dw1, db1, dw2, db2)
         return grads + tuple(d.view(d.shape[0], 1, 3, 3) for d in dlw) + tuple(dlb)
 
 
-def cswin_block(x, reso, split, idx, heads, scale, norm1, qkv, proj, norm2, fc1, fc2, lepe_w, lepe_b, rs1=None, rs2=None, attn_drop=0.0):
+def cswin_block(x, reso, split, idx, heads, scale, norm1, qkv, proj, norm2, fc1, fc2, lepe_w, lepe_b, rs1=None, rs2=None, attn_drop=0.0,
+                pre=None):
+    g1, b1 = (norm1.weight, norm1.bias) if pre is None else (None, None)
     return _CSWinBlock.apply(x, reso, split, tuple(idx), tuple(heads), scale, norm1.eps, norm2.eps, rs1, rs2, _attn_drop(attn_drop),
-                             norm1.weight, norm1.bias, qkv.weight, qkv.bias, proj.weight, proj.bias, norm2.weight,
+                             *(pre or (None, None, None)), g1, b1, qkv.weight, qkv.bias, proj.weight, proj.bias, norm2.weight,
                              norm2.bias, fc1.weight, fc1.bias, fc2.weight, fc2.bias, *lepe_w, *lepe_b)
 
 
diff --git a/include/cswin_hip.h b/include/cswin_hip.h
--- a/include/cswin_hip.h
+++ b/include/cswin_hip.h
@@ -49,12 +49,25 @@
                         const float* dres, float* dx, float* dgamma, float* dbeta, void* workspace, size_t ws_bytes,
                         int M, int C, cswin_reduce_job* deferred, void* dx_bf16, void* stream);
 
+int cswin_layernorm_pair_fwd(const float* x, const float* gamma_a, const float* beta_a, const float* gamma_b, const float* beta_b,
+                             float* y, float* h, float* mean_a, float* rstd_a, float* mean_b, float* rstd_b, int M, int C, float eps_a,
+                             float eps_b, void* stream);
+size_t cswin_layernorm_pair_bwd_workspace(int M, int C);
+int cswin_layernorm_pair_bwd(const float* dh, const float* dy, const float* x, const float* ya, const float* mean_a, const float* rstd_a,
+                             const float* mean_b, const float* rstd_b, const float* gamma_a, const float* gamma_b, float* dx,
+                             float* dgamma_a, float* dbeta_a, float* dgamma_b, float* dbeta_b, void* workspace, size_t ws_bytes, int M,
+                             int C, cswin_reduce_job* deferred, void* stream);
+
 int cswin_linear_fwd(const float* x, const float* x2, int k_split, const float* w, const float* bias, float* y,
                      float* y_act, const float* residual, const float* row_scale, int rows_per_sample, int M, int N,
                      int K, int precision, int io_bf16, void* stream);
 int cswin_linear_bwd_data(const float* dy, const float* w, float* dx, float* dx2, int k_split, const float* gelu_pre,
                           const float* row_scale, int rows_per_sample, const float* add, int M, int N, int K,
                           int precision, int io_bf16, void* stream);
+int cswin_linear_pair_fwd(const float* x, const float* w1, const float* b1, const float* w2, const float* b2, float* y1, float* y2,
+                          int M, int N1, int N2, int K, int precision, void* stream);
+int cswin_linear_pair_bwd_data(const float* dy1, const float* dy2, const float* w1, const float* w2, float* dx, int M, int N1, int N2,
+                               int K, int precision, void* stream);
 size_t cswin_linear_bwd_weight_workspace(int M, int N, int K);
 int cswin_linear_bwd_weight(const float* dy, const float* x, const float* x2, int k_split, const float* row_scale,
                             int rows_per_sample, float* dw, float* dbias, void* workspace, size_t ws_bytes, int M,
```

Measured after the change: 1960 images/sec (median of 6 runs). No clear change (+0.7%).
